# matsengrp/linearham

Measured on AMD Instinct MI355X. Metric: phylo-HMM log-likelihood evals/sec (100-leaf x 400-site family), higher is better.
Workload: dtype f64

## Files before the change

include/linearham_amd.h:

```cpp
#ifndef LINEARHAM_AMD_H_
#define LINEARHAM_AMD_H_

#include <stddef.h>
#include <stdint.h>

#ifdef __cplusplus
extern "C" {
#endif

#define LH_ABI_VERSION 1

typedef struct lh_family lh_family;

typedef struct {
  int32_t n_genes;
  const int32_t* offsets;
  const int32_t* xmsa_inds;
} lh_segments;

typedef struct {
  int32_t n_rows;
  int32_t n_left;
  int32_t n_right;
  const double* enter_trans;
  const double* enter_lo;
  const double* left_trans;
  const double* left_lo;
  const int32_t* left_xmsa;
  const double* right_gp_nli;
  const double* right_ntt;
  const double* right_nlo;
  const double* right_trans;
  const double* right_gp_li;
  const int32_t* right_xmsa;
  const int32_t* nti_xmsa;
  const double* exit_nlo;
  const double* exit_trans;
  const double* exit_gp_li;
} lh_junction;

typedef struct {
  int32_t abi_version;
  int32_t has_d;
  int32_t n_seqs;
  int32_t n_sites;
  const uint8_t* msa;
  int32_t n_xmsa;
  const int32_t* xmsa_site;
  const uint8_t* xmsa_naive_base;
  lh_segments vpadding, vgerm, dgerm, jgerm, jpadding;
  const double* vgerm_gene_prob;
  const double* vpadding_transition;
  const double* vgerm_trans_prod;
  const double* jpadding_transition;
  lh_junction vd, dj;
} lh_family_desc;

typedef struct {
  double* rates;
  double* xmsa_emission;
  double* forward;
  int32_t* scaler_counts;
} lh_eval_outputs;

const char* lh_last_error(void);
int lh_device_count(void);

int lh_warmup(void);
int lh_set_device(int32_t device);
void* lh_host_alloc(size_t bytes);
void lh_host_free(void* p);

int lh_family_create(const lh_family_desc* desc, lh_family** out);
void lh_family_destroy(lh_family* fam);

int64_t lh_forward_size(const lh_family* fam);
int64_t lh_scaler_size(const lh_family* fam);

int lh_family_info(const lh_family* fam, int32_t* n_patterns, int32_t* n_unique_columns);

int lh_family_consensus_sets(const lh_family* fam);

const char* lh_family_prune_form(const lh_family* fam);

const char* lh_family_forward_form(const lh_family* fam);

int lh_family_forward_dj_samples(const lh_family* fam);

int lh_family_forward_dj_waves(const lh_family* fam);

int lh_family_set_extended_range(lh_family* fam, int enable);

typedef struct {
  int32_t n_rows, n_left, n_right, n_states;
  const int32_t* left_rows;
  const int32_t* left_dense;
  const double* left_lo;
  const double* left_trans;
  const double* enter_lo;
  const int32_t* right_dense;
  const int32_t* right_first;
  const double* gene_prob;
  const double* nti_landing_in;
  const double* nti_transition;
  const double* nti_landing_out;
  const double* landing_in;
  const double* right_trans;
  const double* exit_nlo;
  const double* exit_trans;
  const double* exit_li;
  const double* prod;
} lh_sampler_junction;

typedef struct {
  lh_sampler_junction vd, dj;
} lh_sampler_desc;

int lh_family_set_sampler(lh_family* fam, const lh_sampler_desc* desc);

int32_t lh_sample_words(const lh_family* fam);
int32_t lh_sample_states(const lh_family* fam);

int lh_eval_sample_batch(lh_family* fam, int32_t n, int32_t n_tips, int32_t max_depth, const int32_t* ops,
                         const double* brlen, const double* er, const double* pi, const double* alpha,
                         int32_t num_rates, const uint32_t* words, double* loglik, double* rates, int32_t* states);

int lh_eval_sample_batch_device(lh_family* fam, int32_t n, int32_t n_tips, int32_t max_depth, const int32_t* ops,
                                const double* brlen, const double* er, const double* pi, const double* alpha,
                                int32_t num_rates, const uint32_t* words, double* loglik, double* rates,
                                int32_t* states, void* hip_stream);

typedef struct {
  const double* log_offset;
  double* loglik;
  double* posterior;
  double* weighted_sum;
  double* weight_stats;
} lh_posterior_outputs;

int lh_eval_posterior_batch(lh_family* fam, int32_t n, int32_t n_tips, int32_t max_depth, const int32_t* ops,
                            const double* brlen, const double* er, const double* pi, const double* alpha,
                            int32_t num_rates, const lh_posterior_outputs* outs);

int lh_eval_posterior_batch_device(lh_family* fam, int32_t n, int32_t n_tips, int32_t max_depth, const int32_t* ops,
                                   const double* brlen, const double* er, const double* pi, const double* alpha,
                                   int32_t num_rates, const lh_posterior_outputs* outs, void* hip_stream);

int lh_posterior_profile_read(lh_family* fam, double* ms_posterior, int64_t* n_launches);

int lh_family_set_candidates(lh_family* fam, int32_t K, const uint8_t* seqs, double* log_prior);

typedef struct {
  const double* log_offset;
  double* loglik;
  double* log_cand;
  double* weighted_sum;
  double* weight_stats;
} lh_candidate_outputs;

int lh_eval_candidates_batch(lh_family* fam, int32_t n, int32_t n_tips, int32_t max_depth, const int32_t* ops,
                             const double* brlen, const double* er, const double* pi, const double* alpha,
                             int32_t num_rates, const lh_candidate_outputs* outs);

int lh_eval_candidates_batch_device(lh_family* fam, int32_t n, int32_t n_tips, int32_t max_depth, const int32_t* ops,
                                    const double* brlen, const double* er, const double* pi, const double* alpha,
                                    int32_t num_rates, const lh_candidate_outputs* outs, void* hip_stream);

int lh_candidates_info(const lh_family* fam, int32_t* n_candidates, int32_t* n_sites);

int lh_candidates_layout(const lh_family* fam, int32_t* n_var_sites, int32_t* n_lem, int32_t* n_vlem);

int lh_candidates_profile_read(lh_family* fam, double* ms, int64_t* n_launches);

int lh_eval_draw_batch(lh_family* fam, int32_t n, int32_t n_tips, int32_t max_depth, const int32_t* ops,
                       const double* brlen, const double* er, const double* pi, const double* alpha,
                       int32_t num_rates, const uint32_t* words, double* loglik, uint64_t* hash, int32_t* states);

int lh_eval_draw_batch_device(lh_family* fam, int32_t n, int32_t n_tips, int32_t max_depth, const int32_t* ops,
                              const double* brlen, const double* er, const double* pi, const double* alpha,
                              int32_t num_rates, const uint32_t* words, double* loglik, uint64_t* hash,
                              int32_t* states, void* hip_stream);

int lh_naive_sequences(lh_family* fam, int32_t n, const int32_t* states, uint8_t* seqs, uint64_t* hash);

int lh_draws_resolve(lh_family* fam, int32_t n, const int32_t* cand, int32_t* n_mismatch, int32_t* mismatch_rows);
int lh_draws_rows_read(lh_family* fam, int32_t n_rows, const int32_t* rows, uint8_t* seqs);
int lh_draws_candidates_read(lh_family* fam, int32_t* K, uint8_t* seqs);
int lh_draws_reset(lh_family* fam);
int lh_collect_profile_read(lh_family* fam, double* ms, int64_t* n_launches);

#define LH_LINEAGE_PAD_HASH 0ull
int lh_lineage_batch(lh_family* fam, int32_t n, int32_t n_tips, int32_t max_depth, const int32_t* ops,
                     const double* brlen, const double* er, const double* pi, const double* rates, int32_t num_rates,
                     const uint8_t* naive, uint64_t seed, uint64_t first_sample, const int32_t* path,
                     int32_t path_len, uint64_t* nt_hash, uint64_t* aa_hash);

int lh_lineage_collect_device(lh_family* fam, int32_t n, int32_t n_tips, const uint8_t* anc, const uint8_t* naive,
                              const int32_t* path, int32_t path_len, uint64_t* nt_hash, uint64_t* aa_hash,
                              void* hip_stream);

int lh_lineage_resolve(lh_family* fam, int32_t n_slots, const int32_t* ids, int32_t* n_mismatch,
                       int32_t* mismatch_slots);
int lh_lineage_rows_read(lh_family* fam, int32_t n_slots, const int32_t* slots, uint8_t* seqs);
int lh_lineage_store_read(lh_family* fam, int32_t first, int32_t count, int32_t* K, uint8_t* seqs);
int lh_lineage_reset(lh_family* fam);
int lh_lineage_profile_read(lh_family* fam, double* ms, int64_t* n_launches);

typedef struct {
  double* loglik;
  double* rates;
  int32_t* states;
  uint8_t* naive;
  uint64_t* naive_hash;
  uint64_t* nt_hash;
  uint64_t* aa_hash;
} lh_lineage_eval_outputs;

int lh_eval_lineage_batch(lh_family* fam, int32_t n, int32_t n_tips, int32_t max_depth, const int32_t* ops,
                          const double* brlen, const double* er, const double* pi, const double* alpha,
                          int32_t num_rates, const uint32_t* words, uint64_t seed, uint64_t first_sample, int32_t draws,
                          const int32_t* path, int32_t path_len, const lh_lineage_eval_outputs* outs);

int lh_eval_lineage_batch_device(lh_family* fam, int32_t n, int32_t n_tips, int32_t max_depth, const int32_t* ops,
                                 const double* brlen, const double* er, const double* pi, const double* alpha,
                                 int32_t num_rates, const uint32_t* words, uint64_t seed, uint64_t first_sample,
                                 int32_t draws, const int32_t* path, int32_t path_len,
                                 const lh_lineage_eval_outputs* outs, void* hip_stream);

int lh_lineage_eval_profile_read(lh_family* fam, double* ms, int64_t* n_launches);

int lh_schedule_tree(int32_t n_tips, const int32_t* children, int32_t root, int32_t* ops,
                     int32_t* max_depth);

int lh_eval_batch(lh_family* fam, int32_t n, int32_t n_tips, int32_t max_depth, const int32_t* ops,
                  const double* brlen, const double* er, const double* pi, const double* alpha,
                  int32_t num_rates, double* loglik, const lh_eval_outputs* outs);

int lh_eval_batch_device(lh_family* fam, int32_t n, int32_t n_tips, int32_t max_depth,
                         const int32_t* ops, const double* brlen, const double* er, const double* pi,
                         const double* alpha, int32_t num_rates, double* loglik,
                         const lh_eval_outputs* outs, void* hip_stream);

int lh_family_status(lh_family* fam);
// ... 202 lines not shown
```

linearham_amd/capi.py:

```python
import ctypes as C
import os

import numpy as np

_HERE = os.path.dirname(os.path.abspath(__file__))

c_i32p = C.POINTER(C.c_int32)
c_u8p = C.POINTER(C.c_uint8)
c_f64p = C.POINTER(C.c_double)


class _Segments(C.Structure):
    _fields_ = [("n_genes", C.c_int32), ("offsets", c_i32p), ("xmsa_inds", c_i32p)]


class _Junction(C.Structure):
    _fields_ = [("n_rows", C.c_int32), ("n_left", C.c_int32), ("n_right", C.c_int32),
                ("enter_trans", c_f64p), ("enter_lo", c_f64p), ("left_trans", c_f64p),
                ("left_lo", c_f64p), ("left_xmsa", c_i32p), ("right_gp_nli", c_f64p),
                ("right_ntt", c_f64p), ("right_nlo", c_f64p), ("right_trans", c_f64p),
                ("right_gp_li", c_f64p), ("right_xmsa", c_i32p), ("nti_xmsa", c_i32p),
                ("exit_nlo", c_f64p), ("exit_trans", c_f64p), ("exit_gp_li", c_f64p)]


class _FamilyDesc(C.Structure):
    _fields_ = [("abi_version", C.c_int32), ("has_d", C.c_int32), ("n_seqs", C.c_int32),
                ("n_sites", C.c_int32), ("msa", c_u8p), ("n_xmsa", C.c_int32),
                ("xmsa_site", c_i32p), ("xmsa_naive_base", c_u8p),
                ("vpadding", _Segments), ("vgerm", _Segments), ("dgerm", _Segments),
                ("jgerm", _Segments), ("jpadding", _Segments),
                ("vgerm_gene_prob", c_f64p), ("vpadding_transition", c_f64p),
                ("vgerm_trans_prod", c_f64p), ("jpadding_transition", c_f64p),
                ("vd", _Junction), ("dj", _Junction)]


class _EvalOutputs(C.Structure):
    _fields_ = [("rates", c_f64p), ("xmsa_emission", c_f64p), ("forward", c_f64p),
                ("scaler_counts", c_i32p)]


EXPORTS = ["lh_last_error", "lh_device_count", "lh_family_create", "lh_family_destroy",
           "lh_forward_size", "lh_scaler_size", "lh_family_info", "lh_family_consensus_sets", "lh_schedule_tree", "lh_eval_batch",
           "lh_eval_batch_device", "lh_forward_batch", "lh_asr_batch", "lh_asr_batch_device",
           "lh_profile_enable", "lh_profile_read", "lh_asr_profile_read", "lh_family_set_extended_range", "lh_warmup", "lh_host_alloc", "lh_host_free", "lh_family_set_sampler",
           "lh_sample_words", "lh_sample_states", "lh_eval_sample_batch", "lh_set_device", "lh_family_status",
           "lh_eval_sample_batch_device", "lh_family_prune_form", "lh_family_forward_form",
           "lh_family_forward_dj_samples", "lh_family_forward_dj_waves"]
CRAFTED_EXPORTS = ["lh_sample_forward_batch", "lh_posterior_forward_batch"]
EXPORTS += CRAFTED_EXPORTS
POSTERIOR_EXPORTS = ["lh_eval_posterior_batch", "lh_eval_posterior_batch_device", "lh_posterior_profile_read"]
EXPORTS += POSTERIOR_EXPORTS
CANDIDATE_EXPORTS = ["lh_family_set_candidates", "lh_eval_candidates_batch", "lh_eval_candidates_batch_device",
                     "lh_candidates_profile_read", "lh_candidates_info", "lh_candidates_layout"]
EXPORTS += CANDIDATE_EXPORTS
COLLECT_EXPORTS = ["lh_eval_draw_batch", "lh_eval_draw_batch_device", "lh_naive_sequences", "lh_draws_resolve",
                   "lh_draws_rows_read", "lh_draws_candidates_read", "lh_draws_reset", "lh_collect_profile_read"]
EXPORTS += COLLECT_EXPORTS
LINEAGE_EXPORTS = ["lh_lineage_batch", "lh_lineage_collect_device", "lh_lineage_resolve", "lh_lineage_rows_read",
                   "lh_lineage_store_read", "lh_lineage_reset", "lh_lineage_profile_read"]
EXPORTS += LINEAGE_EXPORTS
LINEAGE_PAD_HASH = 0
LINEAGE_EVAL_EXPORTS = ["lh_eval_lineage_batch", "lh_eval_lineage_batch_device", "lh_lineage_eval_profile_read"]
EXPORTS += LINEAGE_EVAL_EXPORTS
VITERBI_EXPORTS = ["lh_eval_viterbi_batch", "lh_eval_viterbi_batch_device", "lh_viterbi_forward_batch",
                   "lh_family_set_candidate_paths", "lh_viterbi_profile_read"]
EXPORTS += VITERBI_EXPORTS
CODON_EXPORTS = ["lh_family_set_codons", "lh_codon_layout", "lh_eval_codons_batch", "lh_eval_codons_batch_device",
                 "lh_codon_profile_read"]
EXPORTS += CODON_EXPORTS
EVENTS_EXPORTS = ["lh_events_layout", "lh_eval_events_batch", "lh_eval_events_batch_device", "lh_events_forward_batch",
                  "lh_events_profile_read"]
EXPORTS += EVENTS_EXPORTS
ANCESTRAL_EXPORTS = ["lh_asr_marginals_batch", "lh_asr_marginals_batch_device", "lh_eval_ancestral_batch",
                     "lh_eval_ancestral_batch_device", "lh_ancestral_profile_read"]
EXPORTS += ANCESTRAL_EXPORTS
EDGES_EXPORTS = ["lh_asr_edges_batch", "lh_asr_edges_batch_device", "lh_eval_edges_batch", "lh_eval_edges_batch_device",
                 "lh_edges_profile_read"]
EXPORTS += EDGES_EXPORTS
ANCESTRAL_PROBS_EXPORTS = ["lh_family_set_ancestral_candidates", "lh_ancestral_candidates_info",
                           "lh_eval_ancestral_candidates_batch", "lh_eval_ancestral_candidates_batch_device",
                           "lh_ancestral_candidates_profile_read"]
EXPORTS += ANCESTRAL_PROBS_EXPORTS
NODE_PARENT, NODE_MRCA = 0, 1


class _CodonOutputs(C.Structure):
    _fields_ = [("log_offset", c_f64p), ("loglik", c_f64p), ("windows", c_f64p), ("genes", c_f64p),
                ("weighted_windows", c_f64p), ("weighted_genes", c_f64p), ("weight_stats", c_f64p)]


class _CodonOutputsDevice(C.Structure):
    _fields_ = [(k, C.c_void_p) for k in ("log_offset", "loglik", "windows", "genes", "weighted_windows",
                                          "weighted_genes", "weight_stats")]


class _EventsOutputs(C.Structure):
    _fields_ = [("log_offset", c_f64p), ("loglik", c_f64p), ("events", c_f64p), ("genes", c_f64p),
                ("weighted_events", c_f64p), ("weighted_genes", c_f64p), ("weight_stats", c_f64p)]


class _EventsOutputsDevice(C.Structure):
    _fields_ = [(k, C.c_void_p) for k in ("log_offset", "loglik", "events", "genes", "weighted_events", "weighted_genes",
                                          "weight_stats")]


class _ViterbiOutputs(C.Structure):
    _fields_ = [("log_offset", c_f64p), ("loglik", c_f64p), ("states", c_i32p), ("log_path", c_f64p),
                ("weight_stats", c_f64p)]


class _ViterbiOutputsDevice(C.Structure):
    _fields_ = [(k, C.c_void_p) for k in ("log_offset", "loglik", "states", "log_path", "weight_stats")]


_ANCESTRAL_MEMBERS = ("log_offset", "loglik", "site_base", "marg", "rate_post", "weighted_sum", "weighted_rate",
                      "weight_stats")


class _AncestralOutputs(C.Structure):
    _fields_ = [(k, c_f64p) for k in _ANCESTRAL_MEMBERS]


class _AncestralOutputsDevice(C.Structure):
    _fields_ = [(k, C.c_void_p) for k in _ANCESTRAL_MEMBERS]


_EDGES_MEMBERS = ("edge", "naive_edge", "chain_counts", "edge_load", "rate_post")
_EVAL_EDGES_MEMBERS = ("log_offset", "loglik", "site_base", "edge", "naive_edge", "chain_counts", "seed_edge", "edge_load",
                       "rate_post", "weighted_counts", "weighted_seed_edge", "weighted_naive_edge", "weight_stats")


class _EdgesOutputs(C.Structure):
    _fields_ = [(k, c_f64p) for k in _EDGES_MEMBERS]


class _EdgesOutputsDevice(C.Structure):
    _fields_ = [(k, C.c_void_p) for k in _EDGES_MEMBERS]


class _EvalEdgesOutputs(C.Structure):
    _fields_ = [(k, c_f64p) for k in _EVAL_EDGES_MEMBERS]


class _EvalEdgesOutputsDevice(C.Structure):
    _fields_ = [(k, C.c_void_p) for k in _EVAL_EDGES_MEMBERS]


_ANCESTRAL_PROBS_MEMBERS = ("log_offset", "loglik", "cond", "log_cand", "weighted_sum", "weight_stats")


class _AncestralProbsOutputs(C.Structure):
    _fields_ = [(k, c_f64p) for k in _ANCESTRAL_PROBS_MEMBERS]


class _AncestralProbsOutputsDevice(C.Structure):
    _fields_ = [(k, C.c_void_p) for k in _ANCESTRAL_PROBS_MEMBERS]


class _SamplerJunction(C.Structure):
    _fields_ = [("n_rows", C.c_int32), ("n_left", C.c_int32), ("n_right", C.c_int32), ("n_states", C.c_int32),
                ("left_rows", c_i32p), ("left_dense", c_i32p), ("left_lo", c_f64p), ("left_trans", c_f64p),
                ("enter_lo", c_f64p), ("right_dense", c_i32p), ("right_first", c_i32p), ("gene_prob", c_f64p),
                ("nti_landing_in", c_f64p), ("nti_transition", c_f64p), ("nti_landing_out", c_f64p),
                ("landing_in", c_f64p), ("right_trans", c_f64p), ("exit_nlo", c_f64p), ("exit_trans", c_f64p),
                ("exit_li", c_f64p), ("prod", c_f64p)]


class _SamplerDesc(C.Structure):
    _fields_ = [("vd", _SamplerJunction), ("dj", _SamplerJunction)]


class _PosteriorOutputs(C.Structure):
    _fields_ = [("log_offset", c_f64p), ("loglik", c_f64p), ("posterior", c_f64p), ("weighted_sum", c_f64p),
                ("weight_stats", c_f64p)]


class _CandidateOutputs(C.Structure):
    _fields_ = [("log_offset", c_f64p), ("loglik", c_f64p), ("log_cand", c_f64p), ("weighted_sum", c_f64p),
                ("weight_stats", c_f64p)]


class _LineageEvalOutputs(C.Structure):
    _fields_ = [("loglik", c_f64p), ("rates", c_f64p), ("states", c_i32p), ("naive", c_u8p),
                ("naive_hash", C.POINTER(C.c_uint64)), ("nt_hash", C.POINTER(C.c_uint64)),
                ("aa_hash", C.POINTER(C.c_uint64))]


class _LineageEvalOutputsDevice(C.Structure):
    _fields_ = [(k, C.c_void_p) for k in ("loglik", "rates", "states", "naive", "naive_hash", "nt_hash", "aa_hash")]


def library_path():
    return os.path.join(os.environ.get("LH_LIB_DIR") or os.path.join(_HERE, "lib"), "liblinearham_hip.so")


_HOST_TREE = [C.c_void_p, C.c_int32, C.c_int32, C.c_int32, c_i32p, c_f64p, c_f64p, c_f64p, c_f64p, C.c_int32]
_DEV_TREE = [C.c_void_p, C.c_int32, C.c_int32, C.c_int32] + [C.c_void_p] * 5 + [C.c_int32]
_PROFILE_READ = [C.c_void_p, c_f64p, C.POINTER(C.c_int64)]


class HipLibrary:
    def __init__(self, path=None):
        path = path or library_path()
        if not os.path.exists(path):
            raise RuntimeError("HIP library %s is missing: run `python -c 'import __graft_entry__ as g; "
                               "g.build()'` (there is no CPU fallback)" % path)
        self.lib = lib = C.CDLL(path)
        c_u32p, c_u64p = C.POINTER(C.c_uint32), C.POINTER(C.c_uint64)
        lib.lh_last_error.restype = C.c_char_p
        lib.lh_device_count.restype = C.c_int
        lib.lh_family_create.argtypes = [C.POINTER(_FamilyDesc), C.POINTER(C.c_void_p)]
        lib.lh_family_destroy.argtypes = [C.c_void_p]
        lib.lh_family_destroy.restype = None
        lib.lh_forward_size.argtypes = [C.c_void_p]
        lib.lh_forward_size.restype = C.c_int64
        lib.lh_scaler_size.argtypes = [C.c_void_p]
        lib.lh_scaler_size.restype = C.c_int64
        lib.lh_family_info.argtypes = [C.c_void_p, C.POINTER(C.c_int32), C.POINTER(C.c_int32)]
        lib.lh_family_info.restype = C.c_int
        lib.lh_family_consensus_sets.argtypes = [C.c_void_p]
        lib.lh_family_consensus_sets.restype = C.c_int
        lib.lh_family_prune_form.argtypes = [C.c_void_p]
        lib.lh_family_prune_form.restype = C.c_char_p
        lib.lh_family_forward_form.argtypes = [C.c_void_p]
        lib.lh_family_forward_form.restype = C.c_char_p
        if hasattr(lib, "lh_family_forward_dj_samples"):
            lib.lh_family_forward_dj_samples.argtypes = [C.c_void_p]
            lib.lh_family_forward_dj_samples.restype = C.c_int
        if hasattr(lib, "lh_family_forward_dj_waves"):
            lib.lh_family_forward_dj_waves.argtypes = [C.c_void_p]
            lib.lh_family_forward_dj_waves.restype = C.c_int
        lib.lh_schedule_tree.argtypes = [C.c_int32, c_i32p, C.c_int32, c_i32p, c_i32p]
        lib.lh_eval_batch.argtypes = _HOST_TREE + [c_f64p, C.POINTER(_EvalOutputs)]
        lib.lh_eval_batch_device.argtypes = _DEV_TREE + [C.c_void_p, C.POINTER(_EvalOutputs), C.c_void_p]
        lib.lh_forward_batch.argtypes = [C.c_void_p, C.c_int32, c_f64p, c_f64p, C.POINTER(_EvalOutputs)]
        lib.lh_asr_batch.argtypes = _HOST_TREE + [c_u8p, C.c_uint64, C.c_uint64, c_u8p, c_u8p]
        lib.lh_asr_batch_device.argtypes = _DEV_TREE + [C.c_void_p, C.c_uint64, C.c_uint64] + [C.c_void_p] * 3
        lib.lh_asr_profile_read.argtypes = _PROFILE_READ
        lib.lh_profile_enable.argtypes = [C.c_void_p, C.c_int]
        lib.lh_family_set_extended_range.argtypes = [C.c_void_p, C.c_int]
        lib.lh_profile_read.argtypes = [C.c_void_p, c_f64p, c_f64p, c_f64p, C.POINTER(C.c_int64)]
        if hasattr(lib, "lh_eval_sample_batch_device"):
            lib.lh_eval_sample_batch_device.argtypes = _DEV_TREE + [C.c_void_p] * 5
            lib.lh_sample_words.argtypes = [C.c_void_p]
            lib.lh_sample_states.argtypes = [C.c_void_p]
        if hasattr(lib, "lh_sample_forward_batch"):
            lib.lh_sample_forward_batch.argtypes = [C.c_void_p, C.c_int32, c_f64p, c_u32p, c_f64p, c_i32p,
                                                    C.POINTER(_EvalOutputs)]
            lib.lh_posterior_forward_batch.argtypes = [C.c_void_p, C.c_int32, c_f64p, c_f64p, c_f64p]
        if hasattr(lib, "lh_eval_posterior_batch"):
            lib.lh_eval_posterior_batch.argtypes = _HOST_TREE + [C.POINTER(_PosteriorOutputs)]
            lib.lh_eval_posterior_batch_device.argtypes = _DEV_TREE + [C.POINTER(_PosteriorOutputs), C.c_void_p]
            lib.lh_posterior_profile_read.argtypes = _PROFILE_READ
        if hasattr(lib, "lh_family_set_candidates"):
            lib.lh_family_set_candidates.argtypes = [C.c_void_p, C.c_int32, c_u8p, c_f64p]
            lib.lh_eval_candidates_batch.argtypes = _HOST_TREE + [C.POINTER(_CandidateOutputs)]
            lib.lh_eval_candidates_batch_device.argtypes = _DEV_TREE + [C.POINTER(_CandidateOutputs), C.c_void_p]
            lib.lh_candidates_profile_read.argtypes = _PROFILE_READ
            lib.lh_candidates_info.argtypes = [C.c_void_p, c_i32p, c_i32p]
            lib.lh_candidates_layout.argtypes = [C.c_void_p, c_i32p, c_i32p, c_i32p]
        if hasattr(lib, "lh_naive_sequences"):
            lib.lh_eval_draw_batch.argtypes = _HOST_TREE + [c_u32p, c_f64p, c_u64p, c_i32p]
            lib.lh_eval_draw_batch_device.argtypes = _DEV_TREE + [C.c_void_p] * 5
            lib.lh_naive_sequences.argtypes = [C.c_void_p, C.c_int32, c_i32p, c_u8p, c_u64p]
            lib.lh_draws_resolve.argtypes = [C.c_void_p, C.c_int32, c_i32p, c_i32p, c_i32p]
            lib.lh_draws_rows_read.argtypes = [C.c_void_p, C.c_int32, c_i32p, c_u8p]
            lib.lh_draws_candidates_read.argtypes = [C.c_void_p, c_i32p, c_u8p]
            lib.lh_draws_reset.argtypes = [C.c_void_p]
            lib.lh_collect_profile_read.argtypes = _PROFILE_READ
        if hasattr(lib, "lh_lineage_batch"):
            lib.lh_lineage_batch.argtypes = _HOST_TREE + [c_u8p, C.c_uint64, C.c_uint64, c_i32p, C.c_int32, c_u64p, c_u64p]
            lib.lh_lineage_collect_device.argtypes = [C.c_void_p, C.c_int32, C.c_int32, C.c_void_p, C.c_void_p,
                                                      C.c_void_p, C.c_int32, C.c_void_p, C.c_void_p, C.c_void_p]
            lib.lh_lineage_resolve.argtypes = [C.c_void_p, C.c_int32, c_i32p, c_i32p, c_i32p]
            lib.lh_lineage_rows_read.argtypes = [C.c_void_p, C.c_int32, c_i32p, c_u8p]
            lib.lh_lineage_store_read.argtypes = [C.c_void_p, C.c_int32, C.c_int32, c_i32p, c_u8p]
            lib.lh_lineage_reset.argtypes = [C.c_void_p]
            lib.lh_lineage_profile_read.argtypes = _PROFILE_READ
        if hasattr(lib, "lh_eval_lineage_batch"):
            lib.lh_eval_lineage_batch.argtypes = _HOST_TREE + [c_u32p, C.c_uint64, C.c_uint64, C.c_int32, c_i32p, C.c_int32,
                                                               C.POINTER(_LineageEvalOutputs)]
            lib.lh_eval_lineage_batch_device.argtypes = _DEV_TREE + [
                C.c_void_p, C.c_uint64, C.c_uint64, C.c_int32, C.c_void_p, C.c_int32, C.POINTER(_LineageEvalOutputsDevice),
                C.c_void_p]
            lib.lh_lineage_eval_profile_read.argtypes = _PROFILE_READ
        if hasattr(lib, "lh_eval_viterbi_batch"):
            lib.lh_family_set_sampler.argtypes = [C.c_void_p, C.POINTER(_SamplerDesc)]
            lib.lh_eval_viterbi_batch.argtypes = _HOST_TREE + [C.POINTER(_ViterbiOutputs)]
            lib.lh_eval_viterbi_batch_device.argtypes = _DEV_TREE + [C.POINTER(_ViterbiOutputsDevice), C.c_void_p]
            lib.lh_viterbi_forward_batch.argtypes = [C.c_void_p, C.c_int32, c_f64p, c_f64p, c_i32p]
            lib.lh_family_set_candidate_paths.argtypes = [C.c_void_p, C.c_int32, c_i32p, c_f64p]
            lib.lh_viterbi_profile_read.argtypes = _PROFILE_READ
        if hasattr(lib, "lh_family_set_codons"):
            lib.lh_family_set_codons.argtypes = [C.c_void_p, C.c_int32]
            lib.lh_codon_layout.argtypes = [C.c_void_p, c_i32p, c_i32p, c_i32p, c_i32p]
            lib.lh_eval_codons_batch.argtypes = _HOST_TREE + [C.POINTER(_CodonOutputs)]
            lib.lh_eval_codons_batch_device.argtypes = _DEV_TREE + [C.POINTER(_CodonOutputsDevice), C.c_void_p]
            lib.lh_codon_profile_read.argtypes = _PROFILE_READ
        if hasattr(lib, "lh_events_layout"):
            c_i64p = C.POINTER(C.c_int64)
            lib.lh_events_layout.argtypes = [C.c_void_p, c_i32p, c_i32p, c_i32p, c_i32p, c_i64p, c_i64p, c_i64p, c_i64p,
                                             c_i32p]
            lib.lh_eval_events_batch.argtypes = _HOST_TREE + [C.POINTER(_EventsOutputs)]
            lib.lh_eval_events_batch_device.argtypes = _DEV_TREE + [C.POINTER(_EventsOutputsDevice), C.c_void_p]
            lib.lh_events_forward_batch.argtypes = [C.c_void_p, C.c_int32, c_f64p, c_f64p, c_f64p]
            lib.lh_events_profile_read.argtypes = _PROFILE_READ
        if hasattr(lib, "lh_asr_marginals_batch"):
            lib.lh_asr_marginals_batch.argtypes = _HOST_TREE + [c_f64p, c_i32p, C.c_int32, c_f64p, c_f64p]
            lib.lh_asr_marginals_batch_device.argtypes = _DEV_TREE + [C.c_void_p, C.c_void_p, C.c_int32] + [C.c_void_p] * 3
            lib.lh_eval_ancestral_batch.argtypes = _HOST_TREE + [c_i32p, C.c_int32, C.POINTER(_AncestralOutputs)]
            lib.lh_eval_ancestral_batch_device.argtypes = _DEV_TREE + [C.c_void_p, C.c_int32,
                                                                       C.POINTER(_AncestralOutputsDevice), C.c_void_p]
            lib.lh_ancestral_profile_read.argtypes = _PROFILE_READ
        if hasattr(lib, "lh_asr_edges_batch"):
            lib.lh_asr_edges_batch.argtypes = _HOST_TREE + [c_f64p, c_i32p, C.c_int32, C.c_int32, C.POINTER(_EdgesOutputs)]
            lib.lh_asr_edges_batch_device.argtypes = _DEV_TREE + [C.c_void_p, C.c_void_p, C.c_int32, C.c_int32,
                                                                  C.POINTER(_EdgesOutputsDevice), C.c_void_p]
            lib.lh_eval_edges_batch.argtypes = _HOST_TREE + [c_i32p, C.c_int32, C.c_int32, C.POINTER(_EvalEdgesOutputs)]
            lib.lh_eval_edges_batch_device.argtypes = _DEV_TREE + [C.c_void_p, C.c_int32, C.c_int32,
                                                                   C.POINTER(_EvalEdgesOutputsDevice), C.c_void_p]
            lib.lh_edges_profile_read.argtypes = _PROFILE_READ
        if hasattr(lib, "lh_family_set_ancestral_candidates"):
            lib.lh_family_set_ancestral_candidates.argtypes = [C.c_void_p, C.c_int32, c_u8p]
            lib.lh_ancestral_candidates_info.argtypes = [C.c_void_p, c_i32p, c_i32p]
            lib.lh_eval_ancestral_candidates_batch.argtypes = _HOST_TREE + [c_i32p, C.c_int32, C.c_int32,
                                                                            C.POINTER(_AncestralProbsOutputs)]
            lib.lh_eval_ancestral_candidates_batch_device.argtypes = _DEV_TREE + [
                C.c_void_p, C.c_int32, C.c_int32, C.POINTER(_AncestralProbsOutputsDevice), C.c_void_p]
            lib.lh_ancestral_candidates_profile_read.argtypes = _PROFILE_READ
        if hasattr(lib, "lh_set_device"):
            lib.lh_set_device.argtypes = [C.c_int32]
            lib.lh_family_status.argtypes = [C.c_void_p]

    def error(self):
        return self.lib.lh_last_error().decode()

    def check(self, rc):
        if rc != 0:
            raise RuntimeError("linearham_hip: " + self.error())

    def device_count(self):
        return self.lib.lh_device_count()

    def _profile_read(self, name, family, n_ms=1):
        ms, k = (C.c_double * n_ms)(), C.c_int64()
        self.check(getattr(self.lib, name)(_handle(family), ms, C.byref(k)))
        return tuple(ms) + (k.value,)

    def eval_posterior_batch(self, family, n_tips, max_depth, ops, brlen, er, pi, alpha, num_rates, log_offset=None,
                             want=("loglik", "posterior", "weighted_sum", "weight_stats")):
        h = _handle(family)
        n, arrays = _tree_args(ops, brlen, er, pi, alpha)
        fs = self.lib.lh_forward_size(h)
        res, outs = _outputs(_PosteriorOutputs, want, log_offset, loglik=(n,), posterior=(n, fs), weighted_sum=(fs,),
                             weight_stats=(3,))
        self.check(self.lib.lh_eval_posterior_batch(h, n, n_tips, max_depth, *_tree_ptrs(arrays), num_rates, C.byref(outs)))
        return res

    def eval_ancestral_batch(self, family, n_tips, max_depth, ops, brlen, er, pi, alpha, num_rates, path, log_offset=None,
                             want=("loglik", "site_base", "marg", "rate_post", "weighted_sum", "weighted_rate",
                                   "weight_stats")):
        h = _handle(family)
        n, arrays = _tree_args(ops, brlen, er, pi, alpha)
        path = _i32(path)
        assert path.ndim == 2 and path.shape[0] == n
        P, R = path.shape[1], num_rates
        _, L = self.candidates_info(h)
        res, outs = _outputs(_AncestralOutputs, want, log_offset, loglik=(n,), site_base=(n, L, 5), marg=(n, P, L, 4),
                             rate_post=(n, L, R), weighted_sum=(2, L, 4), weighted_rate=(L, R), weight_stats=(3,))
        self.check(self.lib.lh_eval_ancestral_batch(h, n, n_tips, max_depth, *_tree_ptrs(arrays), num_rates,
                                                    _ptr(path, c_i32p), P, C.byref(outs)))
        return res

    def eval_ancestral_batch_device(self, family, n, n_tips, max_depth, ops_ptr, brlen_ptr, er_ptr, pi_ptr, alpha_ptr,
                                    num_rates, path_ptr, path_len, outs, stream=0):
        o = _AncestralOutputsDevice(**{k: int(v) for k, v in outs.items() if v})
        self.check(self.lib.lh_eval_ancestral_batch_device(_handle(family), n, n_tips, max_depth, ops_ptr, brlen_ptr, er_ptr,
                                                           pi_ptr, alpha_ptr, num_rates, path_ptr, path_len, C.byref(o),
                                                           stream))

    def ancestral_profile_read(self, family):
        return self._profile_read("lh_ancestral_profile_read", family, 3)

    def ancestral_candidates_info(self, family):
# ... 412 lines not shown

    def c(self):
        j = _Junction()
        j.n_rows, j.n_left, j.n_right = self.n_rows, self.n_left, self.n_right
        for k in self.F64:
            setattr(j, k, getattr(self, k).ctypes.data_as(c_f64p))
        for k in self.I32:
            setattr(j, k, getattr(self, k).ctypes.data_as(c_i32p))
        return j


class SamplerJunction:
    F64 = ["left_lo", "left_trans", "enter_lo", "gene_prob", "nti_landing_in", "nti_transition", "nti_landing_out",
           "landing_in", "right_trans", "exit_nlo", "exit_trans", "exit_li", "prod"]
    I32 = ["left_rows", "left_dense", "right_dense", "right_first"]

    def __init__(self, n_rows, n_left, n_right, n_states, **arrays):
        self.n_rows, self.n_left, self.n_right, self.n_states = n_rows, n_left, n_right, n_states
        for k in self.F64:
            setattr(self, k, _f64(arrays[k]))
        for k in self.I32:
            setattr(self, k, _i32(arrays[k]))

    def c(self):
        j = _SamplerJunction()
        j.n_rows, j.n_left, j.n_right, j.n_states = self.n_rows, self.n_left, self.n_right, self.n_states
        for k in self.F64:
            setattr(j, k, getattr(self, k).ctypes.data_as(c_f64p))
        for k in self.I32:
            setattr(j, k, getattr(self, k).ctypes.data_as(c_i32p))
        return j


class FamilyDesc:

    def __init__(self, has_d, msa, xmsa_site, xmsa_naive_base, vpadding, vgerm, dgerm, jgerm, jpadding,
                 vgerm_gene_prob, vpadding_transition, vgerm_trans_prod, jpadding_transition, vd, dj,
                 n_xmsa=None):
        self.has_d = int(has_d)
        self.msa = np.ascontiguousarray(msa, dtype=np.uint8)
        self.xmsa_site = _i32(xmsa_site)
        self.xmsa_naive_base = np.ascontiguousarray(xmsa_naive_base, dtype=np.uint8)
        self.n_xmsa = int(n_xmsa if n_xmsa is not None else len(self.xmsa_site))
        self.vpadding, self.vgerm, self.dgerm, self.jgerm, self.jpadding = vpadding, vgerm, dgerm, jgerm, jpadding
        self.vgerm_gene_prob = _f64(vgerm_gene_prob)
        self.vpadding_transition = _f64(vpadding_transition)
        self.vgerm_trans_prod = _f64(vgerm_trans_prod)
        self.jpadding_transition = _f64(jpadding_transition)
        self.vd, self.dj = vd, dj

    def c(self):
        d = _FamilyDesc()
        d.abi_version = 1
        d.has_d = self.has_d
        d.n_seqs = self.msa.shape[0] if self.msa.ndim == 2 else 0
        d.n_sites = self.msa.shape[1] if self.msa.ndim == 2 else 0
        d.msa = self.msa.ctypes.data_as(c_u8p)
        d.n_xmsa = self.n_xmsa
        d.xmsa_site = self.xmsa_site.ctypes.data_as(c_i32p)
        d.xmsa_naive_base = self.xmsa_naive_base.ctypes.data_as(c_u8p)
        d.vpadding, d.vgerm, d.jgerm, d.jpadding = (self.vpadding.c(), self.vgerm.c(), self.jgerm.c(),
                                                    self.jpadding.c())
        if self.dgerm is not None:
            d.dgerm = self.dgerm.c()
        d.vgerm_gene_prob = self.vgerm_gene_prob.ctypes.data_as(c_f64p)
        d.vpadding_transition = self.vpadding_transition.ctypes.data_as(c_f64p)
        d.vgerm_trans_prod = self.vgerm_trans_prod.ctypes.data_as(c_f64p)
        d.jpadding_transition = self.jpadding_transition.ctypes.data_as(c_f64p)
        d.vd = self.vd.c()
        if self.dj is not None:
            d.dj = self.dj.c()
        return d


class Family:

    def __init__(self, desc, lib=None):
        self.hip = lib or load_library()
        self.desc = desc
        h = C.c_void_p()
        cdesc = desc.c()
        self.hip.check(self.hip.lib.lh_family_create(C.byref(cdesc), C.byref(h)))
        self.handle = h
        self.forward_size = self.hip.lib.lh_forward_size(h)
        self.scaler_size = self.hip.lib.lh_scaler_size(h)
        self.n_xmsa = desc.n_xmsa
        self.consensus_sets = self.hip.lib.lh_family_consensus_sets(h)

    @classmethod
    def borrow(cls, handle, lib=None):
        self = cls.__new__(cls)
        self.hip = lib or load_library()
        self.desc = None
        self.handle = C.c_void_p(handle) if isinstance(handle, int) else handle
        self.owned = False
        self.forward_size = self.hip.lib.lh_forward_size(self.handle)
        self.scaler_size = self.hip.lib.lh_scaler_size(self.handle)
        return self

    def close(self):
        if self.handle:
            if getattr(self, "owned", True):
                self.hip.lib.lh_family_destroy(self.handle)
            self.handle = None

    def __del__(self):
        try:
            self.close()
        except Exception:
            pass

    def _outs(self, n, R, want):
        shapes = dict(rates=(n, R), forward=(n, self.forward_size), scaler_counts=((n, self.scaler_size), np.int32))
        if "xmsa_emission" in want:
            shapes["xmsa_emission"] = (n, self.n_xmsa)
        res, outs = _outputs(_EvalOutputs, want, **shapes)
        return outs, res

    def eval_batch(self, n_tips, max_depth, ops, brlen, er, pi, alpha, num_rates, want=()):
        _, arrays = _tree_args(ops, brlen, er, pi, alpha)
        ops, brlen, er, pi, alpha = arrays
        n = alpha.shape[0]
        assert ops.shape == (n, n_tips - 2, 4) and brlen.shape == (n, 2 * n_tips - 2)
        assert er.shape == (n, 6) and pi.shape == (n, 4)
        ll = np.zeros(n)
        outs, res = self._outs(n, num_rates, want)
        self.hip.check(self.hip.lib.lh_eval_batch(self.handle, n, n_tips, max_depth, *_tree_ptrs(arrays), num_rates,
                                                  _ptr(ll), C.byref(outs)))
        return ll, res

    def eval_batch_device(self, n, n_tips, max_depth, ops_ptr, brlen_ptr, er_ptr, pi_ptr, alpha_ptr,
                          num_rates, loglik_ptr, stream=0):
        self.hip.check(self.hip.lib.lh_eval_batch_device(
            self.handle, n, n_tips, max_depth, ops_ptr, brlen_ptr, er_ptr, pi_ptr, alpha_ptr, num_rates,
            loglik_ptr, None, stream))

    def info(self):
        a, b = C.c_int32(), C.c_int32()
        self.hip.check(self.hip.lib.lh_family_info(self.handle, C.byref(a), C.byref(b)))
        return a.value, b.value

    def k1_form(self):
        return self.hip.lib.lh_family_prune_form(self.handle).decode()

    def k2_form(self):
        return self.hip.lib.lh_family_forward_form(self.handle).decode()

    def k2_dj_samples(self):
        return int(self.hip.lib.lh_family_forward_dj_samples(self.handle))

    def k2_dj_waves(self):
        return int(self.hip.lib.lh_family_forward_dj_waves(self.handle))

    def status(self):
        self.hip.check(self.hip.lib.lh_family_status(self.handle))

    def forward_batch(self, em, want=()):
        em = _f64(em)
        n = em.shape[0]
        assert em.shape == (n, self.n_xmsa)
        ll = np.zeros(n)
        outs, res = self._outs(n, 1, [w for w in want if w in ("forward", "scaler_counts")])
        self.hip.check(self.hip.lib.lh_forward_batch(self.handle, n, em.ctypes.data_as(c_f64p),
                                                     ll.ctypes.data_as(c_f64p), C.byref(outs)))
        return ll, res

    def asr_batch(self, n_tips, max_depth, ops, brlen, er, pi, rates, naive, seed, first_sample=0):
        _, arrays = _tree_args(ops, brlen, er, pi, rates)
        ops, brlen, er, pi, rates = arrays
        naive = np.ascontiguousarray(naive, dtype=np.uint8)
        n, L = naive.shape
        assert ops.shape == (n, n_tips - 2, 4) and brlen.shape == (n, 2 * n_tips - 2)
        assert er.shape == (n, 6) and pi.shape == (n, 4) and rates.shape[0] == n
        anc = np.zeros((n, n_tips - 2, L), dtype=np.uint8)
        choice = np.zeros((n, L), dtype=np.uint8)
        self.hip.check(self.hip.lib.lh_asr_batch(self.handle, n, n_tips, max_depth, *_tree_ptrs(arrays), rates.shape[1],
                                                 _ptr(naive, c_u8p), seed, first_sample, _ptr(anc, c_u8p),
                                                 _ptr(choice, c_u8p)))
        return anc, choice

    def asr_marginals_batch(self, n_tips, max_depth, ops, brlen, er, pi, rates, naive_prob, path,
                            want=("marg", "rate_post")):
        _, arrays = _tree_args(ops, brlen, er, pi, rates)
        ops, brlen, er, pi, rates = arrays
        naive_prob = _f64(naive_prob)
        path = _i32(path)
        n, L = naive_prob.shape[:2]
        assert naive_prob.shape == (n, L, 5) and path.ndim == 2 and path.shape[0] == n
        assert ops.shape == (n, n_tips - 2, 4) and brlen.shape == (n, 2 * n_tips - 2)
        assert er.shape == (n, 6) and pi.shape == (n, 4) and rates.shape[0] == n
        P, R = path.shape[1], rates.shape[1]
        marg = np.zeros((n, P, L, 4)) if "marg" in want else None
        rate_post = np.zeros((n, L, R)) if "rate_post" in want else None
        self.hip.check(self.hip.lib.lh_asr_marginals_batch(
            self.handle, n, n_tips, max_depth, *_tree_ptrs(arrays), R, _ptr(naive_prob), _ptr(path, c_i32p), P,
            _ptr(marg), _ptr(rate_post)))
        return marg, rate_post

    def asr_marginals_batch_device(self, n, n_tips, max_depth, ops_ptr, brlen_ptr, er_ptr, pi_ptr, rates_ptr, num_rates,
                                   naive_prob_ptr, path_ptr, path_len, marg_ptr, rate_post_ptr, stream=0):
        self.hip.check(self.hip.lib.lh_asr_marginals_batch_device(
            self.handle, n, n_tips, max_depth, ops_ptr, brlen_ptr, er_ptr, pi_ptr, rates_ptr, num_rates, naive_prob_ptr,
            path_ptr, path_len, marg_ptr, rate_post_ptr, stream))

    def ancestral_profile_read(self):
        r = self.hip._profile_read("lh_ancestral_profile_read", self.handle, 3)
        return dict(zip(("k11a_ms", "k11b_ms", "reduce_ms"), r[:3])), r[3]

    def asr_edges_batch(self, n_tips, max_depth, ops, brlen, er, pi, rates, naive_prob, path, seed_tip,
                        want=_EDGES_MEMBERS):
        _, arrays = _tree_args(ops, brlen, er, pi, rates)
        ops, brlen, er, pi, rates = arrays
        naive_prob = _f64(naive_prob)
        path = _i32(path)
        n, L = naive_prob.shape[:2]
        assert naive_prob.shape == (n, L, 5) and path.ndim == 2 and path.shape[0] == n
        assert ops.shape == (n, n_tips - 2, 4) and brlen.shape == (n, 2 * n_tips - 2)
        assert er.shape == (n, 6) and pi.shape == (n, 4) and rates.shape[0] == n
        P, R = path.shape[1], rates.shape[1]
        res, outs = _outputs(_EdgesOutputs, want, edge=(n, P, L, 4, 4), naive_edge=(n, L, 5, 4), chain_counts=(n, L, 4, 4),
                             edge_load=(n, P + 1), rate_post=(n, L, R))
        self.hip.check(self.hip.lib.lh_asr_edges_batch(
            self.handle, n, n_tips, max_depth, *_tree_ptrs(arrays), R, _ptr(naive_prob), _ptr(path, c_i32p), P, int(seed_tip),
            C.byref(outs)))
        return res

    def asr_edges_batch_device(self, n, n_tips, max_depth, ops_ptr, brlen_ptr, er_ptr, pi_ptr, rates_ptr, num_rates,
                               naive_prob_ptr, path_ptr, path_len, seed_tip, outs, stream=0):
        o = _EdgesOutputsDevice(**{k: int(v) for k, v in outs.items() if v})
        self.hip.check(self.hip.lib.lh_asr_edges_batch_device(
            self.handle, n, n_tips, max_depth, ops_ptr, brlen_ptr, er_ptr, pi_ptr, rates_ptr, num_rates, naive_prob_ptr,
            path_ptr, path_len, int(seed_tip), C.byref(o), stream))

    def edges_profile_read(self):
        r = self.hip._profile_read("lh_edges_profile_read", self.handle, 3)
        return dict(zip(("k11a_ms", "k12b_ms", "reduce_ms"), r[:3])), r[3]

    def lineage_batch(self, n_tips, max_depth, ops, brlen, er, pi, rates, naive, seed, path, first_sample=0):
        _, arrays = _tree_args(ops, brlen, er, pi, rates)
        ops, brlen, er, pi, rates = arrays
        naive = np.ascontiguousarray(naive, dtype=np.uint8)
        path = _i32(path)
        n, L = naive.shape
        assert ops.shape == (n, n_tips - 2, 4) and brlen.shape == (n, 2 * n_tips - 2)
        assert er.shape == (n, 6) and pi.shape == (n, 4) and rates.shape[0] == n and path.shape[0] == n
        P = path.shape[1]
        nt = np.zeros((n, P + 1), dtype=np.uint64)
        aa = np.zeros((n, P + 1), dtype=np.uint64)
        u64 = C.POINTER(C.c_uint64)
        self.hip.check(self.hip.lib.lh_lineage_batch(
            self.handle, n, n_tips, max_depth, *_tree_ptrs(arrays), rates.shape[1], _ptr(naive, c_u8p), seed, first_sample,
            _ptr(path, c_i32p), P, _ptr(nt, u64), _ptr(aa, u64)))
        self._lineage_sites = L
        return nt, aa

    def eval_lineage_batch(self, n_tips, max_depth, ops, brlen, er, pi, alpha, num_rates, words, seed, path, draws=1,
                           first_sample=0):
        n, arrays = _tree_args(ops, brlen, er, pi, alpha)
        ops, brlen, er, pi, alpha = arrays
        words = np.ascontiguousarray(words, dtype=np.uint32)
        path = _i32(path)
        assert ops.shape == (n, n_tips - 2, 4) and brlen.shape == (n, 2 * n_tips - 2)
        assert er.shape == (n, 6) and pi.shape == (n, 4) and alpha.shape == (n,) and path.shape[0] == n
        P = path.shape[1]
        lib = self.hip.lib
        _, L = self.hip.candidates_info(self.handle)
        d = max(int(draws), 0)
        shapes = dict(loglik=(n,), rates=(n, num_rates), states=((n, lib.lh_sample_states(self.handle)), np.int32),
                      naive=((n, L), np.uint8), naive_hash=((n,), np.uint64), nt_hash=((n, d, P + 1), np.uint64),
                      aa_hash=((n, d, P + 1), np.uint64))
        res, outs = _outputs(_LineageEvalOutputs, shapes, **shapes)
        self.hip.check(lib.lh_eval_lineage_batch(
            self.handle, n, n_tips, max_depth, *_tree_ptrs(arrays), num_rates, _ptr(words, C.POINTER(C.c_uint32)), seed,
            first_sample, draws, _ptr(path, c_i32p), P, C.byref(outs)))
        self._lineage_sites = L
        return res

    def eval_lineage_batch_device(self, n, n_tips, max_depth, ops_ptr, brlen_ptr, er_ptr, pi_ptr, alpha_ptr, num_rates,
                                  words_ptr, seed, first_sample, draws, path_ptr, path_len, outs, stream=0):
        o = _LineageEvalOutputsDevice(**{k: int(v) for k, v in outs.items() if v})
        self.hip.check(self.hip.lib.lh_eval_lineage_batch_device(
            self.handle, n, n_tips, max_depth, ops_ptr, brlen_ptr, er_ptr, pi_ptr, alpha_ptr, num_rates, words_ptr, seed,
            first_sample, draws, path_ptr, path_len, C.byref(o), stream))
        _, self._lineage_sites = self.hip.candidates_info(self.handle)

    def lineage_eval_profile_read(self):
        r = self.hip._profile_read("lh_lineage_eval_profile_read", self.handle, 5)
        return dict(zip(("k0_ms", "k1_ms", "k2_k4_k6c_ms", "k3_ms", "k7_ms"), r[:5])), r[5]

    def lineage_collect_device(self, n, n_tips, anc_ptr, naive_ptr, path_ptr, path_len, nt_hash_ptr, aa_hash_ptr,
                               stream=0):
        self.hip.check(self.hip.lib.lh_lineage_collect_device(self.handle, n, n_tips, anc_ptr, naive_ptr, path_ptr,
                                                              path_len, nt_hash_ptr, aa_hash_ptr, stream))

    def lineage_resolve(self, ids):
        ids = np.ascontiguousarray(ids, dtype=np.int32).reshape(-1)
        slots = np.zeros(max(len(ids), 1), dtype=np.int32)
        nm = C.c_int32()
        self.hip.check(self.hip.lib.lh_lineage_resolve(self.handle, len(ids), ids.ctypes.data_as(c_i32p), C.byref(nm),
                                                       slots.ctypes.data_as(c_i32p)))
        return slots[:nm.value].copy()

    def lineage_rows_read(self, slots, n_sites=None):
        slots = np.ascontiguousarray(slots, dtype=np.int32)
        out = np.zeros((len(slots), n_sites or self._lineage_sites), dtype=np.uint8)
        self.hip.check(self.hip.lib.lh_lineage_rows_read(self.handle, len(slots), slots.ctypes.data_as(c_i32p),
# ... 49 lines not shown
```

linearham_amd/csrc/lh_capi.hip:

```cpp
#include <algorithm>
#include <array>
#include <map>
#include <cstdio>
#include <cstring>
#include <functional>
#include <atomic>
#include <chrono>
#include <string>
#include <thread>
#include <utility>
#include <vector>

#include "lh_device.h"

namespace lh {
const DebugOptions& debug_options() {
  static const DebugOptions opts = [] {
    DebugOptions o;
    auto set = [](const char* name) { return std::getenv(name) != nullptr; };
    auto num = [](const char* name, int dflt) { const char* e = std::getenv(name); return e ? std::atoi(e) : dflt; };
    o.chunk = std::max(256, num("LH_CHUNK", o.chunk));
    o.host_sub = std::max(256, num("LH_HOST_SUB", o.host_sub));
    o.eval_split = std::min(8, std::max(0, num("LH_EVAL_SPLIT", o.eval_split)));
    o.k0_serial = set("LH_K0_SERIAL");
    o.eval_fwd_priority = std::min(1, num("LH_EVAL_FWD_PRIORITY", o.eval_fwd_priority));
    o.k2b_no_pair = set("LH_K2B_NO_PAIR");
    o.k2b_vd_single = set("LH_K2B_VD_SINGLE");
    o.k2b_dj_pair = set("LH_K2B_DJ_PAIR");
    o.sample_timing = set("LH_SAMPLE_TIMING");
    o.k4_no_save = set("LH_K4_NO_SAVE");
    o.k1_tile_cap = num("LH_K1_TILE_CAP", 0);
    o.k1_cxx_walk = set("LH_K1_CXX_WALK");
    o.k1_tables = set("LH_K1_TABLES");
    o.k1_stack = set("LH_K1_STACK");
    o.k1_no_tables = set("LH_K1_NO_TABLES");
    o.k1_segments = set("LH_K1_SEGMENTS");
    o.k1_seg_waves = num("LH_K1_SEG_WAVES", o.k1_seg_waves);
    o.k1_no_fuse = set("LH_K1_NO_FUSE");
    o.codon_blocks = std::max(1, num("LH_CODON_BLOCKS", o.codon_blocks));
    o.events_blocks = std::max(1, num("LH_EVENTS_BLOCKS", o.events_blocks));
    o.anc_out_mb = std::max(1, num("LH_ANC_OUT_MB", o.anc_out_mb));
    o.edge_out_mb = std::max(1, num("LH_EDGE_OUT_MB", o.edge_out_mb));
    o.anc_pairs = std::max(0, num("LH_ANC_PAIRS", o.anc_pairs));
    o.collect_hash_bits = std::min(64, std::max(1, num("LH_COLLECT_HASH_BITS", o.collect_hash_bits)));
    return o;
  }();
  return opts;
}
}

namespace {

thread_local std::string g_error;

int fail(const std::string& msg) {
  g_error = msg;
  return 1;
}

#define LH_HIP(expr)                                                                      \
  do {                                                                                    \
    hipError_t e_ = (expr);                                                               \
    if (e_ != hipSuccess)                                                                 \
      return fail(std::string(#expr) + ": " + hipGetErrorString(e_));                     \
  } while (0)

template <bool Pinned>
class Buffer {
 public:
  Buffer() = default;
  Buffer(const Buffer&) = delete;
  Buffer& operator=(const Buffer&) = delete;
  ~Buffer() { release(); }
  int ensure(size_t bytes) {
    bytes = std::max<size_t>(bytes, 64);
    if (bytes <= cap_) return 0;
    if (p_) {
      LH_HIP(hipDeviceSynchronize());
      release();
    }
    LH_HIP(Pinned ? hipHostMalloc(&p_, bytes, hipHostMallocDefault) : hipMalloc(&p_, bytes));
    cap_ = bytes;
    return 0;
  }
  template <typename T = void>
  T* get() const { return static_cast<T*>(p_); }

 private:
  void release() {
    if (p_) (void)(Pinned ? hipHostFree(p_) : hipFree(p_));
    p_ = nullptr;
    cap_ = 0;
  }
  void* p_ = nullptr;
  size_t cap_ = 0;
};
using DevBuf = Buffer<false>;
using PinnedBuf = Buffer<true>;

template <int Stages>
class KernelTimer {
 public:
  KernelTimer() = default;
  KernelTimer(const KernelTimer&) = delete;
  KernelTimer& operator=(const KernelTimer&) = delete;
  ~KernelTimer() {
    for (Events& es : done_) destroy(es);
    destroy(open_);
    destroy(done_spans_);
    destroy(open_spans_);
  }
  int begin(hipStream_t s) {
    destroy(open_);
    for (hipEvent_t& e : open_) LH_HIP(hipEventCreate(&e));
    return mark(0, s);
  }
  int mark(int k, hipStream_t s) {
    LH_HIP(hipEventRecord(open_[k], s));
    return 0;
  }
  int end(hipStream_t s) {
    if (mark(Stages, s)) return 1;
    done_.push_back(std::exchange(open_, Events{}));
    return 0;
  }
  void begin_spans() {
    destroy(open_);
    destroy(open_spans_);
  }
  int span_begin(int stage, hipStream_t s) {
    Span sp{stage, nullptr, nullptr};
    LH_HIP(hipEventCreate(&sp.a));
    open_spans_.push_back(sp);
    LH_HIP(hipEventCreate(&open_spans_.back().b));
    LH_HIP(hipEventRecord(sp.a, s));
    return 0;
  }
  int span_end(hipStream_t s) {
    LH_HIP(hipEventRecord(open_spans_.back().b, s));
    return 0;
  }
  void end_spans() {
    done_spans_.insert(done_spans_.end(), open_spans_.begin(), open_spans_.end());
    open_spans_.clear();
    ++span_groups_;
  }
  int read(double* ms, int64_t* launches) {
    double sum[Stages] = {};
    hipError_t e = hipSuccess;
    for (Span& sp : done_spans_) {
      if (e == hipSuccess) e = hipEventSynchronize(sp.b);
      float t = 0;
      if (e == hipSuccess) e = hipEventElapsedTime(&t, sp.a, sp.b);
      sum[sp.stage] += t;
    }
    destroy(done_spans_);
    for (Events& es : done_) {
      if (e == hipSuccess) e = hipEventSynchronize(es[Stages]);
      for (int k = 0; k < Stages && e == hipSuccess; ++k) {
        float t = 0;
        e = hipEventElapsedTime(&t, es[k], es[k + 1]);
        sum[k] += t;
      }
      destroy(es);
    }
    const int64_t n = (int64_t)done_.size() + std::exchange(span_groups_, 0);
    done_.clear();
    LH_HIP(e);
    if (ms) std::copy(sum, sum + Stages, ms);
    if (launches) *launches = n;
    return 0;
  }

 private:
  using Events = std::array<hipEvent_t, Stages + 1>;
  static void destroy(Events& es) {
    for (hipEvent_t& e : es)
      if (e) (void)hipEventDestroy(std::exchange(e, nullptr));
  }
  struct Span {
    int stage;
// ... 300 lines not shown
    for (int j = a + 1; j < b; ++j)
      if (xmsa_site[s.xmsa_inds[j]] != xmsa_site[s.xmsa_inds[j - 1]] + 1) return 0;
    lo = std::min(lo, xmsa_site[s.xmsa_inds[a]]);
    hi = std::max(hi, xmsa_site[s.xmsa_inds[b - 1]] + 1);
    total += b - a;
  }
  if (hi < 0 || total < 4096) return 0;
  const int ns = hi - lo;
  if (ns > 510) return 0;
  std::vector<std::map<int32_t, int>> votes(ns);
  for (int g = 0; g < n; ++g)
    for (int j = s.offsets[g]; j < s.offsets[g + 1]; ++j) ++votes[xmsa_site[s.xmsa_inds[j]] - lo][ucol[s.xmsa_inds[j]]];
  std::vector<int32_t> cons(ns, n_ucol);
  for (int p = 0; p < ns; ++p) {
    int best = 0;
    for (const auto& kv : votes[p])
      if (kv.second > best) {
        best = kv.second;
        cons[p] = kv.first;
      }
  }
  std::vector<std::vector<uint32_t>> diffs(n);
  std::vector<uint32_t> rng(n, 0);
  size_t max_diff = 0;
  for (int g = 0; g < n; ++g) {
    const int a = s.offsets[g], b = s.offsets[g + 1];
    if (a == b) continue;
    const int first = xmsa_site[s.xmsa_inds[a]] - lo;
    rng[g] = (uint32_t)first | ((uint32_t)(first + (b - a)) << 16);
    for (int j = a; j < b; ++j) {
      const int p = first + (j - a);
      const int32_t u = ucol[s.xmsa_inds[j]];
      if (u != cons[p]) diffs[g].push_back((uint32_t)p | ((uint32_t)(u * scale) << 16));
    }
    max_diff = std::max(max_diff, diffs[g].size());
    rng[g] |= (uint32_t)((diffs[g].size() + 7) / 8) << 25;
  }
  max_diff = (max_diff + 7) & ~(size_t)7;
  if ((long long)ns + (long long)n * (long long)(max_diff + 8) > total / 2) return 0;
  std::vector<uint16_t> col(ns);
  for (int p = 0; p < ns; ++p) col[p] = (uint16_t)(cons[p] * scale);
  const uint32_t pad = (uint32_t)ns | ((uint32_t)(n_ucol * scale) << 16);
  std::vector<uint32_t> dif(std::max<size_t>(max_diff, 8) * n, pad);
  for (int g = 0; g < n; ++g)
    for (size_t k = 0; k < diffs[g].size(); ++k) dif[k * n + g] = diffs[g][k];
  if (upload_vec(f, col, &d->cons_col)) return 1;
  if (upload_vec(f, rng, &d->cons_rng)) return 1;
  if (upload_vec(f, dif, &d->cons_dif)) return 1;
  d->cons_sites = ns;
  d->cons_diffs = (int32_t)max_diff;
  return 0;
}

int upload_segments(lh_family* f, const lh_segments& s, int n_xmsa, const std::vector<int32_t>& ucol, int n_ucol,
                    const int32_t* xmsa_site, lh::DevSegments* d) {
  const int scale = f->host.idx_byte_offsets ? 8 : 1;
  if (s.n_genes < 0) return fail("segments: negative gene count");
  d->n_genes = s.n_genes;
  d->cons_sites = 0;
  d->cons_diffs = 0;
  d->cons_col = nullptr;
  d->cons_rng = nullptr;
  d->cons_dif = nullptr;
  if (s.n_genes > 0) {
    if (!s.offsets) return fail("segments: null offsets");
    if (s.offsets[0] != 0) return fail("segments: offsets[0] != 0");
    for (int g = 0; g < s.n_genes; ++g)
      if (s.offsets[g + 1] < s.offsets[g]) return fail("segments: offsets not monotone");
    const int total = s.offsets[s.n_genes];
    for (int j = 0; j < total; ++j)
      if (s.xmsa_inds[j] < 0 || s.xmsa_inds[j] >= n_xmsa) return fail("segments: xMSA index out of range");
    int longest = 0;
    for (int g = 0; g < s.n_genes; ++g) longest = std::max(longest, s.offsets[g + 1] - s.offsets[g]);
    d->n_chunks = (longest + 7) / 8;
    if (n_ucol > 0xfffe) return fail("segments: more than 65534 distinct xMSA columns");
    std::vector<uint16_t> t((size_t)d->n_chunks * s.n_genes * 8, (uint16_t)(n_ucol * scale));
    for (int g = 0; g < s.n_genes; ++g)
      for (int j = s.offsets[g]; j < s.offsets[g + 1]; ++j) {
        const int k = j - s.offsets[g];
        t[((size_t)(k / 8) * s.n_genes + g) * 8 + (k % 8)] = (uint16_t)(ucol[s.xmsa_inds[j]] * scale);
      }
    const uint16_t* dev = nullptr;
    if (upload(f, t.data(), t.size(), &dev)) return 1;
    d->inds_c = reinterpret_cast<const uint4*>(dev);
    if (upload_consensus(f, s, ucol, n_ucol, xmsa_site, scale, d)) return 1;
  } else {
    d->n_chunks = 0;
    const uint16_t* dev = nullptr;
    if (upload<uint16_t>(f, nullptr, 0, &dev)) return 1;
    d->inds_c = reinterpret_cast<const uint4*>(dev);
  }
  return 0;
}

int check_idx(const int32_t* a, size_t n, int n_xmsa, bool allow_neg, const char* what) {
  for (size_t i = 0; i < n; ++i)
    if (a[i] >= n_xmsa || (a[i] < 0 && !(allow_neg && a[i] == -1)))
      return fail(std::string("junction: xMSA index out of range in ") + what);
  return 0;
}

int collect_junction_cols(const lh_junction& j, int n_xmsa, std::vector<int32_t>* used) {
  const size_t W = j.n_rows, nL = j.n_left, nR = j.n_right;
  if (j.n_rows < 1 || j.n_left < 1 || j.n_right < 1) return fail("junction: bad dimensions");
  if (!j.left_xmsa || !j.right_xmsa || !j.nti_xmsa) return fail("lh_family_create: null array in junction descriptor");
  if (check_idx(j.left_xmsa, W * nL, n_xmsa, true, "left_xmsa")) return 1;
  if (check_idx(j.right_xmsa, W * nR, n_xmsa, true, "right_xmsa")) return 1;
  if (check_idx(j.nti_xmsa, W * nR * 4, n_xmsa, false, "nti_xmsa")) return 1;
  auto mark = [&](const int32_t* p, size_t n) {
    for (size_t i = 0; i < n; ++i)
      if (p[i] >= 0) (*used)[p[i]] = 1;
  };
  mark(j.left_xmsa, W * nL);
  mark(j.right_xmsa, W * nR);
  mark(j.nti_xmsa, W * nR * 4);
  return 0;
}

template <typename T>
std::vector<T> pad_genes(const T* src, size_t rows, size_t n, size_t n_pad, size_t inner, T fill) {
  std::vector<T> t(rows * n_pad * inner, fill);
  for (size_t i = 0; i < rows; ++i)
    for (size_t g = 0; g < n; ++g)
      for (size_t u = 0; u < inner; ++u) t[(i * n_pad + g) * inner + u] = src[(i * n + g) * inner + u];
  return t;
}

template <typename T>
int upload_vec(lh_family* f, const std::vector<T>& v, const T** out) {
  return upload(f, v.data(), v.size(), out);
}

int upload_junction(lh_family* f, const lh_junction& j, const std::vector<int32_t>& remap, int n_jcols,
                    const int32_t* xmsa_site, const std::vector<int32_t>& pat_of_site, int left_chunks, int right_chunks,
                    lh::DevJunction* d) {
  const size_t W = j.n_rows, nL = j.n_left, nR = j.n_right;
  const size_t pL = std::max<size_t>((nL + 63) / 64, (size_t)left_chunks) * 64,
               pR = std::max<size_t>((nR + 63) / 64, (size_t)right_chunks) * 64;
  d->n_rows = j.n_rows;
  d->n_left = j.n_left;
  d->n_right = j.n_right;
  d->left_pad = (int32_t)pL;
  d->right_pad = (int32_t)pR;
  if (!j.enter_trans || !j.enter_lo || !j.left_trans || !j.left_lo || !j.right_gp_nli || !j.right_ntt ||
      !j.right_nlo || !j.right_trans || !j.right_gp_li || !j.exit_nlo || !j.exit_trans || !j.exit_gp_li)
    return fail("lh_family_create: null array in junction descriptor");
  auto cols = [&](const int32_t* src, size_t rows, size_t n, size_t n_pad, size_t inner) {
    std::vector<int32_t> t = pad_genes<int32_t>(src, rows, n, n_pad, inner, -1);
    for (int32_t& x : t) x = x >= 0 ? remap[x] : n_jcols;
    return t;
  };
  std::vector<double> ltr = pad_genes<double>(j.left_trans, W, nL, pL, 1, 0.0);
  for (size_t l = 0; l < nL; ++l) ltr[l] = j.enter_trans[l];
  std::vector<double> ntt(pR * 16, 0.0);
  for (size_t r = 0; r < nR; ++r)
    for (int a = 0; a < 4; ++a)
      for (int b = 0; b < 4; ++b) ntt[r * 16 + b * 4 + a] = j.right_ntt[r * 16 + a * 4 + b];
  if (upload_vec(f, pad_genes<double>(j.enter_lo, 1, nL, pL, 1, 0.0), &d->enter_lo)) return 1;
  if (upload_vec(f, ltr, &d->left_trans)) return 1;
  if (upload_vec(f, pad_genes<double>(j.left_lo, W, nL, pL, 1, 0.0), &d->left_lo)) return 1;
  if (upload_vec(f, cols(j.left_xmsa, W, nL, pL, 1), &d->left_xmsa)) return 1;
  if (upload_vec(f, pad_genes<double>(j.right_gp_nli, 1, nR, pR, 4, 0.0), &d->right_gp_nli)) return 1;
  if (upload_vec(f, ntt, &d->right_ntt)) return 1;
  if (upload_vec(f, pad_genes<double>(j.right_nlo, W, nR, pR, 4, 0.0), &d->right_nlo)) return 1;
  if (upload_vec(f, pad_genes<double>(j.right_trans, W, nR, pR, 1, 0.0), &d->right_trans)) return 1;
  if (upload_vec(f, pad_genes<double>(j.right_gp_li, W, nR, pR, 1, 0.0), &d->right_gp_li)) return 1;
  if (upload_vec(f, cols(j.right_xmsa, W, nR, pR, 1), &d->right_xmsa)) return 1;
  if (upload_vec(f, cols(j.nti_xmsa, W, nR, pR, 4), &d->nti_xmsa)) return 1;
  if (upload_vec(f, pad_genes<double>(j.exit_nlo, 1, nR, pR, 4, 0.0), &d->exit_nlo)) return 1;
  if (upload_vec(f, pad_genes<double>(j.exit_trans, 1, nR, pR, 1, 0.0), &d->exit_trans)) return 1;
  if (upload_vec(f, pad_genes<double>(j.exit_gp_li, 1, nR, pR, 1, 0.0), &d->exit_gp_li)) return 1;
  std::vector<int32_t> row_pat(W, f->host.n_prune);
  if (xmsa_site)
    for (size_t i = 0; i < W; ++i) row_pat[i] = pat_of_site[xmsa_site[j.nti_xmsa[i * nR * 4]]];
  if (upload_vec(f, row_pat, &d->row_pat)) return 1;
  return 0;
}

size_t k1_bytes_per_sample(const lh_family* f, int T, int R) {
  const lh::PruneWsSizes z = lh::prune_ws_sizes(T, f->host.msa_mixed_n != 0);
  const size_t n_ops = (size_t)std::max(T - 2, 1);
  return sizeof(double) * R * z.scratch_doubles_per_rate + n_ops * (sizeof(int2) + sizeof(double)) +
         z.tabs_per_sample * sizeof(int4) + sizeof(int4);
}

int ensure_workspace(lh_family* f, int n, int R, int T) {
  Workspace& w = f->ws;
  const size_t L = std::max<size_t>(f->host.n_prune, 1), cap = std::max(n, 1);
  const lh::PruneWsSizes z = lh::prune_ws_sizes(T, f->host.msa_mixed_n != 0);
  const size_t n_ops = (size_t)std::max(T - 2, 1);
  if (w.rates.ensure(sizeof(double) * cap * R) || w.eig.ensure(sizeof(double) * cap * 36) ||
      w.scratch.ensure(sizeof(double) * cap * R * z.scratch_doubles_per_rate) || w.wops.ensure(sizeof(int2) * cap * n_ops) ||
      w.wlen.ensure(sizeof(double) * cap * n_ops) || w.tabs.ensure(sizeof(int4) * cap * z.tabs_per_sample) ||
      w.hdr.ensure(sizeof(int4) * cap) || w.site_lik.ensure(sizeof(double) * cap * R * 5 * L) ||
      w.site_scal.ensure(sizeof(int32_t) * cap * R * L))
    return 1;
  w.prune = {w.scratch.get<double>(), w.wops.get<int2>(), w.wlen.get<double>(), w.tabs.get<int4>(), w.hdr.get<int4>(),
             f->err_flag};
  return 0;
}

static const int kChunk = lh::debug_options().chunk;

int run_forward(lh_family* f, int n, int R, const double* site_lik, const int32_t* site_scal, const double* pi,
                const double* em_in, double* em_out, double* loglik_dev, const lh_eval_outputs* outs,
                size_t sample_offset, hipStream_t stream, const lh::LogEmRequest& lem = lh::LogEmRequest{}, size_t row0 = 0,
                size_t rows = 0) {
  double* fwd = (outs && outs->forward) ? outs->forward + sample_offset * f->host.forward_size : nullptr;
  int32_t* sco =
      (outs && outs->scaler_counts) ? outs->scaler_counts + sample_offset * f->host.scaler_size : nullptr;
  ForwardWs& w = f->fws;
  const size_t m = std::max(rows, row0 + (size_t)n);
  const size_t jrows = f->host.vd.n_rows + (f->host.has_d ? f->host.dj.n_rows : 0);
  if (w.jrs.ensure(sizeof(int32_t) * m * std::max(f->host.vd.n_rows + f->host.dj.n_rows, 1)) ||
      w.dxf.ensure(sizeof(double) * m * 32) || w.dxc.ensure(sizeof(int32_t) * m) ||
      w.gem.ensure(sizeof(double) * m * std::max<int64_t>(f->host.gem_size, 1)) ||
      w.jem.ensure(sizeof(double) * m * std::max(f->host.n_jcols, 1)) || w.gcnt.ensure(sizeof(int32_t) * m * 3))
    return 1;
  lh::launch_forward(f->host, f->dev, n, R, site_lik, site_scal, pi, em_in, em_out, w.gem.get<double>() + row0 * f->host.gem_size,
                     w.gcnt.get<int32_t>() + row0 * 3, w.jem.get<double>() + row0 * f->host.n_jcols,
                     w.jrs.get<int32_t>() + row0 * jrows, w.dxf.get<double>() + row0 * 32, w.dxc.get<int32_t>() + row0, loglik_dev,
                     fwd, sco, f->extended, stream, lem);
  f->k2_form = lh::forward_last_form();
  f->k2_dj_samples = lh::forward_last_dj_samples();
  f->k2_dj_waves = lh::forward_last_dj_waves();
  LH_HIP(hipGetLastError());
  return 0;
}

int check_async_error(lh_family* f, const char* who) {
  int32_t flag = 0;
  LH_HIP(hipDeviceSynchronize());
  LH_HIP(hipMemcpy(&flag, f->err_flag, sizeof(flag), hipMemcpyDeviceToHost));
  if (flag) {
    LH_HIP(hipMemset(f->err_flag, 0, sizeof(flag)));
    if (flag == 2)
      return fail(std::string(who) + ": lineage path that is not a chain up to the root, or (edge tables) a seed tip that is not a "
                                     "child of its first node; the affected samples' results are NaN");
    return fail(std::string(who) + ": malformed schedule op (use lh_schedule_tree); the affected samples' results are NaN");
  }
  return 0;
}

struct TreeBatch {
  int32_t n, T, max_depth;
  const int32_t* ops;
  const double* brlen;
  const double* er;
  const double* pi;
  const double* model;
  int32_t R;
  bool per_rate = false;
  size_t nodes() const { return 2 * (size_t)T - 2; }
  size_t n_ops() const { return (size_t)T - 2; }
  size_t model_stride() const { return per_rate ? (size_t)R : 1; }
  bool has_arrays() const { return ops && brlen && er && pi && model; }
  const int32_t* schedule(size_t i) const { return ops + i * n_ops() * 4; }
  TreeBatch slice(size_t off, int32_t m) const {
    return {m, T, max_depth, schedule(off), brlen + off * nodes(), er + off * 6, pi + off * 4, model + off * model_stride(),
            R, per_rate};
  }
  std::array<size_t, 5> sample_bytes() const {
    return {sizeof(int32_t) * 4 * n_ops(), sizeof(double) * nodes(), sizeof(double) * 6, sizeof(double) * 4,
            sizeof(double) * model_stride()};
  }
};

int check_batch(const lh_family* f, const std::string& w, const TreeBatch& b, bool needs_sampler = false) {
  const int n = b.n, T = b.T, R = b.R, max_depth = b.max_depth;
  if (!f) return fail(w + ": null family");
  if (needs_sampler && !f->have_sampler) return fail(w + ": lh_family_set_sampler has not been called");
  if (n < 0) return fail(w + ": negative batch size");
  if (n == 0) return -1;
  if (f->host.n_seqs < 1) return fail(w + ": family was created without an MSA (forward-only)");
  if (T != f->host.n_seqs + 1) return fail(w + ": n_tips must equal n_seqs + 1 (naive)");
  if (T < 3) return fail(w + ": need at least 3 tips");
  if (R < 1 || R > 64) return fail(w + ": num_rates out of range");
  if (max_depth < 0 || max_depth > 16) return fail(w + ": max_depth out of range");
  if ((size_t)T * 128 > 160 * 1024) return fail(w + ": too many tips for the LDS tip table");
  return 0;
}

size_t eval_bytes_per_sample(const lh_family* f, int T, int R) {
  return k1_bytes_per_sample(f, T, R) + sizeof(double) * R * 6 * (size_t)std::max(f->host.n_prune, 1);
}

size_t eval_group(const lh_family* f, int T, int R) {
  return std::min<size_t>(kChunk, std::max<size_t>(1024, ((size_t)16 << 30) / eval_bytes_per_sample(f, T, R)));
}

size_t asr_group(const lh_family* f, int T, int R, size_t clv_per_sample) {
  return std::min<size_t>(8192, std::max<size_t>(64, ((size_t)8 << 30) / (clv_per_sample + eval_bytes_per_sample(f, T, R))));
}

int prune_group(lh_family* f, const std::string& who, const TreeBatch& g, const double* rates, bool mix, hipStream_t stream,
                int* planes, size_t row0 = 0, int row0_planes = 0, const lh::PruneFork* fork = nullptr) {
  Workspace& w = f->ws;
  const lh::PruneWsSizes z = lh::prune_ws_sizes(g.T, f->host.msa_mixed_n != 0);
  const size_t L = (size_t)std::max(f->host.n_prune, 0), pl = (size_t)row0_planes;
  lh::PruneWs p = w.prune;
  p.scratch += row0 * g.R * z.scratch_doubles_per_rate;
  p.wops += row0 * g.n_ops();
  p.wlen += row0 * g.n_ops();
  p.tabs += row0 * z.tabs_per_sample;
  p.hdr += row0;
  *planes = lh::launch_prune(f->host, g.n, g.R, g.T, g.max_depth, g.ops, g.brlen, rates, w.eig.get<double>() + row0 * 36, p, g.pi,
                             w.site_lik.get<double>() + row0 * pl * 5 * L, w.site_scal.get<int32_t>() + row0 * pl * L, stream,
                             mix, f->extended || !mix, fork);
  if (*planes < 0) return fail(who + ": " + lh::prune_last_error());
  f->k1_form = lh::prune_last_form();
  if (!mix && *planes != g.R && f->host.n_prune > 0) return fail(who + ": internal error (rate planes were mixed)");
  if (row0 > 0 && *planes != row0_planes) return fail(who + ": internal error (sub-batches with different rate planes)");
  return 0;
}

bool valid_op(const int32_t* op, int T, int nodes, int max_depth) {
  const int kind = op[0] & 15;
  const bool push = op[0] & lh::OP_PUSH_FLAG;
  const int rank = op[0] >> lh::OP_RANK_SHIFT;
// ... 313 lines not shown
      rc = rc || upload(f, u_pat.data(), u_pat.size(), &h.u_pat);
      rc = rc || upload(f, u_base.data(), u_base.size(), &h.u_base);
      rc = rc || upload(f, ucol.data(), C, &h.ucol_of_col);
      rc = rc || upload(f, col_of_ucol.data(), col_of_ucol.size(), &h.col_of_ucol);
    }
  } else {
    for (size_t c = 0; c < C; ++c) ucol[c] = (int32_t)c;
    h.n_pat = 0;
    h.n_prune = 0;
    h.msa_mixed_n = 0;
    h.n_ucol = (int32_t)C;
    f->n_ucol_used = (int32_t)C;
    rc = rc || upload<uint8_t>(f, nullptr, 0, &h.msa);
    h.msa_planes = nullptr;
    rc = rc || upload<int32_t>(f, nullptr, 0, &h.site_pat);
    rc = rc || upload<int32_t>(f, nullptr, 0, &h.u_pat);
    rc = rc || upload<uint8_t>(f, nullptr, 0, &h.u_base);
    rc = rc || upload(f, ucol.data(), C, &h.ucol_of_col);
    rc = rc || upload(f, ucol.data(), C, &h.col_of_ucol);
  }
  h.idx_byte_offsets = ((int64_t)h.n_ucol + 1) * 8 <= 0xffff ? 1 : 0;
  const int32_t* seg_site = (desc->n_seqs > 0 && !rc) ? desc->xmsa_site : nullptr;
  rc = rc || upload_segments(f, desc->vpadding, desc->n_xmsa, ucol, h.n_ucol, seg_site, &h.vpadding);
  rc = rc || upload_segments(f, desc->vgerm, desc->n_xmsa, ucol, h.n_ucol, seg_site, &h.vgerm);
  rc = rc || upload_segments(f, desc->jgerm, desc->n_xmsa, ucol, h.n_ucol, seg_site, &h.jgerm);
  rc = rc || upload_segments(f, desc->jpadding, desc->n_xmsa, ucol, h.n_ucol, seg_site, &h.jpadding);
  const size_t nV = desc->vgerm.n_genes, nJ = desc->jgerm.n_genes;
  if (!rc && (desc->vpadding.n_genes != (int)nV || desc->jpadding.n_genes != (int)nJ))
    rc = fail("lh_family_create: padding/germline gene counts differ");
  rc = rc || upload(f, desc->vgerm_gene_prob, nV, &h.vgerm_gene_prob);
  rc = rc || upload(f, desc->vpadding_transition, nV, &h.vpadding_transition);
  rc = rc || upload(f, desc->vgerm_trans_prod, nV, &h.vgerm_trans_prod);
  rc = rc || upload(f, desc->jpadding_transition, nJ, &h.jpadding_transition);
  std::vector<int32_t> remap(desc->n_xmsa, 0);
  rc = rc || collect_junction_cols(desc->vd, desc->n_xmsa, &remap);
  if (h.has_d) rc = rc || collect_junction_cols(desc->dj, desc->n_xmsa, &remap);
  if (!rc) {
    std::vector<int32_t> jpos(h.n_ucol, -1), jcols;
    std::vector<char> used_u(h.n_ucol, 0);
    for (int c = 0; c < desc->n_xmsa; ++c)
      if (remap[c]) used_u[ucol[c]] = 1;
    for (int u = 0; u < h.n_ucol; ++u)
      if (used_u[u]) {
        jpos[u] = (int32_t)jcols.size();
        jcols.push_back(u);
      }
    for (int c = 0; c < desc->n_xmsa; ++c) remap[c] = remap[c] ? jpos[ucol[c]] : -1;
    h.n_jcols = (int32_t)jcols.size();
    rc = upload(f, jcols.data(), jcols.size(), &h.jcols);
  }
  auto round_to = [](int c, std::initializer_list<int> steps) {
    for (int s : steps)
      if (c <= s) return s;
    return c;
  };
  const int ga_t = round_to(((int)nV + 63) / 64, {1, 2, 4, 8, 16});
  const int gb_t = round_to((std::max((int)desc->dgerm.n_genes * (h.has_d ? 1 : 0), (int)nJ) + 63) / 64, {1, 2, 4});
  rc = rc || upload_junction(f, desc->vd, remap, h.n_jcols, seg_site, pat_of_site_all, ga_t, gb_t, &h.vd);
  if (!rc && desc->vd.n_left != (int)nV) rc = fail("lh_family_create: vd.n_left != number of V genes");
  if (h.has_d) {
    rc = rc || upload_segments(f, desc->dgerm, desc->n_xmsa, ucol, h.n_ucol, seg_site, &h.dgerm);
    rc = rc || upload_junction(f, desc->dj, remap, h.n_jcols, seg_site, pat_of_site_all, gb_t, gb_t, &h.dj);
    if (!rc && (desc->vd.n_right != desc->dgerm.n_genes || desc->dj.n_left != desc->dgerm.n_genes ||
                desc->dj.n_right != (int)nJ))
      rc = fail("lh_family_create: junction gene counts do not match the germline regions");
  } else {
    lh_segments empty{0, nullptr, nullptr};
    rc = rc || upload_segments(f, empty, desc->n_xmsa, ucol, h.n_ucol, seg_site, &h.dgerm);
    memset(&h.dj, 0, sizeof(h.dj));
    if (!rc && desc->vd.n_right != (int)nJ) rc = fail("lh_family_create: vd.n_right != number of J genes");
  }
  if (!rc) {
    h.max_genes = std::max({(int)nV, (int)nJ, h.dgerm.n_genes, 1});
    h.forward_size = (int64_t)nV + (int64_t)h.vd.n_rows * (h.vd.n_left + 5 * (int64_t)h.vd.n_right) + nJ;
    h.scaler_size = 1 + h.vd.n_rows + 1;
    if (h.has_d) {
      h.forward_size += h.dgerm.n_genes + (int64_t)h.dj.n_rows * (h.dj.n_left + 5 * (int64_t)h.dj.n_right);
      h.scaler_size += h.dj.n_rows + 1;
    }
    h.gem_size = 2 * (int64_t)nV + h.dgerm.n_genes + 2 * (int64_t)nJ;
    if (lh::forward_lds_bytes(h) > 160 * 1024)
      rc = fail("lh_family_create: family too large for the forward kernels' LDS working set");
    else if (nV > 1024 || h.dgerm.n_genes > 256 || nJ > 256)
      rc = fail("lh_family_create: more than 1024 V genes or 256 D/J genes");
  }
  if (!rc) {
    void* p = nullptr;
    if (hipMalloc(&p, sizeof(lh::DevFamily)) != hipSuccess ||
        hipMemcpy(p, &h, sizeof(lh::DevFamily), hipMemcpyHostToDevice) != hipSuccess)
      rc = fail("lh_family_create: device allocation failed");
    else {
      f->dev = static_cast<lh::DevFamily*>(p);
      f->allocs.push_back(p);
    }
  }
  if (!rc && desc->n_seqs > 0) {
    CodonSource& cs = f->codon_src;
    cs.site.assign(desc->xmsa_site, desc->xmsa_site + C);
    cs.base.assign(desc->xmsa_naive_base, desc->xmsa_naive_base + C);
    auto seg = [](const lh_segments& s, CodonSegments* o) {
      o->offsets.assign(s.offsets, s.offsets + s.n_genes + 1);
      o->inds.assign(s.xmsa_inds, s.xmsa_inds + s.offsets[s.n_genes]);
    };
    auto junc = [](const lh_junction& j, CodonSourceJunction* o) {
      const size_t W = j.n_rows, nL = j.n_left, nR = j.n_right;
      o->left_xmsa.assign(j.left_xmsa, j.left_xmsa + W * nL);
      o->right_xmsa.assign(j.right_xmsa, j.right_xmsa + W * nR);
      o->nti_xmsa.assign(j.nti_xmsa, j.nti_xmsa + W * nR * 4);
    };
    seg(desc->vgerm, &cs.v);
    seg(desc->jgerm, &cs.j);
    junc(desc->vd, &cs.vd);
    if (h.has_d) {
      seg(desc->dgerm, &cs.d);
      junc(desc->dj, &cs.dj);
    }
    cs.have = true;
  }
  if (!rc && desc->n_seqs > 0) {
    rc = upload(f, desc->xmsa_site, C, &f->cand.col_site) || upload(f, desc->xmsa_naive_base, C, &f->cand.col_base);
    lh_family_desc d2 = *desc;
    d2.n_seqs = 0;
    d2.msa = nullptr;
    const std::string keep = g_error;
    if (!rc && lh_family_create(&d2, &f->cand.twin)) f->cand.twin_error = g_error;
    g_error = keep;
  }
  if (rc) {
    std::string keep = g_error;
    lh_family_destroy(f);
    g_error = keep;
    return 1;
  }
  *out = f;
  return 0;
}

void lh_family_destroy(lh_family* f) {
  if (!f) return;
  DeviceGuard guard(f);
  lh_family_destroy(std::exchange(f->cand.twin, nullptr));
  for (void* p : f->allocs) (void)hipFree(p);
  delete f;
}

int64_t lh_forward_size(const lh_family* f) { return f ? f->host.forward_size : 0; }

const char* lh_family_prune_form(const lh_family* f) { return f ? f->k1_form.c_str() : ""; }

const char* lh_family_forward_form(const lh_family* f) { return f ? f->k2_form.c_str() : ""; }
int lh_family_forward_dj_samples(const lh_family* f) { return f ? f->k2_dj_samples : 0; }
int lh_family_forward_dj_waves(const lh_family* f) { return f ? f->k2_dj_waves : 0; }

int lh_family_consensus_sets(const lh_family* f) {
  if (!f) return 0;
  const lh::DevFamily& h = f->host;
  return (h.vpadding.cons_sites > 0) | (h.vgerm.cons_sites > 0) << 1 | (h.dgerm.cons_sites > 0) << 2 |
         (h.jgerm.cons_sites > 0) << 3 | (h.jpadding.cons_sites > 0) << 4;
}

int lh_family_info(const lh_family* f, int32_t* n_patterns, int32_t* n_unique_columns) {
  if (!f) return fail("lh_family_info: null family");
  if (n_patterns) *n_patterns = f->host.n_prune;
  if (n_unique_columns) *n_unique_columns = f->n_ucol_used;
  return 0;
}
int64_t lh_scaler_size(const lh_family* f) { return f ? f->host.scaler_size : 0; }

int lh_schedule_tree(int32_t T, const int32_t* children, int32_t root, int32_t* ops, int32_t* max_depth) {
  if (T < 3) return fail("lh_schedule_tree: need at least 3 tips (naive + 2 sequences)");
  const int n_nodes = 2 * T - 2, I = T - 2;
  if (!children || !ops) return fail("lh_schedule_tree: null argument");
  if (root < T || root >= n_nodes) return fail("lh_schedule_tree: root must be an inner node");
  std::vector<int> seen(n_nodes, 0);
  for (int i = 0; i < 2 * I; ++i) {
    const int c = children[i];
    if (c < 1 || c >= n_nodes) return fail("lh_schedule_tree: child id out of range");
    if (seen[c]++) return fail("lh_schedule_tree: node appears twice as a child");
  }
  if (seen[root]) return fail("lh_schedule_tree: root appears as a child");
  for (int v = 1; v < n_nodes; ++v)
    if (v != root && !seen[v]) return fail("lh_schedule_tree: node is not attached to the tree");
  std::vector<int> size(n_nodes, 0), order;
  order.reserve(I);
  {
    std::vector<int> stack{root};
    std::vector<char> visited(n_nodes, 0);
    while (!stack.empty()) {
      const int v = stack.back();
      stack.pop_back();
      if (visited[v]) return fail("lh_schedule_tree: cycle in children array");
      visited[v] = 1;
      if (v >= T) {
        order.push_back(v);
        stack.push_back(children[2 * (v - T)]);
        stack.push_back(children[2 * (v - T) + 1]);
      }
    }
    if ((int)order.size() != I) return fail("lh_schedule_tree: tree does not span all inner nodes");
    for (int k = I - 1; k >= 0; --k) {
      const int v = order[k];
      const int a = children[2 * (v - T)], b = children[2 * (v - T) + 1];
      size[v] = (a < T ? 1 : size[a]) + (b < T ? 1 : size[b]);
    }
  }
  struct Frame {
    int v, phase, first, second;
  };
  std::vector<Frame> fs;
  fs.push_back({root, 0, 0, 0});
  int n_out = 0, depth = 0, maxd = 0;
  int n_inner_mats = 0;
  bool acc_live = false;
  bool push_pending = false;
  while (!fs.empty()) {
    Frame& fr = fs.back();
    const int v = fr.v;
    const int a = children[2 * (v - T)], b = children[2 * (v - T) + 1];
    const bool ta = a < T, tb = b < T;
    int32_t* op = ops + 4 * (size_t)n_out;
    if (ta && tb) {
      op[0] = lh::OP_CHERRY;
      op[1] = a;
      op[2] = b;
      op[3] = 0;
      if (push_pending) {
        op[0] |= lh::OP_PUSH_FLAG;
        op[3] = depth++;
        maxd = std::max(maxd, depth);
        push_pending = false;
      }
      ++n_out;
      acc_live = true;
      fs.pop_back();
    } else if (ta != tb) {
      const int tip = ta ? a : b, inner = ta ? b : a;
      if (fr.phase == 0) {
        fr.phase = 1;
        fs.push_back({inner, 0, 0, 0});
      } else {
        op[0] = lh::OP_TIP_ACC | (n_inner_mats << lh::OP_RANK_SHIFT);
        n_inner_mats += 1;
        op[1] = tip;
        op[2] = inner;
        op[3] = 0;
        ++n_out;
        fs.pop_back();
      }
    } else {
      if (fr.phase == 0) {
        fr.first = size[a] >= size[b] ? a : b;
        fr.second = size[a] >= size[b] ? b : a;
        fr.phase = 1;
        const int first = fr.first;
        fs.push_back({first, 0, 0, 0});
      } else if (fr.phase == 1) {
        fr.phase = 2;
        push_pending = true;
        const int second = fr.second;
        fs.push_back({second, 0, 0, 0});
      } else {
        op[0] = lh::OP_POP_ACC | (n_inner_mats << lh::OP_RANK_SHIFT);
        n_inner_mats += 2;
        op[1] = fr.first;
        op[2] = fr.second;
        op[3] = --depth;
        ++n_out;
        fs.pop_back();
      }
    }
  }
  (void)acc_live;
  if (n_out != I || depth != 0) return fail("lh_schedule_tree: internal scheduling error");
  if (maxd > 16) return fail("lh_schedule_tree: tree needs more than 16 stack slots");
  if (max_depth) *max_depth = maxd;
  return 0;
}

int lh_family_set_extended_range(lh_family* f, int enable) {
  if (!f) return fail("null family");
  f->extended = enable != 0;
  return 0;
}

static int upload_sampler_junction(lh_family* f, const lh_sampler_junction& j, lh::DevSampleJunction* d) {
  const size_t W = j.n_rows, nL = j.n_left, nR = j.n_right;
  if (j.n_rows < 1 || j.n_left < 1 || j.n_right < 1 || j.n_states < 2) return fail("lh_family_set_sampler: bad dimensions");
  if (!j.left_rows || !j.left_dense || !j.left_lo || !j.left_trans || !j.enter_lo || !j.right_dense || !j.right_first ||
      !j.gene_prob || !j.nti_landing_in || !j.nti_transition || !j.nti_landing_out || !j.landing_in || !j.right_trans ||
      !j.exit_nlo || !j.exit_trans || !j.exit_li || !j.prod)
    return fail("lh_family_set_sampler: null array in descriptor");
  int lo_l = INT32_MAX, hi_l = -1, lo_r = INT32_MAX, hi_r = -1;
  for (size_t l = 0; l < nL; ++l) {
    if (j.left_rows[l] < 0 || j.left_rows[l] > j.n_rows || j.left_dense[l] < 0) return fail("lh_family_set_sampler: bad left gene");
    if (l > 0 && j.left_dense[l] < j.left_dense[l - 1] + j.left_rows[l - 1]) return fail("lh_family_set_sampler: left genes out of order");
    lo_l = std::min(lo_l, j.left_dense[l]);
    hi_l = std::max(hi_l, j.left_dense[l] + j.left_rows[l]);
  }
  for (size_t r = 0; r < nR; ++r) {
    if (j.right_first[r] < 0 || j.right_first[r] > j.n_rows || j.right_dense[r] < 0) return fail("lh_family_set_sampler: bad right gene");
    const int len = 4 + (j.n_rows - j.right_first[r]);
    if (r > 0 && j.right_dense[r] < j.right_dense[r - 1] + 4) return fail("lh_family_set_sampler: right genes out of order");
    lo_r = std::min(lo_r, j.right_dense[r]);
    hi_r = std::max(hi_r, j.right_dense[r] + len);
  }
  if (!(hi_r <= lo_l || hi_l <= lo_r) || std::max(hi_l, hi_r) > j.n_states)
// ... 2549 lines not shown
```

linearham_amd/csrc/lh_device.h:

```cpp
#pragma once
#include <hip/hip_runtime.h>
#include <stdint.h>

#include <functional>

#include "linearham_amd.h"

namespace lh {

constexpr double kScaleFactor = 0x1p256;
constexpr double kScaleThreshold = 0x1p-256;
constexpr double kLogScaleFactor = 177.445678223345993274;

template <class... P, class... A>
static inline void launch_lds(void (*kernel)(P...), dim3 grid, dim3 block, size_t lds, hipStream_t stream,
                              const A&... args) {
  if (lds > 64 * 1024)
    (void)hipFuncSetAttribute(reinterpret_cast<const void*>(kernel), hipFuncAttributeMaxDynamicSharedMemorySize, (int)lds);
  hipLaunchKernelGGL(kernel, grid, block, lds, stream, args...);
}

enum : int { OP_CHERRY = 0, OP_TIP_ACC = 1, OP_POP_ACC = 2, OP_PUSH_FLAG = 16, OP_RANK_SHIFT = 8 };

enum : int { W_CHERRY = 0, W_TIP_ACC = 1, W_POP = 2, W_CTIP = 3, W_CTAB_ACC = 4 };

struct PruneWs {
  double* scratch;
  int2* wops;
  double* wlen;
  int4* tabs;
  int4* hdr;
  int32_t* err_flag;
};
struct PruneWsSizes {
  size_t scratch_doubles_per_rate;
  size_t tabs_per_sample;
};
PruneWsSizes prune_ws_sizes(int T, bool mixed_n);
struct PruneFork {
  hipStream_t sched;
  std::function<int()> join;
};

struct DevSegments {
  int32_t n_genes;
  int32_t n_chunks;
  int32_t cons_sites;
  int32_t cons_diffs;
  const uint16_t* cons_col;
  const uint32_t* cons_rng;
  const uint32_t* cons_dif;
  const uint4* inds_c;
};

struct DevJunction {
  int32_t n_rows, n_left, n_right;
  int32_t left_pad, right_pad;
  const double *enter_lo;
  const double *left_trans;
  const double *left_lo;
  const int32_t* left_xmsa;
  const double *right_gp_nli;
  const double *right_ntt;
  const double *right_nlo;
  const double *right_trans, *right_gp_li;
  const int32_t *right_xmsa;
  const int32_t *nti_xmsa;
  const double *exit_nlo;
  const double *exit_trans, *exit_gp_li;
  const int32_t* row_pat;
};

struct DevFamily {
  int32_t has_d, n_seqs, n_sites, n_xmsa;
  int32_t n_pat;
  int32_t n_prune;
  int32_t msa_mixed_n;
  int32_t n_ucol;
  int32_t idx_byte_offsets;
  const uint8_t* msa;
  const uint64_t* msa_planes;
  const int32_t* site_pat;
  const int32_t* u_pat;
  const uint8_t* u_base;
  const int32_t* ucol_of_col;
  const int32_t* col_of_ucol;
  DevSegments vpadding, vgerm, dgerm, jgerm, jpadding;
  const double *vgerm_gene_prob, *vpadding_transition, *vgerm_trans_prod, *jpadding_transition;
  DevJunction vd, dj;
  int32_t max_genes;
  int32_t n_jcols;
  const int32_t* jcols;
  int64_t gem_size;
  int64_t forward_size;
  int64_t scaler_size;
};

__device__ static inline double fast_rcp(double v) {
  double r = __builtin_amdgcn_rcp(v);
  r = fma(fma(-v, r, 1.0), r, r);
  r = fma(fma(-v, r, 1.0), r, r);
  return r;
}

struct DevSampleJunction {
  int32_t n_rows, n_left, n_right, n_states;
  int32_t right_first_block;
  const int32_t* state_class;
  const int32_t* left_rows;
  const int32_t* left_dense;
  const double* left_lo;
  const double* left_trans;
  const double* enter_lo;
  const int32_t* right_dense;
  const int32_t* right_first;
  const double* gp;
  const double* nli;
  const double* ntt;
  const double* nlo;
  const double* li;
  const double* rtrans;
  const double* exit_nlo;
  const double* exit_trans;
  const double* exit_li;
  const double* prod;
};

struct DevSampler {
  int32_t has_d, n_v, n_d, n_j, states_per_sample, words_per_sample;
  DevSampleJunction vd, dj;
};

void launch_sample(const DevSampler& smp, const DevSampler* smp_dev, int n, const double* fwd, size_t forward_size, const uint32_t* words,
                   int words_per_sample, int32_t* states, hipStream_t stream);

void launch_posterior(const DevSampler* smp_dev, int n, double* post, size_t forward_size, const double* loglik,
                      hipStream_t stream);
int posterior_slabs(int n);
void launch_posterior_reduce(int n, size_t forward_size, const double* post, const double* loglik, const double* log_offset,
                             double* w, double* partial, double* weighted_sum, double* stats, hipStream_t stream);
void launch_slab_sum(int n_slabs, size_t size, const double* partial, double* out, hipStream_t stream);
void launch_weighted_slabs(int n, size_t size, const double* rows, const double* w, double* partial, double* weighted_sum,
                           hipStream_t stream);

struct CodonWindow {
  int32_t npos, top, out;
  int32_t mult[3], ncodes[3], code_off[3];
};
struct CodonTables {
  int32_t n_window, n_genes, n_pos;
  int32_t max_vec;
  const CodonWindow* win;
  const uint8_t* codes;
};
int codon_slots(int n);
void launch_codons(const DevSampler* smp_dev, const CodonTables& t, int n, const double* fwd, size_t forward_size,
                   const double* loglik, double* scratch, double* windows, double* genes, hipStream_t stream);

int events_slots(int n);
size_t events_scratch_doubles(const DevSampler& smp);
void launch_events(const DevSampler& smp, const DevSampler* smp_dev, int n, const double* fwd, const double* post,
                   size_t forward_size, const double* loglik, double* scratch, double* events, size_t events_size,
                   double* genes, hipStream_t stream);

void launch_candidate_indicators(int K, int L, int C, const uint8_t* seqs, const int32_t* col_site, const uint8_t* col_base,
                                 double* em, hipStream_t stream);
struct CandidateTables {
  int32_t K, V, n_lem, n_vlem;
  const uint16_t* idx;
  const double* agree;
  const double* log_prior;
};
int candidate_slabs(int n);
size_t candidate_lds_limit();
void launch_candidates(const CandidateTables& t, int n, const double* lem, const double* loglik, const double* w,
                       double* base, double* log_cand, double* partial, hipStream_t stream);

struct CollectSegments {
  int32_t n_genes, n_chunks;
  const uint4* inds;
};
struct CollectJunction {
  int32_t n_rows, n_left, n_right, left_pad, right_pad, n_states;
  const int32_t *left_xmsa, *right_xmsa, *nti_xmsa;
  const int32_t* state_class;
};
struct CollectTables {
  int32_t L, has_d, states_per_sample, n_cols;
  int32_t seg_scale, seg_sentinel;
  CollectSegments vg, dg, jg;
  CollectJunction vd, dj;
  const int32_t* jcols;
  int32_t n_jcols;
  const int32_t* col_site;
  const uint8_t* col_base;
  uint64_t hash_mask;
};
__host__ __device__ inline uint64_t mix64(uint64_t z) {
  z = (z ^ (z >> 30)) * 0xbf58476d1ce4e5b9ull;
  z = (z ^ (z >> 27)) * 0x94d049bb133111ebull;
  return z ^ (z >> 31);
}
__host__ __device__ inline uint64_t hash_word(uint64_t word, int q) {
  return mix64(word + 0x9e3779b97f4a7c15ull * (uint64_t)(q + 1));
}
__host__ __device__ inline uint64_t hash_finish(uint64_t h, int length) { return mix64(h ^ (uint64_t)length); }

void launch_collect(const CollectTables& t, int n, const int32_t* states, uint8_t* seqs, uint64_t* hash, hipStream_t stream);
size_t collect_lds_bytes(int L);

struct FlatRows {
  int32_t n, L;
  const uint8_t* seqs;
};
__host__ __device__ inline size_t n_slots(const FlatRows& r) { return r.n > 0 ? (size_t)r.n : 0; }
__device__ inline const uint8_t* slot_row(const FlatRows& r, int x) { return r.seqs + (size_t)x * r.L; }

struct LineageBatch {
  int32_t n, T, L, P;
  const uint8_t* anc;
  const uint8_t* naive;
  const int32_t* path;
  uint64_t hash_mask;
// ... 14 lines not shown
void launch_lineage(const LineageBatch& b, uint64_t* nt_hash, uint64_t* aa_hash, hipStream_t stream);

template <class Rows>
void launch_store_verify(const Rows& src, int K, const int32_t* ids, const uint8_t* store, uint8_t* flag,
                         hipStream_t stream);
template <class Rows>
void launch_store_append(const Rows& src, int K, int n_pairs, const int32_t* pairs, uint8_t* store, hipStream_t stream);
template <class Rows>
void launch_store_gather(const Rows& src, int n_out, const int32_t* slots, uint8_t* out, hipStream_t stream);

__device__ static inline void compute_pmatrix(const double* __restrict__ e, double tr, double P[4][4]) {
  double ex[4];
#pragma unroll
  for (int k = 1; k < 4; ++k) ex[k] = expm1(e[k] * tr);
#pragma unroll
  for (int i = 0; i < 4; ++i)
#pragma unroll
    for (int j = 0; j < 4; ++j) {
      double v = (i == j) ? 1.0 : 0.0;
#pragma unroll
      for (int k = 1; k < 4; ++k) v = fma(e[4 + i * 4 + k] * ex[k], e[20 + k * 4 + j], v);
      P[i][j] = fmax(v, 0.0);
    }
}


void launch_model_setup(int n, int R, const double* er, const double* pi, const double* alpha,
                        double* rates, double* eig, hipStream_t stream);

int launch_prune(const DevFamily& fam, int n, int R, int T, int max_depth, const int32_t* ops,
                 const double* brlen, const double* rates, const double* eig, const PruneWs& ws, const double* pi,
                 double* site_lik, int32_t* site_scal, hipStream_t stream, bool allow_fused = true,
                 bool test_every_op = false, const PruneFork* fork = nullptr);
const char* prune_last_form();
const char* prune_last_error();

void launch_gtr_setup(int n, const double* er, const double* pi, double* eig, hipStream_t stream);

int launch_asr(const DevFamily& fam, int n, int R, int T, const int32_t* ops, const double* brlen, const double* rates,
               const double* eig, const double* pi, const double* site_lik, const int32_t* site_scal,
               const uint8_t* naive, uint64_t seed, uint64_t sample0, double* clv, void* desc, uint8_t* anc,
               uint8_t* rate_choice, const int4* hdr , hipStream_t stream,
               int draws = 1);
size_t asr_desc_bytes(int T);
size_t asr_lds_bytes(int T, int L, int R, int n_prune);
size_t asr_slots(int L, int R);

struct AsrOp {
  int4 a, b;
};

void launch_asr_sched(int n, int T, const int32_t* ops, const int4* hdr, void* desc, hipStream_t stream);

struct AncWs {
  double* clv;
  double* part;
  double* tvec;
  double* rho;
  int32_t* chain;
  int32_t* plen;
  void* desc;
};
struct AncWsBytes {
  size_t clv, part, tvec, rho, chain;
  size_t total() const { return clv + part + tvec + rho + chain; }
};
AncWsBytes anc_ws_bytes(int T, int L, int R, int n_prune, int P);
size_t anc_lds_bytes(int T);
int launch_ancestral(const DevFamily& fam, int n, int R, int T, const int32_t* ops, const double* brlen, const double* rates,
                     const double* eig, const double* pi, const double* site_lik, const int32_t* site_scal,
                     const double* naive_prob, const int32_t* path, int P, const AncWs& ws, double* marg, double* rate_post,
                     const int4* hdr, int32_t* err_flag, hipStream_t stream);
void launch_site_base(int n, int L, size_t forward_size, const int32_t* off, const int32_t* idx, const double* post,
                      const double* loglik, double* site_base, hipStream_t stream);
void launch_ancestral_ends(int n, int P, int L, const int32_t* plen, const double* marg, const double* loglik, double* ends,
                           double* ll_used, hipStream_t stream);
void launch_ancestral_front(const DevFamily& fam, int n, int R, int T, const int32_t* ops, const double* pi,
                            const double* site_lik, const int32_t* site_scal, const double* naive_prob, const int32_t* path,
                            int P, const AncWs& ws, double* rate_post, const int4* hdr, int32_t* err_flag, hipStream_t stream);
size_t anc_lp(int n_prune);

void launch_rate_sum(int n, int R, int slots, size_t width, bool last_live, const int32_t* plen, const double* part,
                     double* out, hipStream_t stream);

struct SubWs {
  double* cc;
  double* ne;
  double* se;
  double* el;
  double* edge;
};
struct SubWsBytes {
  size_t cc, ne, se, el, edge;
  size_t total(bool with_edge) const { return cc + ne + se + el + (with_edge ? edge : 0); }
};
SubWsBytes sub_ws_bytes(int L, int R, int P);
size_t sub_lds_bytes(int T, int P);
struct SubOut {
  double *edge, *naive_edge, *chain_counts, *seed_edge, *edge_load, *rate_post;
};
int launch_substitutions(const DevFamily& fam, int n, int R, int T, const int32_t* ops, const double* brlen, const double* rates,
                         const double* eig, const double* pi, const double* site_lik, const int32_t* site_scal,
                         const double* naive_prob, const int32_t* path, int P, int seed_tip, const AncWs& ws, const SubWs& sws,
                         const SubOut& out, const int4* hdr, int32_t* err_flag, hipStream_t stream);

struct CondWsBytes {
  size_t part, table;
};
CondWsBytes cond_ws_bytes(int R, int n_prune);
int launch_ancestral_cond(const DevFamily& fam, int n, int R, int T, const int32_t* ops, const double* brlen,
                          const double* rates, const double* eig, const double* pi, const double* site_lik,
                          const int32_t* site_scal, const double* naive_prob, const int32_t* path, int P, int node,
                          const AncWs& ws, double* table, double* cond, const int4* hdr, int32_t* err_flag,
                          hipStream_t stream);
void launch_row_mask(int n, int C, const int32_t* plen, double* em, hipStream_t stream);
void launch_pair_emissions(const DevFamily& fam, int K, long long q0, int count, const uint8_t* seqs, const int32_t* col_site,
                           const uint8_t* col_base, const int32_t* plen, const double* em, const double* table, double* out,
                           hipStream_t stream);
void launch_pair_finish(int K, long long q0, int count, const double* pair_ll, const double* open_ll, const int32_t* plen,
                        double* log_cand, double* prob, hipStream_t stream);

struct LogEmRequest {
  const int32_t* cols = nullptr;
  int n = 0;
  double* out = nullptr;
};
void launch_forward(const DevFamily& fam, const DevFamily* fam_dev, int n, int R, const double* site_lik,
                    const int32_t* site_scal, const double* pi, const double* em_in, double* em_out, double* gem,
                    int32_t* gcnt, double* jem,
                    int32_t* jrs, double* dxf, int32_t* dxc, double* loglik, double* forward_out, int32_t* scaler_out,
                    bool extended, hipStream_t stream, const LogEmRequest& lem = LogEmRequest{});
size_t forward_lds_bytes(const DevFamily& fam);
const char* forward_last_form();
int forward_last_dj_samples();
int forward_last_dj_waves();

size_t viterbi_bp_bytes(const DevFamily& fam);
size_t viterbi_lds_bytes(const DevFamily& fam);
void launch_viterbi(const DevFamily& fam, const DevSampler* smp_dev, int n, const double* gem, const int32_t* gcnt,
                    const double* jem, const int32_t* jrs, const double* loglik, uint8_t* bp, int32_t* states,
                    double* log_path, bool extended, hipStream_t stream);
void launch_path_prior(const DevFamily& fam, const DevSampler* smp_dev, int K, const int32_t* states, double* log_prior,
                       int32_t* first_bad, hipStream_t stream);

struct DebugOptions {
  int chunk = 49152;
  int host_sub = 12288;
  int eval_split = 0;
  bool k0_serial = false;
  int eval_fwd_priority = -1;
  bool k2b_no_pair = false;
  bool k2b_vd_single = false;
  bool k2b_dj_pair = false;
  bool sample_timing = false;
  bool k4_no_save = false;
  int k1_tile_cap = 0;
  bool k1_cxx_walk = false;
  bool k1_tables = false;
  bool k1_stack = false;
  bool k1_no_tables = false;
  bool k1_segments = false;
  int k1_seg_waves = 4;
  bool k1_no_fuse = false;
  int codon_blocks = 2048;
  int events_blocks = 1024;
  int anc_out_mb = 4096;
  int edge_out_mb = 4096;
  int anc_pairs = 0;
  int collect_hash_bits = 64;
};
const DebugOptions& debug_options();

}
```

linearham_amd/csrc/lh_forward.hip:

```cpp
#include <cstdio>
#include <cstdlib>
#include <type_traits>

#include "lh_device.h"

namespace lh {

constexpr int kFwdThreads = 256;
constexpr int kFwdWaves = kFwdThreads / 64;
constexpr int kJunctionWaves = 4;

thread_local char g_k2a_form[64] = "", g_k2b_form[32] = "", g_forward_form[160] = "";
thread_local int g_k2b_dj_samples = 0;
thread_local int g_k2b_dj_waves = 0;

__device__ static inline int block_max_int(int v, int* red, int phase) {
#pragma unroll
  for (int off = 32; off > 0; off >>= 1) v = max(v, __shfl_xor(v, off, 64));
  int* r = red + phase * kFwdWaves;
  if ((threadIdx.x & 63) == 0) r[threadIdx.x >> 6] = v;
  __syncthreads();
  return max(max(r[0], r[1]), max(r[2], r[3]));
}

// ... 486 lines not shown
      jrs[r] = smin;
    }
  }

  const int nV = fam.vgerm.n_genes, nD = fam.dgerm.n_genes, nJ = fam.jgerm.n_genes;
  double* gem = gem_all + s * fam.gem_size;
  const bool direct = *em_bad != 0;
  auto fill = [&](const DevSegments& seg, double* out, int phase) {
    if constexpr (kExt) return fill_segments_ext<kG, kByteOff>(seg, em, ems, tid, out, redi, phase);
    if (seg.cons_sites > 0 && !direct)
      return fill_consensus<kG, kByteOff>(seg, em, tid, out, redi, phase, cons_inv, cons_pv, cons_pk, cons_cap);
    return fill_segments<kG, kByteOff>(seg, em, tid, out, redi, phase);
  };
  int cv = fill(fam.vpadding, gem, 0);
  cv += fill(fam.vgerm, gem + nV, 1);
  int cd = 0, cj;
  if (small_sets_by_wave(fam, kExt, direct)) {
    const int wave = tid >> 6, lane = tid & 63;
    double* jg = gem + 2 * (size_t)nV + (fam.has_d ? nD : 0);
    int m = 0;
    if (wave == 1 && fam.has_d) m = fill_segments_wave<kByteOff>(fam.dgerm, em, lane, gem + 2 * (size_t)nV);
    if (wave == 2) m = fill_segments_wave<kByteOff>(fam.jgerm, em, lane, jg);
    if (wave == 3) m = fill_segments_wave<kByteOff>(fam.jpadding, em, lane, jg + nJ);
    if (lane == 0) redi[wave] = m;
    __syncthreads();
    cd = redi[1];
    cj = redi[2] + redi[3];
  } else if (fam.has_d) {
    cd = fill(fam.dgerm, gem + 2 * (size_t)nV, 0);
    cj = fill(fam.jgerm, gem + 2 * (size_t)nV + nD, 1);
    cj += fill(fam.jpadding, gem + 2 * (size_t)nV + nD + nJ, 0);
  } else {
    cj = fill(fam.jgerm, gem + 2 * (size_t)nV, 0);
    cj += fill(fam.jpadding, gem + 2 * (size_t)nV + nJ, 1);
  }
  if (tid == 0) {
    gcnt_all[s * 3 + 0] = cv;
    gcnt_all[s * 3 + 1] = cd;
    gcnt_all[s * 3 + 2] = cj;
  }
}


template <int kCtrl>
__device__ static inline double dpp_move(double v) {
  const int lo = __builtin_amdgcn_update_dpp(0, __double2loint(v), kCtrl, 0xf, 0xf, true);
  const int hi = __builtin_amdgcn_update_dpp(0, __double2hiint(v), kCtrl, 0xf, 0xf, true);
  return __hiloint2double(hi, lo);
}

__device__ static inline double read_lane(double v, int lane) {
  return __hiloint2double(__builtin_amdgcn_readlane(__double2hiint(v), lane),
                          __builtin_amdgcn_readlane(__double2loint(v), lane));
}

constexpr int kDppQuadSwap1 = 0xB1;
constexpr int kDppQuadSwap2 = 0x4E;
constexpr int kDppHalfMirror = 0x141;
constexpr int kDppMirror = 0x140;

__device__ static inline double wave_sum(double v) {
  v += dpp_move<kDppQuadSwap1>(v);
  v += dpp_move<kDppQuadSwap2>(v);
  v += dpp_move<kDppHalfMirror>(v);
  v += dpp_move<kDppMirror>(v);
  return (read_lane(v, 0) + read_lane(v, 16)) + (read_lane(v, 32) + read_lane(v, 48));
}

__device__ static inline unsigned scale_key(double v) { return (unsigned)__double2hiint(v) - 1u; }

template <int kCtrl>
__device__ static inline unsigned dpp_min_u32(unsigned v) {
  return min(v, (unsigned)__builtin_amdgcn_update_dpp(0, (int)v, kCtrl, 0xf, 0xf, true));
}

__device__ static inline unsigned wave_min_key(unsigned v) {
  v = dpp_min_u32<kDppQuadSwap1>(v);
  v = dpp_min_u32<kDppQuadSwap2>(v);
  v = dpp_min_u32<kDppHalfMirror>(v);
  v = dpp_min_u32<kDppMirror>(v);
  const unsigned a = __builtin_amdgcn_readlane((int)v, 0), b = __builtin_amdgcn_readlane((int)v, 16);
  const unsigned c = __builtin_amdgcn_readlane((int)v, 32), d = __builtin_amdgcn_readlane((int)v, 48);
  return min(min(a, b), min(c, d));
}

template <int kCtrl>
__device__ static inline unsigned dpp_max_u32(unsigned v) {
  return max(v, (unsigned)__builtin_amdgcn_update_dpp(0, (int)v, kCtrl, 0xf, 0xf, true));
}

__device__ static inline unsigned wave_max_u32(unsigned v) {
  v = dpp_max_u32<kDppQuadSwap1>(v);
  v = dpp_max_u32<kDppQuadSwap2>(v);
  v = dpp_max_u32<kDppHalfMirror>(v);
  v = dpp_max_u32<kDppMirror>(v);
  const unsigned a = __builtin_amdgcn_readlane((int)v, 0), b = __builtin_amdgcn_readlane((int)v, 16);
  const unsigned c = __builtin_amdgcn_readlane((int)v, 32), d = __builtin_amdgcn_readlane((int)v, 48);
  return max(max(a, b), max(c, d));
}

template <bool kExt>
__device__ static inline unsigned key_start() {
  return kExt ? 0u : 0xffffffffu;
}
template <bool kExt>
__device__ static inline unsigned key_add(unsigned key, double v) {
  return kExt ? max(key, (unsigned)__double2hiint(v)) : min(key, scale_key(v));
}

struct RowScale {
  int k;
  double factor;
  bool extra;
  __device__ double apply(double v) const {
    v *= factor;
    if (extra) v *= kScaleFactor;
    return v;
  }
};

__device__ static inline RowScale row_scale(unsigned min_key) {
  const unsigned hw = min_key + 1u;
  const unsigned e = (hw >> 20) & 0x7ffu;
  RowScale s;
  s.extra = hw != 0 && e == 0 && (hw & 0xfffffu) < (1u << 18);
  const int k3 = hw == 0 ? 0 : (e < 767u) + (e < 511u) + (e < 255u);
  s.k = k3 + (s.extra ? 1 : 0);
  s.factor = __hiloint2double((1023 + 256 * k3) << 20, 0);
  return s;
}

template <bool kExt>
__device__ static inline RowScale wave_row_scale(unsigned key) {
  return row_scale(kExt ? wave_max_u32(key) - 1u : wave_min_key(key));
}

__device__ static __forceinline__ RowScale pick(bool hi, const RowScale& sa, const RowScale& sb) {
  return RowScale{hi ? sb.k : sa.k, hi ? sb.factor : sa.factor, hi ? sb.extra : sa.extra};
}

struct RightRow {
  double nlo[4], rtr, rli;
  int ridx;
  int4 nx;
};

template <int GL, int GR>
struct RowTables {
  double ltr[GL], llo[GL];
  int lidx[GL];
  RightRow right[GR];
};

__device__ static __forceinline__ void load_right_row(const DevJunction& J, int i, unsigned r, RightRow& t) {
  const size_t orr = (size_t)i * J.right_pad;
  const double2* pn = reinterpret_cast<const double2*>(J.right_nlo) + 2 * orr;
  const double2 a = pn[2u * r], b = pn[2u * r + 1u];
  t.nlo[0] = a.x;
  t.nlo[1] = a.y;
  t.nlo[2] = b.x;
  t.nlo[3] = b.y;
  t.nx = (reinterpret_cast<const int4*>(J.nti_xmsa) + orr)[r];
  t.rtr = (J.right_trans + orr)[r];
  t.rli = (J.right_gp_li + orr)[r];
  t.ridx = (J.right_xmsa + orr)[r];
}

template <int GL, int GR>
__device__ static inline void load_row(const DevJunction& J, int i, unsigned lane, RowTables<GL, GR>& t) {
  const size_t ol = (size_t)i * J.left_pad;
  const double* lt = J.left_trans + ol;
  const double* ll = J.left_lo + ol;
  const int32_t* lx = J.left_xmsa + ol;
#pragma unroll
  for (int q = 0; q < GL; ++q) {
    t.ltr[q] = lt[lane + 64u * q];
    t.llo[q] = ll[lane + 64u * q];
    t.lidx[q] = lx[lane + 64u * q];
  }
#pragma unroll
  for (int q = 0; q < GR; ++q) load_right_row(J, i, lane + 64u * q, t.right[q]);
}


__device__ static __forceinline__ void load_nli(const DevJunction& J, unsigned r, double (&nli)[4]) {
  const double2* p = reinterpret_cast<const double2*>(J.right_gp_nli) + 2u * r;
  const double2 a = p[0], b = p[1];
  nli[0] = a.x, nli[1] = a.y, nli[2] = b.x, nli[3] = b.y;
}

template <bool kExt>
__device__ static __forceinline__ unsigned right_gene_step(unsigned key, double (&fN)[4], double& fR, double A,
                                                           const double (&nli)[4], const double* ntt_lds, unsigned r,
                                                           const RightRow& t, const double* jem) {
  const double n0 = fN[0], n1 = fN[1], n2 = fN[2], n3 = fN[3];
  const double2* tt = reinterpret_cast<const double2*>(ntt_lds) + 8u * r;
  const int nxs[4] = {t.nx.x, t.nx.y, t.nx.z, t.nx.w};
#pragma unroll
  for (int b = 0; b < 4; ++b) {
    const double2 t01 = tt[2 * b], t23 = tt[2 * b + 1];
    double s = ((n0 * t01.x + n1 * t01.y) + n2 * t23.x) + n3 * t23.y;
    s += A * nli[b];
    fN[b] = s * jem[nxs[b]];
  }
  double s = ((n0 * t.nlo[0] + n1 * t.nlo[1]) + n2 * t.nlo[2]) + n3 * t.nlo[3];
  s += fR * t.rtr;
  s += A * t.rli;
  fR = s * jem[t.ridx];
#pragma unroll
  for (int b = 0; b < 4; ++b) key = key_add<kExt>(key, fN[b]);
  return key_add<kExt>(key, fR);
}

__device__ static __forceinline__ double exit_handoff(const DevJunction& J, unsigned r, int nR, const double (&fN)[4],
                                                      double fR, double A, const double* __restrict__ germ_em,
                                                      const double* __restrict__ pad_trans,
                                                      const double* __restrict__ pad_em) {
  const double2* xn = reinterpret_cast<const double2*>(J.exit_nlo) + 2u * r;
  const double2 x01 = xn[0], x23 = xn[1];
  double s = ((fN[0] * x01.x + fN[1] * x01.y) + fN[2] * x23.x) + fN[3] * x23.y;
  s += fR * J.exit_trans[r];
  s += A * J.exit_gp_li[r];
  double v = 0.0;
  if ((int)r < nR) {
    v = s * germ_em[r];
    if (pad_trans) v *= pad_trans[r];
    if (pad_em) v *= pad_em[r];
  }
  return v;
}

__device__ static __forceinline__ void store_right(double* __restrict__ o, int nL, int nR, unsigned r,
                                                   const double (&fN)[4], double fR) {
  if ((int)r < nR) {
    o[nL + 4 * (size_t)r + 0] = fN[0];
    o[nL + 4 * (size_t)r + 1] = fN[1];
    o[nL + 4 * (size_t)r + 2] = fN[2];
    o[nL + 4 * (size_t)r + 3] = fN[3];
    o[nL + 4 * (size_t)nR + r] = fR;
  }
}

__device__ static __forceinline__ size_t junction_fwd_size(const DevJunction& J) {
  return (size_t)J.n_rows * (J.n_left + 5 * (size_t)J.n_right);
}

template <int GL, int GR, bool kExt>
__device__ static int junction_wave(const DevJunction& J, const double* jem, const double* ntt_lds, int lane,
                                    const double (&f_in)[GL], int count_in, const double* __restrict__ germ_em,
                                    const double* __restrict__ pad_trans, const double* __restrict__ pad_em,
                                    double (&g_out)[GR], double* __restrict__ fwd_out,
                                    int32_t* __restrict__ scal_out, const int32_t* __restrict__ jrs) {
  const int W = J.n_rows, nL = J.n_left, nR = J.n_right;
  int count = count_in;
  double fL[GL], fN[GR][4], fR[GR];
  double nli[GR][4];
#pragma unroll
  for (int q = 0; q < GL; ++q) fL[q] = f_in[q];
#pragma unroll
  for (int q = 0; q < GR; ++q) {
    fR[q] = 0.0;
    fN[q][0] = fN[q][1] = fN[q][2] = fN[q][3] = 0.0;
    load_nli(J, lane + 64u * q, nli[q]);
  }
  const size_t row_stride = (size_t)nL + 5 * (size_t)nR;
  double A;
  {
    double part = 0.0;
#pragma unroll
    for (int q = 0; q < GL; ++q) part += f_in[q] * J.enter_lo[lane + 64u * q];
    A = wave_sum(part);
  }

  auto step = [&](int i, const RowTables<GL, GR>& t) __attribute__((always_inline)) {
    unsigned key = key_start<kExt>();
    double part = 0.0;
#pragma unroll
    for (int q = 0; q < GL; ++q) {
      const double v = (fL[q] * t.ltr[q]) * jem[t.lidx[q]];
      fL[q] = v;
      key = key_add<kExt>(key, v);
      part += v * t.llo[q];
    }
#pragma unroll
    for (int q = 0; q < GR; ++q)
      key = right_gene_step<kExt>(key, fN[q], fR[q], A, nli[q], ntt_lds, lane + 64u * q, t.right[q], jem);
    A = wave_sum(part);
    const RowScale sc = wave_row_scale<kExt>(key);
    if constexpr (kExt) count += jrs[i];
    if (sc.k != 0) {
      A = sc.apply(A);
#pragma unroll
      for (int q = 0; q < GL; ++q) fL[q] = sc.apply(fL[q]);
#pragma unroll
      for (int q = 0; q < GR; ++q) {
        fR[q] = sc.apply(fR[q]);
#pragma unroll
        for (int b = 0; b < 4; ++b) fN[q][b] = sc.apply(fN[q][b]);
      }
      count += sc.k;
    }
    if (fwd_out) {
      double* o = fwd_out + (size_t)i * row_stride;
#pragma unroll
      for (int q = 0; q < GL; ++q) {
        const int g = lane + 64 * q;
        if (g < nL) o[g] = fL[q];
      }
#pragma unroll
      for (int q = 0; q < GR; ++q) store_right(o, nL, nR, lane + 64u * q, fN[q], fR[q]);
    }
    if (scal_out && lane == 0) scal_out[i] = count;
  };

  for (int i = 0; i < W; ++i) {
    RowTables<GL, GR> t;
    load_row<GL, GR>(J, i, lane, t);
    step(i, t);
  }

  unsigned key = key_start<kExt>();
#pragma unroll
  for (int q = 0; q < GR; ++q) {
    const double v = exit_handoff(J, lane + 64u * q, nR, fN[q], fR[q], A, germ_em, pad_trans, pad_em);
    key = key_add<kExt>(key, v);
    g_out[q] = v;
  }
  const RowScale last = wave_row_scale<kExt>(key);
#pragma unroll
  for (int q = 0; q < GR; ++q) g_out[q] = last.apply(g_out[q]);
  return count + last.k;
}


struct HalfPair {
  double a, b;
};

__device__ static inline HalfPair half_sums(double v) {
  v += dpp_move<kDppQuadSwap1>(v);
  v += dpp_move<kDppQuadSwap2>(v);
  v += dpp_move<kDppHalfMirror>(v);
  v += dpp_move<kDppMirror>(v);
  return HalfPair{read_lane(v, 0) + read_lane(v, 16), read_lane(v, 32) + read_lane(v, 48)};
}

struct HalfKeys {
  unsigned a, b;
};

template <bool kExt>
__device__ static inline HalfKeys half_keys(unsigned v) {
  if (kExt) {
    v = dpp_max_u32<kDppQuadSwap1>(v);
    v = dpp_max_u32<kDppQuadSwap2>(v);
    v = dpp_max_u32<kDppHalfMirror>(v);
    v = dpp_max_u32<kDppMirror>(v);
  } else {
    v = dpp_min_u32<kDppQuadSwap1>(v);
    v = dpp_min_u32<kDppQuadSwap2>(v);
    v = dpp_min_u32<kDppHalfMirror>(v);
    v = dpp_min_u32<kDppMirror>(v);
  }
  const unsigned a = __builtin_amdgcn_readlane((int)v, 0), b = __builtin_amdgcn_readlane((int)v, 16);
  const unsigned c = __builtin_amdgcn_readlane((int)v, 32), d = __builtin_amdgcn_readlane((int)v, 48);
  return kExt ? HalfKeys{max(a, b) - 1u, max(c, d) - 1u} : HalfKeys{min(a, b), min(c, d)};
}

template <bool kExt>
__device__ static int junction_pair(const DevJunction& J, const double* jem, const double* ntt_lds, int lane, bool hi,
                                    double f_in, int count_in, const double* __restrict__ germ_em,
                                    const double* __restrict__ pad_trans, const double* __restrict__ pad_em,
                                    double& g_out, double* __restrict__ fwd_out, int32_t* __restrict__ scal_out,
                                    const int32_t* __restrict__ jrs, bool valid) {
  const int W = J.n_rows, nL = J.n_left, nR = J.n_right;
  const unsigned g = lane & 31;
  int count = count_in;
  double fL = f_in, fR = 0.0, fN[4] = {0.0, 0.0, 0.0, 0.0}, nli[4];
  load_nli(J, g, nli);
  const size_t row_stride = (size_t)nL + 5 * (size_t)nR;
  auto mine = [&](const HalfPair& p) { return hi ? p.b : p.a; };
  double A = mine(half_sums(f_in * J.enter_lo[g]));
  for (int i = 0; i < W; ++i) {
    const size_t ol = (size_t)i * J.left_pad;
    const double ltr = J.left_trans[ol + g], llo = J.left_lo[ol + g];
    const int lidx = J.left_xmsa[ol + g];
    RightRow t;
    load_right_row(J, i, g, t);

    unsigned key = key_start<kExt>();
    {
      const double v = (fL * ltr) * jem[lidx];
      fL = v;
      key = key_add<kExt>(key, v);
    }
    const double part = fL * llo;
    key = right_gene_step<kExt>(key, fN, fR, A, nli, ntt_lds, g, t, jem);
    A = mine(half_sums(part));
    const HalfKeys hk = half_keys<kExt>(key);
    const RowScale sa = row_scale(hk.a), sb = row_scale(hk.b);
    if constexpr (kExt) count += jrs[i];
    if ((sa.k | sb.k) != 0) {
      const RowScale sc = pick(hi, sa, sb);
      A = sc.apply(A);
      fL = sc.apply(fL);
      fR = sc.apply(fR);
#pragma unroll
      for (int b = 0; b < 4; ++b) fN[b] = sc.apply(fN[b]);
      count += sc.k;
    }
    if (fwd_out && valid) {
      double* o = fwd_out + (size_t)i * row_stride;
      if ((int)g < nL) o[g] = fL;
      store_right(o, nL, nR, g, fN, fR);
    }
    if (scal_out && valid && g == 0) scal_out[i] = count;
  }
  g_out = exit_handoff(J, g, nR, fN, fR, A, germ_em, pad_trans, pad_em);
  const HalfKeys hk = half_keys<kExt>(key_add<kExt>(key_start<kExt>(), g_out));
  const RowScale last = pick(hi, row_scale(hk.a), row_scale(hk.b));
  g_out = last.apply(g_out);
  return count + last.k;
}

template <int GL, bool kExt>
__device__ static void junction_vd_pair(const DevJunction& J, const double* jemA, const double* jemB,
                                        const double* ntt_lds, int lane, bool hi, const double (&fA_in)[GL],
                                        const double (&fB_in)[GL], int countA_in, int countB_in,
                                        const double* __restrict__ germ_em_mine, double& g_out, int& count_mine,
                                        double* __restrict__ fwdA, double* __restrict__ fwdB,
                                        int32_t* __restrict__ scoA, int32_t* __restrict__ scoB,
                                        const int32_t* __restrict__ jrsA, const int32_t* __restrict__ jrsB) {
  const int W = J.n_rows, nL = J.n_left, nR = J.n_right;
  const unsigned g = lane & 31;
  const double* jemM = hi ? jemB : jemA;
  int countA = countA_in, countB = countB_in;
  double fA[GL], fB[GL], fN[4] = {0.0, 0.0, 0.0, 0.0}, fR = 0.0, nli[4];
#pragma unroll
  for (int q = 0; q < GL; ++q) {
    fA[q] = fA_in[q];
    fB[q] = fB_in[q];
  }
  load_nli(J, g, nli);
  const size_t row_stride = (size_t)nL + 5 * (size_t)nR;
  double AA, AB;
  {
    double pa = 0.0, pb = 0.0;
#pragma unroll
    for (int q = 0; q < GL; ++q) {
      const double lo = J.enter_lo[lane + 64u * q];
      pa += fA_in[q] * lo;
      pb += fB_in[q] * lo;
    }
    AA = wave_sum(pa);
    AB = wave_sum(pb);
  }
  auto combine = [](unsigned a, unsigned b) { return kExt ? max(a, b) : min(a, b); };
  for (int i = 0; i < W; ++i) {
    const size_t ol = (size_t)i * J.left_pad;
    unsigned keyA = key_start<kExt>(), keyB = key_start<kExt>();
    double partA = 0.0, partB = 0.0;
    {
      const double* lt = J.left_trans + ol;
      const double* ll = J.left_lo + ol;
      const int32_t* lx = J.left_xmsa + ol;
#pragma unroll
      for (int q = 0; q < GL; ++q) {
        const double ltr = lt[lane + 64u * q], llo = ll[lane + 64u * q];
        const int lidx = lx[lane + 64u * q];
        const double va = (fA[q] * ltr) * jemA[lidx];
        const double vb = (fB[q] * ltr) * jemB[lidx];
        fA[q] = va;
        fB[q] = vb;
        keyA = key_add<kExt>(keyA, va);
        keyB = key_add<kExt>(keyB, vb);
        partA += va * llo;
        partB += vb * llo;
      }
    }
    {
      RightRow t;
      load_right_row(J, i, g, t);
      const unsigned keyR = right_gene_step<kExt>(key_start<kExt>(), fN, fR, hi ? AB : AA, nli, ntt_lds, g, t, jemM);
      if (hi)
        keyB = combine(keyB, keyR);
      else
        keyA = combine(keyA, keyR);
    }
    AA = wave_sum(partA);
    AB = wave_sum(partB);
    const RowScale sa = wave_row_scale<kExt>(keyA), sb = wave_row_scale<kExt>(keyB);
    if constexpr (kExt) {
      countA += jrsA[i];
      countB += jrsB[i];
    }
    if ((sa.k | sb.k) != 0) {
      AA = sa.apply(AA);
      AB = sb.apply(AB);
#pragma unroll
      for (int q = 0; q < GL; ++q) {
        fA[q] = sa.apply(fA[q]);
        fB[q] = sb.apply(fB[q]);
      }
      const RowScale sm = pick(hi, sa, sb);
      fR = sm.apply(fR);
#pragma unroll
      for (int b = 0; b < 4; ++b) fN[b] = sm.apply(fN[b]);
      countA += sa.k;
      countB += sb.k;
    }
    if (fwdA) {
      double* oa = fwdA + (size_t)i * row_stride;
      double* ob = fwdB ? fwdB + (size_t)i * row_stride : nullptr;
#pragma unroll
      for (int q = 0; q < GL; ++q) {
        const int t = lane + 64 * q;
        if (t < nL) {
          oa[t] = fA[q];
          if (ob) ob[t] = fB[q];
        }
      }
      double* om = hi ? ob : oa;
      if (om) store_right(om, nL, nR, g, fN, fR);
    }
    if (lane == 0) {
      if (scoA) scoA[i] = countA;
      if (scoB) scoB[i] = countB;
    }
  }
  g_out = exit_handoff(J, g, nR, fN, fR, hi ? AB : AA, germ_em_mine, nullptr, nullptr);
  const HalfKeys hk = half_keys<kExt>(key_add<kExt>(key_start<kExt>(), g_out));
  const RowScale last = pick(hi, row_scale(hk.a), row_scale(hk.b));
  g_out = last.apply(g_out);
  count_mine = (hi ? countB : countA) + last.k;
}


__device__ static __forceinline__ void stage_ntt(double* dst, const double* __restrict__ src, int count, int threads) {
  for (int t = threadIdx.x; t < count; t += threads) dst[t] = src[t];
}

template <int kSamples>
__device__ static __forceinline__ void stage_jem(double* jem0, const double* __restrict__ jem_all, int first, int n,
                                                 int NJ, int lane) {
  for (int h = 0; h < kSamples; ++h) {
    const double* src = jem_all + (size_t)min(first + h, n - 1) * NJ;
    double* dst = jem0 + (size_t)h * (NJ + 1);
    for (int j = lane; j < NJ; j += 64) dst[j] = src[j];
    if (lane == 0) dst[NJ] = 0.0;
  }
  __builtin_amdgcn_fence(__ATOMIC_RELEASE, "wavefront");
  __builtin_amdgcn_wave_barrier();
  __builtin_amdgcn_fence(__ATOMIC_ACQUIRE, "wavefront");
}

template <int GA, bool kExt>
__device__ static __forceinline__ int initial_v_forward(const DevFamily& fam, const double* __restrict__ gem, int lane,
                                                        int cv, double (&gV)[GA], double* __restrict__ fwd,
                                                        int32_t* __restrict__ sco) {
  const int nV = fam.vgerm.n_genes;
  unsigned key = key_start<kExt>();
#pragma unroll
  for (int q = 0; q < GA; ++q) {
    const int t = lane + 64 * q;
    double v = 0.0;
    if (t < nV) {
      v = fam.vgerm_gene_prob[t];
      v *= fam.vpadding_transition[t];
      v *= gem[t];
      v *= fam.vgerm_trans_prod[t];
      v *= gem[nV + t];
    }
    key = key_add<kExt>(key, v);
    gV[q] = v;
  }
  const RowScale sc = wave_row_scale<kExt>(key);
#pragma unroll
  for (int q = 0; q < GA; ++q) gV[q] = sc.apply(gV[q]);
  const int vcount = cv + sc.k;
  if (fwd) {
#pragma unroll
    for (int q = 0; q < GA; ++q)
      if (lane + 64 * q < nV) fwd[lane + 64 * q] = gV[q];
  }
  if (sco && lane == 0) sco[0] = vcount;
  return vcount;
}

template <int GA, bool kExt>
__global__ void __launch_bounds__(64 * kJunctionWaves)
    junction_vd_kernel(const DevFamily fam, int n, const double* __restrict__ gem_all,
                       const int32_t* __restrict__ gcnt_all, const double* __restrict__ jem_all,
                       const int32_t* __restrict__ jrs_all, double* __restrict__ fwd_all,
                       int32_t* __restrict__ scal_all, double* __restrict__ dxf, int32_t* __restrict__ dxc) {
  extern __shared__ double jlds[];
  const int lane = threadIdx.x & 63, wave = threadIdx.x >> 6;
  const int s = blockIdx.x * kJunctionWaves + wave;
  const int NJ = fam.n_jcols;
  double* ntt_vd = jlds;
  double* jem = ntt_vd + 16 * (size_t)fam.vd.right_pad + (size_t)wave * (NJ + 1);
  stage_ntt(ntt_vd, fam.vd.right_ntt, 16 * fam.vd.right_pad, 64 * kJunctionWaves);
  __syncthreads();
  if (s >= n) return;
  const int nV = fam.vgerm.n_genes, nD = fam.dgerm.n_genes;
  const size_t vd_fwd = junction_fwd_size(fam.vd);
  stage_jem<1>(jem, jem_all, s, n, NJ, lane);
  const double* gem = gem_all + (size_t)s * fam.gem_size;
  const int cv = gcnt_all[(size_t)s * 3 + 0], cd = gcnt_all[(size_t)s * 3 + 1];
  double* fwd = fwd_all ? fwd_all + (size_t)s * fam.forward_size : nullptr;
  int32_t* sco = scal_all ? scal_all + (size_t)s * fam.scaler_size : nullptr;
  double gV[GA];
  const int vcount = initial_v_forward<GA, kExt>(fam, gem, lane, cv, gV, fwd, sco);
  double gD[1];
  const int dcount =
      cd + junction_wave<GA, 1, kExt>(fam.vd, jem, ntt_vd, lane, gV, vcount, gem + 2 * (size_t)nV, nullptr, nullptr, gD,
                                      fwd ? fwd + nV : nullptr, sco ? sco + 1 : nullptr,
                                      kExt ? jrs_all + (size_t)s * (fam.vd.n_rows + fam.dj.n_rows) : nullptr);
  if (fwd && lane < nD) fwd[nV + vd_fwd + lane] = gD[0];
  if (sco && lane == 0) sco[1 + fam.vd.n_rows] = dcount;
  if (lane < 32) dxf[(size_t)s * 32 + lane] = gD[0];
  if (lane == 0) dxc[s] = dcount;
}

constexpr int kVdPairWaves = 4;
template <int GA, bool kExt>
__global__ void __launch_bounds__(64 * kVdPairWaves)
    junction_vd2_kernel(const DevFamily fam, int n, const double* __restrict__ gem_all,
                        const int32_t* __restrict__ gcnt_all, const double* __restrict__ jem_all,
                        const int32_t* __restrict__ jrs_all, double* __restrict__ fwd_all,
                        int32_t* __restrict__ scal_all, double* __restrict__ dxf, int32_t* __restrict__ dxc) {
  extern __shared__ double jlds[];
  const int lane = threadIdx.x & 63, wave = threadIdx.x >> 6;
  const int NJ = fam.n_jcols;
  double* ntt_vd = jlds;
  double* jem0 = ntt_vd + 16 * (size_t)fam.vd.right_pad + (size_t)(2 * wave) * (NJ + 1);
  stage_ntt(ntt_vd, fam.vd.right_ntt, 16 * fam.vd.right_pad, 64 * kVdPairWaves);
  __syncthreads();
  const int p = blockIdx.x * kVdPairWaves + wave;
  if (2 * p >= n) return;
  const bool hi = lane >= 32;
  const int sA = 2 * p, sB = min(2 * p + 1, n - 1);
  const bool validB = 2 * p + 1 < n;
  stage_jem<2>(jem0, jem_all, sA, n, NJ, lane);
  const int nV = fam.vgerm.n_genes, nD = fam.dgerm.n_genes;
  const size_t vd_fwd = junction_fwd_size(fam.vd);
  const double* gemA = gem_all + (size_t)sA * fam.gem_size;
  const double* gemB = gem_all + (size_t)sB * fam.gem_size;
  double* fwdA = fwd_all ? fwd_all + (size_t)sA * fam.forward_size : nullptr;
  double* fwdB = fwd_all && validB ? fwd_all + (size_t)sB * fam.forward_size : nullptr;
  int32_t* scoA = scal_all ? scal_all + (size_t)sA * fam.scaler_size : nullptr;
  int32_t* scoB = scal_all && validB ? scal_all + (size_t)sB * fam.scaler_size : nullptr;
  double gA[GA], gB[GA];
  unsigned keyA = key_start<kExt>(), keyB = key_start<kExt>();
#pragma unroll
  for (int q = 0; q < GA; ++q) {
    const int t = lane + 64 * q;
    double va = 0.0, vb = 0.0;
    if (t < nV) {
      const double c0 = fam.vgerm_gene_prob[t], c1 = fam.vpadding_transition[t], c2 = fam.vgerm_trans_prod[t];
      va = c0;
      va *= c1;
      va *= gemA[t];
      va *= c2;
      va *= gemA[nV + t];
      vb = c0;
      vb *= c1;
      vb *= gemB[t];
      vb *= c2;
      vb *= gemB[nV + t];
    }
    keyA = key_add<kExt>(keyA, va);
    keyB = key_add<kExt>(keyB, vb);
    gA[q] = va;
    gB[q] = vb;
  }
  int countA = gcnt_all[(size_t)sA * 3 + 0], countB = gcnt_all[(size_t)sB * 3 + 0];
  {
    const RowScale sa = wave_row_scale<kExt>(keyA), sb = wave_row_scale<kExt>(keyB);
#pragma unroll
    for (int q = 0; q < GA; ++q) {
      gA[q] = sa.apply(gA[q]);
      gB[q] = sb.apply(gB[q]);
    }
    countA += sa.k;
    countB += sb.k;
  }
  if (fwdA) {
#pragma unroll
    for (int q = 0; q < GA; ++q)
      if (lane + 64 * q < nV) {
        fwdA[lane + 64 * q] = gA[q];
        if (fwdB) fwdB[lane + 64 * q] = gB[q];
      }
  }
  if (lane == 0) {
    if (scoA) scoA[0] = countA;
    if (scoB) scoB[0] = countB;
  }
  const size_t jr = (size_t)fam.vd.n_rows + fam.dj.n_rows;
  double gD;
  int count_mine;
  junction_vd_pair<GA, kExt>(fam.vd, jem0, jem0 + (NJ + 1), ntt_vd, lane, hi, gA, gB, countA, countB,
                             (hi ? gemB : gemA) + 2 * (size_t)nV, gD, count_mine, fwdA ? fwdA + nV : nullptr,
                             fwdB ? fwdB + nV : nullptr, scoA ? scoA + 1 : nullptr, scoB ? scoB + 1 : nullptr,
                             kExt ? jrs_all + (size_t)sA * jr : nullptr, kExt ? jrs_all + (size_t)sB * jr : nullptr);
  const unsigned g = lane & 31;
  const int dcount = gcnt_all[(size_t)(hi ? sB : sA) * 3 + 1] + count_mine;
  if (!hi || validB) {
    const int sM = hi ? sB : sA;
    double* fwdM = hi ? fwdB : fwdA;
    int32_t* scoM = hi ? scoB : scoA;
    if (fwdM && (int)g < nD) fwdM[nV + vd_fwd + g] = gD;
    if (scoM && g == 0) scoM[1 + fam.vd.n_rows] = dcount;
    dxf[(size_t)sM * 32 + g] = gD;
    if (g == 0) dxc[sM] = dcount;
  }
}

constexpr int kPairWaves = 4;

struct DjSample {
  const double *jgerm_em, *jpad_em;
  int cj;
  double* fwd;
  int32_t* sco;
  const int32_t* jrs;
};

template <bool kExt>
__device__ static __forceinline__ DjSample dj_sample(const DevFamily& fam, int s, const double* __restrict__ gem_all,
                                                     const int32_t* __restrict__ gcnt_all,
                                                     const int32_t* __restrict__ jrs_all, double* __restrict__ fwd_all,
                                                     int32_t* __restrict__ scal_all) {
  const int nV = fam.vgerm.n_genes, nD = fam.dgerm.n_genes, nJ = fam.jgerm.n_genes;
  DjSample d;
  d.jgerm_em = gem_all + (size_t)s * fam.gem_size + 2 * (size_t)nV + nD;
  d.jpad_em = d.jgerm_em + nJ;
  d.cj = gcnt_all[(size_t)s * 3 + 2];
  d.fwd = fwd_all ? fwd_all + (size_t)s * fam.forward_size + nV + junction_fwd_size(fam.vd) + nD : nullptr;
  d.sco = scal_all ? scal_all + (size_t)s * fam.scaler_size + 2 + fam.vd.n_rows : nullptr;
  d.jrs = kExt ? jrs_all + (size_t)s * (fam.vd.n_rows + fam.dj.n_rows) + fam.vd.n_rows : nullptr;
  return d;
}

template <class Total>
__device__ static __forceinline__ void dj_finish(const DevFamily& fam, const DjSample& d, int s, bool valid, unsigned g,
                                                 double gJ, int jcount, Total&& total, double* __restrict__ loglik) {
  if (d.fwd && valid && (int)g < fam.jgerm.n_genes) d.fwd[junction_fwd_size(fam.dj) + g] = gJ;
  if (d.sco && valid && g == 0) d.sco[fam.dj.n_rows] = jcount;
  const double part = total();
  if (valid && g == 0) loglik[s] = log(part) - jcount * kLogScaleFactor;
}

template <bool kExt>
__global__ void __launch_bounds__(64 * kPairWaves)
    junction_dj_kernel(const DevFamily fam, int n, const double* __restrict__ gem_all,
                       const int32_t* __restrict__ gcnt_all, const double* __restrict__ jem_all,
                       const int32_t* __restrict__ jrs_all, const double* __restrict__ dxf,
                       const int32_t* __restrict__ dxc, double* __restrict__ loglik, double* __restrict__ fwd_all,
                       int32_t* __restrict__ scal_all) {
  extern __shared__ double jlds[];
  const int lane = threadIdx.x & 63, wave = threadIdx.x >> 6;
  const int NJ = fam.n_jcols;
  double* ntt_dj = jlds;
  double* jem0 = ntt_dj + 16 * (size_t)fam.dj.right_pad + (size_t)(2 * wave) * (NJ + 1);
  stage_ntt(ntt_dj, fam.dj.right_ntt, 16 * fam.dj.right_pad, 64 * kPairWaves);
  __syncthreads();
  const int p = blockIdx.x * kPairWaves + wave;
  if (2 * p >= n) return;
  const bool hi = lane >= 32;
  const int s2 = 2 * p + (hi ? 1 : 0);
  const bool valid = s2 < n;
  const int sr = valid ? s2 : n - 1;
  stage_jem<2>(jem0, jem_all, 2 * p, n, NJ, lane);
  const unsigned g = lane & 31;
  const DjSample d = dj_sample<kExt>(fam, sr, gem_all, gcnt_all, jrs_all, fwd_all, scal_all);
  const double f_in = valid ? dxf[(size_t)s2 * 32 + g] : 0.0;
  const int dcount = valid ? dxc[s2] : 0;
  double gJ;
  const int jcount = d.cj + junction_pair<kExt>(fam.dj, jem0 + (size_t)(hi ? 1 : 0) * (NJ + 1), ntt_dj, lane, hi, f_in,
                                                dcount, d.jgerm_em, fam.jpadding_transition, d.jpad_em, gJ, d.fwd,
                                                d.sco, d.jrs, valid);
  dj_finish(fam, d, s2, valid, g, gJ, jcount, [&] {
    const HalfPair tot = half_sums(gJ);
    return hi ? tot.b : tot.a;
  }, loglik);
}

constexpr int kDppRowFirst = 0x150;

__device__ static inline double row_tree_sum(double v) {
  v += dpp_move<kDppQuadSwap1>(v);
  v += dpp_move<kDppQuadSwap2>(v);
  v += dpp_move<kDppHalfMirror>(v);
  v += dpp_move<kDppMirror>(v);
  return v;
}

template <int GL>
__device__ static inline double row_sums(const double (&p)[GL]) {
  double t = row_tree_sum(p[0]);
  if constexpr (GL == 2)
    t = t + row_tree_sum(p[1]);
  else
    t = t + 0.0;
  return dpp_move<kDppRowFirst>(t);
}

template <bool kExt>
__device__ static inline unsigned row_key(unsigned v) {
  if (kExt) {
    v = dpp_max_u32<kDppQuadSwap1>(v);
    v = dpp_max_u32<kDppQuadSwap2>(v);
    v = dpp_max_u32<kDppHalfMirror>(v);
    v = dpp_max_u32<kDppMirror>(v);
    return v - 1u;
  }
  v = dpp_min_u32<kDppQuadSwap1>(v);
  v = dpp_min_u32<kDppQuadSwap2>(v);
  v = dpp_min_u32<kDppHalfMirror>(v);
  v = dpp_min_u32<kDppMirror>(v);
  return v;
}

constexpr unsigned kRescaleKeyEnd = (767u << 20) - 1u;

template <int GL, bool kExt>
__device__ static int junction_quad(const DevJunction& J, const double* jem, const double* ntt_lds, unsigned l,
                                    const double (&f_in)[GL], int count_in, const double* __restrict__ germ_em,
                                    const double* __restrict__ pad_trans, const double* __restrict__ pad_em,
                                    double& g_out, double* __restrict__ fwd_out, int32_t* __restrict__ scal_out,
                                    const int32_t* __restrict__ jrs, bool valid) {
  const int W = J.n_rows, nL = J.n_left, nR = J.n_right;
  int count = count_in;
  double fL[GL], fR = 0.0, fN[4] = {0.0, 0.0, 0.0, 0.0}, nli[4];
#pragma unroll
  for (int q = 0; q < GL; ++q) fL[q] = f_in[q];
  load_nli(J, l, nli);
  const size_t row_stride = (size_t)nL + 5 * (size_t)nR;
  double A;
  {
    double part[GL];
#pragma unroll
    for (int q = 0; q < GL; ++q) part[q] = f_in[q] * J.enter_lo[l + 16u * q];
    A = row_sums<GL>(part);
  }
  for (int i = 0; i < W; ++i) {
    const size_t ol = (size_t)i * J.left_pad;
    double ltr[GL], llo[GL];
    int lidx[GL];
#pragma unroll
    for (int q = 0; q < GL; ++q) {
      ltr[q] = J.left_trans[ol + l + 16u * q];
      llo[q] = J.left_lo[ol + l + 16u * q];
      lidx[q] = J.left_xmsa[ol + l + 16u * q];
    }
    RightRow t;
    load_right_row(J, i, l, t);

    unsigned key = key_start<kExt>();
    double part[GL];
#pragma unroll
    for (int q = 0; q < GL; ++q) {
      const double v = (fL[q] * ltr[q]) * jem[lidx[q]];
      fL[q] = v;
      key = key_add<kExt>(key, v);
      part[q] = fL[q] * llo[q];
    }
    key = right_gene_step<kExt>(key, fN, fR, A, nli, ntt_lds, l, t, jem);
    A = row_sums<GL>(part);
    const unsigned rk = row_key<kExt>(key);
    if constexpr (kExt) count += jrs[i];
    if (__builtin_amdgcn_ballot_w64(rk < kRescaleKeyEnd) != 0) {
      const RowScale sc = row_scale(rk);
      A = sc.apply(A);
#pragma unroll
      for (int q = 0; q < GL; ++q) fL[q] = sc.apply(fL[q]);
      fR = sc.apply(fR);
#pragma unroll
      for (int b = 0; b < 4; ++b) fN[b] = sc.apply(fN[b]);
      count += sc.k;
    }
    if (fwd_out && valid) {
      double* o = fwd_out + (size_t)i * row_stride;
#pragma unroll
      for (int q = 0; q < GL; ++q)
        if ((int)(l + 16u * q) < nL) o[l + 16u * q] = fL[q];
      store_right(o, nL, nR, l, fN, fR);
    }
    if (scal_out && valid && l == 0) scal_out[i] = count;
  }
  g_out = exit_handoff(J, l, nR, fN, fR, A, germ_em, pad_trans, pad_em);
  const RowScale last = row_scale(row_key<kExt>(key_add<kExt>(key_start<kExt>(), g_out)));
  g_out = last.apply(g_out);
  return count + last.k;
}

template <int GL, bool kExt>
__global__ void __launch_bounds__(1024)
    junction_dj4_kernel(const DevFamily fam, int n, const double* __restrict__ gem_all,
                        const int32_t* __restrict__ gcnt_all, const double* __restrict__ jem_all,
                        const int32_t* __restrict__ jrs_all, const double* __restrict__ dxf,
                        const int32_t* __restrict__ dxc, double* __restrict__ loglik, double* __restrict__ fwd_all,
                        int32_t* __restrict__ scal_all) {
  extern __shared__ double jlds[];
  const int lane = threadIdx.x & 63, wave = threadIdx.x >> 6, waves = blockDim.x >> 6;
  const int NJ = fam.n_jcols;
  double* ntt_dj = jlds;
  double* jem0 = ntt_dj + 16 * 16 + (size_t)(4 * wave) * (NJ + 1);
  stage_ntt(ntt_dj, fam.dj.right_ntt, 16 * 16, blockDim.x);
  __syncthreads();
  const int p = blockIdx.x * waves + wave;
  if (4 * p >= n) return;
  const int sub = lane >> 4;
  const unsigned l = lane & 15;
  const int s4 = 4 * p + sub;
  const bool valid = s4 < n;
  const int sr = valid ? s4 : n - 1;
  stage_jem<4>(jem0, jem_all, 4 * p, n, NJ, lane);
  const DjSample d = dj_sample<kExt>(fam, sr, gem_all, gcnt_all, jrs_all, fwd_all, scal_all);
  double f_in[GL];
#pragma unroll
  for (int q = 0; q < GL; ++q) f_in[q] = valid ? dxf[(size_t)s4 * 32 + l + 16u * q] : 0.0;
  const int dcount = valid ? dxc[s4] : 0;
  double gJ;
  const int jcount = d.cj + junction_quad<GL, kExt>(fam.dj, jem0 + (size_t)sub * (NJ + 1), ntt_dj, l, f_in, dcount,
                                                    d.jgerm_em, fam.jpadding_transition, d.jpad_em, gJ, d.fwd, d.sco,
                                                    d.jrs, valid);
  dj_finish(fam, d, s4, valid, l, gJ, jcount, [&] { return row_sums<1>({gJ}); }, loglik);
}

template <int GA, int GB, bool kExt = false>
__global__ void __launch_bounds__(64 * kJunctionWaves)
    junction_kernel(const DevFamily fam, int n, const double* __restrict__ gem_all,
                    const int32_t* __restrict__ gcnt_all, const double* __restrict__ jem_all,
                    const int32_t* __restrict__ jrs_all, double* __restrict__ loglik, double* __restrict__ fwd_all,
                    int32_t* __restrict__ scal_all) {
  extern __shared__ double jlds[];
  const int lane = threadIdx.x & 63, wave = threadIdx.x >> 6;
  const int s = blockIdx.x * kJunctionWaves + wave;
  const int NJ = fam.n_jcols;
  double* ntt_vd = jlds;
  double* ntt_dj = ntt_vd + 16 * (size_t)fam.vd.right_pad;
  double* jem = ntt_dj + (fam.has_d ? 16 * (size_t)fam.dj.right_pad : 0) + (size_t)wave * (NJ + 1);
  stage_ntt(ntt_vd, fam.vd.right_ntt, 16 * fam.vd.right_pad, 64 * kJunctionWaves);
  if (fam.has_d) stage_ntt(ntt_dj, fam.dj.right_ntt, 16 * fam.dj.right_pad, 64 * kJunctionWaves);
  __syncthreads();
  if (s >= n) return;
  stage_jem<1>(jem, jem_all, s, n, NJ, lane);

  const int nV = fam.vgerm.n_genes, nD = fam.dgerm.n_genes, nJ = fam.jgerm.n_genes;
  const double* gem = gem_all + (size_t)s * fam.gem_size;
  const int cv = gcnt_all[(size_t)s * 3 + 0], cd = gcnt_all[(size_t)s * 3 + 1], cj = gcnt_all[(size_t)s * 3 + 2];
  double* fwd = fwd_all ? fwd_all + (size_t)s * fam.forward_size : nullptr;
  int32_t* sco = scal_all ? scal_all + (size_t)s * fam.scaler_size : nullptr;

  double gV[GA];
  const int vcount = initial_v_forward<GA, kExt>(fam, gem, lane, cv, gV, fwd, sco);
  const int32_t* jrs = kExt ? jrs_all + (size_t)s * (fam.vd.n_rows + (fam.has_d ? fam.dj.n_rows : 0)) : nullptr;
  if (fwd) fwd += nV;
  if (sco) sco += 1;

  double gJ[GB];
  int jcount;
  if (fam.has_d) {
    double gD[GB];
    const double* dgerm_em = gem + 2 * (size_t)nV;
    const double* jgerm_em = dgerm_em + nD;
    const double* jpad_em = jgerm_em + nJ;
    const int dcount = cd + junction_wave<GA, GB, kExt>(fam.vd, jem, ntt_vd, lane, gV, vcount, dgerm_em, nullptr,
                                                        nullptr, gD, fwd, sco, jrs);
    if (fwd) {
      fwd += junction_fwd_size(fam.vd);
#pragma unroll
      for (int q = 0; q < GB; ++q)
        if (lane + 64 * q < nD) fwd[lane + 64 * q] = gD[q];
      fwd += nD;
    }
    if (sco) {
      sco += fam.vd.n_rows;
      if (lane == 0) sco[0] = dcount;
      sco += 1;
    }
    jcount = cj + junction_wave<GB, GB, kExt>(fam.dj, jem, ntt_dj, lane, gD, dcount, jgerm_em,
                                              fam.jpadding_transition, jpad_em, gJ, fwd, sco,
                                              kExt ? jrs + fam.vd.n_rows : nullptr);
    if (fwd) fwd += junction_fwd_size(fam.dj);
    if (sco) sco += fam.dj.n_rows;
  } else {
    const double* jgerm_em = gem + 2 * (size_t)nV;
    const double* jpad_em = jgerm_em + nJ;
    jcount = cj + junction_wave<GA, GB, kExt>(fam.vd, jem, ntt_vd, lane, gV, vcount, jgerm_em,
                                              fam.jpadding_transition, jpad_em, gJ, fwd, sco, jrs);
    if (fwd) fwd += junction_fwd_size(fam.vd);
    if (sco) sco += fam.vd.n_rows;
  }
  if (fwd) {
#pragma unroll
    for (int q = 0; q < GB; ++q)
      if (lane + 64 * q < nJ) fwd[lane + 64 * q] = gJ[q];
  }
  if (sco && lane == 0) sco[0] = jcount;

  double part = 0.0;
#pragma unroll
  for (int q = 0; q < GB; ++q) part += gJ[q];
  part = wave_sum(part);
  if (lane == 0) loglik[s] = log(part) - jcount * kLogScaleFactor;
}

static size_t junction_lds_bytes(const DevFamily& fam) {
  return ((size_t)2 * kJunctionWaves * (fam.n_jcols + 1) +
          16 * ((size_t)fam.vd.right_pad + (fam.has_d ? fam.dj.right_pad : 0))) *
         sizeof(double);
}

static bool junction_pair_form(const DevFamily& fam) {
  static const bool off = debug_options().k2b_no_pair;
  return !off && fam.has_d && fam.dgerm.n_genes <= 32 && fam.jgerm.n_genes <= 32;
}

static size_t dj4_lds_bytes(const DevFamily& fam, int waves) {
  return ((size_t)4 * waves * (fam.n_jcols + 1) + 16 * 16) * sizeof(double);
}

static int dj4_waves(const DevFamily& fam, size_t lds_pair) {
  static const bool pair = debug_options().k2b_dj_pair;
  if (pair || fam.jgerm.n_genes > 16 || fam.dgerm.n_genes > 32) return 0;
  constexpr size_t kCuLds = 160 * 1024;
  auto per_simd = [](size_t lds, int waves) { return std::min<size_t>(4, lds > kCuLds ? 0 : kCuLds / lds * waves / 4); };
  const size_t need = per_simd(lds_pair, kPairWaves);
  for (int waves = 4; waves <= 16; waves *= 2)
    if (per_simd(dj4_lds_bytes(fam, waves), waves) >= need && need > 0) return waves;
  return 0;
}

static size_t emission_lds_bytes(const DevFamily& fam, bool ext) {
  const size_t cap = (size_t)cons_capacity(fam);
  return ((((size_t)fam.n_ucol + 2) & ~(size_t)1) + 6) * sizeof(double) + (2 * kFwdWaves + 2) * sizeof(int) +
         (cap ? (2 * cap + 4) * sizeof(double) + (cap + 4) * sizeof(int) : 0) +
         (ext ? ((size_t)fam.n_ucol + 2) * sizeof(int) : 0);
}

size_t forward_lds_bytes(const DevFamily& fam) {
  const size_t a = emission_lds_bytes(fam, true), b = junction_lds_bytes(fam);
  return a > b ? a : b;
}

template <class F>
static void with_bool(bool b, F&& f) {
  if (b)
    f(std::true_type{});
  else
    f(std::false_type{});
}
template <int N>
using slots_c = std::integral_constant<int, N>;

template <int kG, bool kSite, bool kByteOff, bool kExt, bool kLem>
static void launch_emission_l(const DevFamily& fam, const DevFamily* fam_dev, int n, int R, const double* site_lik,
                              const int32_t* site_scal, const double* pi, const double* em_in, double* em_out,
                              double* gem, int32_t* gcnt, double* jem, int32_t* jrs, const LogEmRequest& lem,
                              hipStream_t stream) {
  const size_t lds = emission_lds_bytes(fam, kExt);
  snprintf(g_k2a_form, sizeof(g_k2a_form), "emission<%d,%s,%s%s%s>", kG, kSite ? "site" : "caller",
           kByteOff ? "byte" : "index", kExt ? ",ext" : "", kLem ? ",lem" : "");
  launch_lds(emission_kernel<kG, kSite, kByteOff, kExt, kLem>, dim3(n), dim3(kFwdThreads), lds, stream, fam_dev, R,
             site_lik, site_scal, pi, em_in, em_out, gem, gcnt, jem, jrs, lem.cols, lem.n, lem.out);
}

template <int kG, bool kSite, bool kByteOff, bool kExt>
static void launch_emission_k(const DevFamily& fam, const DevFamily* fam_dev, int n, int R, const double* site_lik,
                              const int32_t* site_scal, const double* pi, const double* em_in, double* em_out,
                              double* gem, int32_t* gcnt, double* jem, int32_t* jrs, const LogEmRequest& lem,
                              hipStream_t stream) {
  if constexpr (kSite) {
    if (lem.out) {
      launch_emission_l<kG, kSite, kByteOff, kExt, true>(fam, fam_dev, n, R, site_lik, site_scal, pi, em_in, em_out, gem,
                                                         gcnt, jem, jrs, lem, stream);
      return;
    }
  }
  launch_emission_l<kG, kSite, kByteOff, kExt, false>(fam, fam_dev, n, R, site_lik, site_scal, pi, em_in, em_out, gem, gcnt,
                                                      jem, jrs, lem, stream);
}

template <int kG>
static void launch_emission_g(const DevFamily& fam, const DevFamily* fam_dev, int n, int R, const double* site_lik,
                              const int32_t* site_scal, const double* pi, const double* em_in, double* em_out,
                              double* gem, int32_t* gcnt, double* jem, int32_t* jrs, bool ext, const LogEmRequest& lem,
                              hipStream_t stream) {
  with_bool(site_lik != nullptr, [&](auto S) {
    with_bool(fam.idx_byte_offsets != 0, [&](auto B) {
      with_bool(ext, [&](auto E) {
        launch_emission_k<kG, decltype(S)::value, decltype(B)::value, decltype(E)::value>(
            fam, fam_dev, n, R, site_lik, site_scal, pi, em_in, em_out, gem, gcnt, jem, jrs, lem, stream);
      });
    });
  });
}

template <bool kExt>
static void launch_dj(const DevFamily& fam, int n, const double* gem, const int32_t* gcnt, const double* jem,
                      const int32_t* jrs, const double* dxf, const int32_t* dxc, double* loglik, double* forward_out,
                      int32_t* scaler_out, hipStream_t stream) {
  const size_t lds_dj = ((size_t)2 * kPairWaves * (fam.n_jcols + 1) + 16 * (size_t)fam.dj.right_pad) * sizeof(double);
  const int waves = dj4_waves(fam, lds_dj);
  g_k2b_dj_samples = waves == 0 ? 2 : 4;
  g_k2b_dj_waves = waves == 0 ? kPairWaves : waves;
  auto kernel = junction_dj_kernel<kExt>;
  size_t lds = lds_dj;
  dim3 grid(((n + 1) / 2 + kPairWaves - 1) / kPairWaves), block(64 * kPairWaves);
  if (waves != 0) {
    kernel = fam.dgerm.n_genes <= 16 ? junction_dj4_kernel<1, kExt> : junction_dj4_kernel<2, kExt>;
    lds = dj4_lds_bytes(fam, waves);
    grid = dim3(((n + 3) / 4 + waves - 1) / waves);
    block = dim3(64 * waves);
  }
  launch_lds(kernel, grid, block, lds, stream, fam, n, gem, gcnt, jem, jrs, dxf, dxc, loglik, forward_out, scaler_out);
}

template <int GA, int GB>
static void launch_junction_g(const DevFamily& fam, int n, const double* gem, const int32_t* gcnt, const double* jem,
                              const int32_t* jrs, double* dxf, int32_t* dxc, double* loglik, double* forward_out,
                              int32_t* scaler_out, bool ext, hipStream_t stream) {
  g_k2b_dj_samples = g_k2b_dj_waves = 0;
  if constexpr (GB == 1) {
    if (junction_pair_form(fam)) {
      const size_t jem_slice = (size_t)fam.n_jcols + 1, ntt_vd = 16 * (size_t)fam.vd.right_pad;
      bool vd2 = false;
      if constexpr (GA <= 4) {
        static const bool vd_single = debug_options().k2b_vd_single;
        vd2 = !vd_single;
      }
      snprintf(g_k2b_form, sizeof(g_k2b_form), vd2 ? "vd2<%d>+dj" : "vd<%d>+dj", GA);
      with_bool(ext, [&](auto E) {
        constexpr bool kE = decltype(E)::value;
        if constexpr (GA <= 4) {
          if (vd2)
            launch_lds(junction_vd2_kernel<GA, kE>, dim3(((n + 1) / 2 + kVdPairWaves - 1) / kVdPairWaves),
                       dim3(64 * kVdPairWaves), (2 * kVdPairWaves * jem_slice + ntt_vd) * sizeof(double), stream, fam, n,
                       gem, gcnt, jem, jrs, forward_out, scaler_out, dxf, dxc);
        }
        if (!vd2)
          launch_lds(junction_vd_kernel<GA, kE>, dim3((n + kJunctionWaves - 1) / kJunctionWaves),
                     dim3(64 * kJunctionWaves), (kJunctionWaves * jem_slice + ntt_vd) * sizeof(double), stream, fam, n,
                     gem, gcnt, jem, jrs, forward_out, scaler_out, dxf, dxc);
        launch_dj<kE>(fam, n, gem, gcnt, jem, jrs, dxf, dxc, loglik, forward_out, scaler_out, stream);
      });
      return;
    }
  }
  snprintf(g_k2b_form, sizeof(g_k2b_form), "junction<%d,%d>", GA, GB);
  with_bool(ext, [&](auto E) {
    launch_lds(junction_kernel<GA, GB, decltype(E)::value>, dim3((n + kJunctionWaves - 1) / kJunctionWaves),
               dim3(64 * kJunctionWaves), junction_lds_bytes(fam), stream, fam, n, gem, gcnt, jem, jrs, loglik,
               forward_out, scaler_out);
  });
}

template <int GA>
static void launch_junction_a(int gb, const DevFamily& fam, int n, const double* gem, const int32_t* gcnt,
                              const double* jem, const int32_t* jrs, double* dxf, int32_t* dxc, double* loglik,
                              double* forward_out, int32_t* scaler_out, bool ext, hipStream_t stream) {
  if (gb <= 1)
    launch_junction_g<GA, 1>(fam, n, gem, gcnt, jem, jrs, dxf, dxc, loglik, forward_out, scaler_out, ext, stream);
  else if (gb <= 2)
    launch_junction_g<GA, 2>(fam, n, gem, gcnt, jem, jrs, dxf, dxc, loglik, forward_out, scaler_out, ext, stream);
  else
    launch_junction_g<GA, 4>(fam, n, gem, gcnt, jem, jrs, dxf, dxc, loglik, forward_out, scaler_out, ext, stream);
}

void launch_forward(const DevFamily& fam, const DevFamily* fam_dev, int n, int R, const double* site_lik,
                    const int32_t* site_scal, const double* pi, const double* em_in, double* em_out, double* gem,
                    int32_t* gcnt, double* jem, int32_t* jrs, double* dxf, int32_t* dxc, double* loglik,
                    double* forward_out, int32_t* scaler_out, bool ext, hipStream_t stream, const LogEmRequest& lem) {
  const int slots = (fam.max_genes + kFwdThreads - 1) / kFwdThreads;
  auto emission = [&](auto G) {
    launch_emission_g<decltype(G)::value>(fam, fam_dev, n, R, site_lik, site_scal, pi, em_in, em_out, gem, gcnt, jem, jrs,
                                          ext, lem, stream);
  };
  if (slots <= 1)
    emission(slots_c<1>{});
  else if (slots <= 2)
    emission(slots_c<2>{});
  else
    emission(slots_c<4>{});
  const int ga = (fam.vgerm.n_genes + 63) / 64;
  const int gb = (std::max(fam.dgerm.n_genes, fam.jgerm.n_genes) + 63) / 64;
  auto junction = [&](auto G) {
    launch_junction_a<decltype(G)::value>(gb, fam, n, gem, gcnt, jem, jrs, dxf, dxc, loglik, forward_out, scaler_out, ext,
                                          stream);
  };
  if (ga <= 1)
    junction(slots_c<1>{});
  else if (ga <= 2)
    junction(slots_c<2>{});
  else if (ga <= 4)
    junction(slots_c<4>{});
  else if (ga <= 8)
    junction(slots_c<8>{});
  else
    junction(slots_c<16>{});
  const int cons = ext ? 0
                       : (fam.vpadding.cons_sites > 0) | (fam.vgerm.cons_sites > 0) << 1 | (fam.dgerm.cons_sites > 0) << 2 |
                             (fam.jgerm.cons_sites > 0) << 3 | (fam.jpadding.cons_sites > 0) << 4;
  snprintf(g_forward_form, sizeof(g_forward_form), "%s cons=%d small=%s | %s", g_k2a_form, cons,
           small_sets_by_wave(fam, ext, false) ? "wave" : "block", g_k2b_form);
}

const char* forward_last_form() { return g_forward_form; }
int forward_last_dj_samples() { return g_k2b_dj_samples; }
int forward_last_dj_waves() { return g_k2b_dj_waves; }

}
```

Before: 8.749 million.

## Split junction row sweep into phases that skip dead left/right-germline rows

At upload time the host finds the last row where the left-gene tables are non-zero and the first row where the right-germline tables are non-zero. Junction kernels now sweep rows in up to four compile-time phases, and each phase leaves out the left-gene loads and maths or the right-germline loads and maths where those tables are all zero. The goal is less memory traffic and arithmetic per row in the junction forward pass. It costs extra code-path specialisation and register pressure, and the phasing is switched off for the VD wave path, the pair path and the extended GL==2 quad path.

Measured after the change: 8.683 million (median of 2 runs). No clear change (-0.8%).

```diff
diff --git a/include/linearham_amd.h b/include/linearham_amd.h
--- a/include/linearham_amd.h
+++ b/include/linearham_amd.h
@@ -89,6 +89,8 @@
 
 int lh_family_forward_dj_waves(const lh_family* fam);
 
+int lh_family_forward_row_phases(const lh_family* fam, int junction, int32_t* left_live_rows, int32_t* right_first_row);
+
 int lh_family_set_extended_range(lh_family* fam, int enable);
 
 typedef struct {
diff --git a/linearham_amd/capi.py b/linearham_amd/capi.py
--- a/linearham_amd/capi.py
+++ b/linearham_amd/capi.py
@@ -45,7 +45,7 @@
            "lh_profile_enable", "lh_profile_read", "lh_asr_profile_read", "lh_family_set_extended_range", "lh_warmup", "lh_host_alloc", "lh_host_free", "lh_family_set_sampler",
            "lh_sample_words", "lh_sample_states", "lh_eval_sample_batch", "lh_set_device", "lh_family_status",
            "lh_eval_sample_batch_device", "lh_family_prune_form", "lh_family_forward_form",
-           "lh_family_forward_dj_samples", "lh_family_forward_dj_waves"]
+           "lh_family_forward_dj_samples", "lh_family_forward_dj_waves", "lh_family_forward_row_phases"]
 CRAFTED_EXPORTS = ["lh_sample_forward_batch", "lh_posterior_forward_batch"]
 EXPORTS += CRAFTED_EXPORTS
 POSTERIOR_EXPORTS = ["lh_eval_posterior_batch", "lh_eval_posterior_batch_device", "lh_posterior_profile_read"]
@@ -230,6 +230,9 @@
         if hasattr(lib, "lh_family_forward_dj_waves"):
             lib.lh_family_forward_dj_waves.argtypes = [C.c_void_p]
             lib.lh_family_forward_dj_waves.restype = C.c_int
+        if hasattr(lib, "lh_family_forward_row_phases"):
+            lib.lh_family_forward_row_phases.argtypes = [C.c_void_p, C.c_int, C.POINTER(C.c_int32), C.POINTER(C.c_int32)]
+            lib.lh_family_forward_row_phases.restype = C.c_int
         lib.lh_schedule_tree.argtypes = [C.c_int32, c_i32p, C.c_int32, c_i32p, c_i32p]
         lib.lh_eval_batch.argtypes = _HOST_TREE + [c_f64p, C.POINTER(_EvalOutputs)]
         lib.lh_eval_batch_device.argtypes = _DEV_TREE + [C.c_void_p, C.POINTER(_EvalOutputs), C.c_void_p]
@@ -948,6 +951,11 @@
     def k2_dj_waves(self):
         return int(self.hip.lib.lh_family_forward_dj_waves(self.handle))
 
+    def k2_row_phases(self, junction):
+        a, b = C.c_int32(), C.c_int32()
+        self.hip.check(self.hip.lib.lh_family_forward_row_phases(self.handle, junction, C.byref(a), C.byref(b)))
+        return a.value, b.value
+
     def status(self):
         self.hip.check(self.hip.lib.lh_family_status(self.handle))
 
diff --git a/linearham_amd/csrc/lh_capi.hip b/linearham_amd/csrc/lh_capi.hip
--- a/linearham_amd/csrc/lh_capi.hip
+++ b/linearham_amd/csrc/lh_capi.hip
@@ -27,6 +27,7 @@
     o.k2b_no_pair = set("LH_K2B_NO_PAIR");
     o.k2b_vd_single = set("LH_K2B_VD_SINGLE");
     o.k2b_dj_pair = set("LH_K2B_DJ_PAIR");
+    o.k2b_full_rows = set("LH_K2B_FULL_ROWS");
     o.sample_timing = set("LH_SAMPLE_TIMING");
     o.k4_no_save = set("LH_K4_NO_SAVE");
     o.k1_tile_cap = num("LH_K1_TILE_CAP", 0);
@@ -633,19 +634,33 @@
   };
   std::vector<double> ltr = pad_genes<double>(j.left_trans, W, nL, pL, 1, 0.0);
   for (size_t l = 0; l < nL; ++l) ltr[l] = j.enter_trans[l];
+  const std::vector<double> llo = pad_genes<double>(j.left_lo, W, nL, pL, 1, 0.0),
+                            nlo = pad_genes<double>(j.right_nlo, W, nR, pR, 4, 0.0),
+                            rtr = pad_genes<double>(j.right_trans, W, nR, pR, 1, 0.0),
+                            rli = pad_genes<double>(j.right_gp_li, W, nR, pR, 1, 0.0);
+  auto row_alive = [](const std::vector<double>& t, size_t i, size_t stride) {
+    return std::any_of(t.begin() + i * stride, t.begin() + (i + 1) * stride, [](double x) { return !(x == 0.0); });
+  };
+  d->left_live_rows = 0;
+  d->right_first_row = j.n_rows;
+  for (size_t i = 0; i < W; ++i) {
+    if (row_alive(ltr, i, pL) || row_alive(llo, i, pL)) d->left_live_rows = (int32_t)i + 1;
+    if (d->right_first_row == j.n_rows && (row_alive(nlo, i, 4 * pR) || row_alive(rtr, i, pR) || row_alive(rli, i, pR)))
+      d->right_first_row = (int32_t)i;
+  }
   std::vector<double> ntt(pR * 16, 0.0);
   for (size_t r = 0; r < nR; ++r)
     for (int a = 0; a < 4; ++a)
       for (int b = 0; b < 4; ++b) ntt[r * 16 + b * 4 + a] = j.right_ntt[r * 16 + a * 4 + b];
   if (upload_vec(f, pad_genes<double>(j.enter_lo, 1, nL, pL, 1, 0.0), &d->enter_lo)) return 1;
   if (upload_vec(f, ltr, &d->left_trans)) return 1;
-  if (upload_vec(f, pad_genes<double>(j.left_lo, W, nL, pL, 1, 0.0), &d->left_lo)) return 1;
+  if (upload_vec(f, llo, &d->left_lo)) return 1;
   if (upload_vec(f, cols(j.left_xmsa, W, nL, pL, 1), &d->left_xmsa)) return 1;
   if (upload_vec(f, pad_genes<double>(j.right_gp_nli, 1, nR, pR, 4, 0.0), &d->right_gp_nli)) return 1;
   if (upload_vec(f, ntt, &d->right_ntt)) return 1;
-  if (upload_vec(f, pad_genes<double>(j.right_nlo, W, nR, pR, 4, 0.0), &d->right_nlo)) return 1;
-  if (upload_vec(f, pad_genes<double>(j.right_trans, W, nR, pR, 1, 0.0), &d->right_trans)) return 1;
-  if (upload_vec(f, pad_genes<double>(j.right_gp_li, W, nR, pR, 1, 0.0), &d->right_gp_li)) return 1;
+  if (upload_vec(f, nlo, &d->right_nlo)) return 1;
+  if (upload_vec(f, rtr, &d->right_trans)) return 1;
+  if (upload_vec(f, rli, &d->right_gp_li)) return 1;
   if (upload_vec(f, cols(j.right_xmsa, W, nR, pR, 1), &d->right_xmsa)) return 1;
   if (upload_vec(f, cols(j.nti_xmsa, W, nR, pR, 4), &d->nti_xmsa)) return 1;
   if (upload_vec(f, pad_genes<double>(j.exit_nlo, 1, nR, pR, 4, 0.0), &d->exit_nlo)) return 1;
@@ -1265,6 +1280,15 @@
 int lh_family_forward_dj_samples(const lh_family* f) { return f ? f->k2_dj_samples : 0; }
 int lh_family_forward_dj_waves(const lh_family* f) { return f ? f->k2_dj_waves : 0; }
 
+int lh_family_forward_row_phases(const lh_family* f, int junction, int32_t* left_live_rows, int32_t* right_first_row) {
+  if (!f || !left_live_rows || !right_first_row) return fail("lh_family_forward_row_phases: null argument");
+  if (junction < 0 || junction > (f->host.has_d ? 1 : 0)) return fail("lh_family_forward_row_phases: no such junction");
+  const lh::DevJunction& d = junction == 0 ? f->host.vd : f->host.dj;
+  *left_live_rows = d.left_live_rows;
+  *right_first_row = d.right_first_row;
+  return 0;
+}
+
 int lh_family_consensus_sets(const lh_family* f) {
   if (!f) return 0;
   const lh::DevFamily& h = f->host;
diff --git a/linearham_amd/csrc/lh_device.h b/linearham_amd/csrc/lh_device.h
--- a/linearham_amd/csrc/lh_device.h
+++ b/linearham_amd/csrc/lh_device.h
@@ -69,6 +69,8 @@
   const double *exit_nlo;
   const double *exit_trans, *exit_gp_li;
   const int32_t* row_pat;
+  int32_t left_live_rows;
+  int32_t right_first_row;
 };
 
 struct DevFamily {
@@ -389,6 +391,7 @@
   bool k2b_no_pair = false;
   bool k2b_vd_single = false;
   bool k2b_dj_pair = false;
+  bool k2b_full_rows = false;
   bool sample_timing = false;
   bool k4_no_save = false;
   int k1_tile_cap = 0;
diff --git a/linearham_amd/csrc/lh_forward.hip b/linearham_amd/csrc/lh_forward.hip
--- a/linearham_amd/csrc/lh_forward.hip
+++ b/linearham_amd/csrc/lh_forward.hip
@@ -662,34 +662,63 @@
   RightRow right[GR];
 };
 
+template <bool kGerm = true>
 __device__ static __forceinline__ void load_right_row(const DevJunction& J, int i, unsigned r, RightRow& t) {
   const size_t orr = (size_t)i * J.right_pad;
-  const double2* pn = reinterpret_cast<const double2*>(J.right_nlo) + 2 * orr;
-  const double2 a = pn[2u * r], b = pn[2u * r + 1u];
-  t.nlo[0] = a.x;
-  t.nlo[1] = a.y;
-  t.nlo[2] = b.x;
-  t.nlo[3] = b.y;
   t.nx = (reinterpret_cast<const int4*>(J.nti_xmsa) + orr)[r];
-  t.rtr = (J.right_trans + orr)[r];
-  t.rli = (J.right_gp_li + orr)[r];
-  t.ridx = (J.right_xmsa + orr)[r];
-}
-
-template <int GL, int GR>
+  if constexpr (kGerm) {
+    const double2* pn = reinterpret_cast<const double2*>(J.right_nlo) + 2 * orr;
+    const double2 a = pn[2u * r], b = pn[2u * r + 1u];
+    t.nlo[0] = a.x;
+    t.nlo[1] = a.y;
+    t.nlo[2] = b.x;
+    t.nlo[3] = b.y;
+    t.rtr = (J.right_trans + orr)[r];
+    t.rli = (J.right_gp_li + orr)[r];
+    t.ridx = (J.right_xmsa + orr)[r];
+  }
+}
+
+template <int GL, int GR, bool kLeft, bool kGerm>
 __device__ static inline void load_row(const DevJunction& J, int i, unsigned lane, RowTables<GL, GR>& t) {
-  const size_t ol = (size_t)i * J.left_pad;
-  const double* lt = J.left_trans + ol;
-  const double* ll = J.left_lo + ol;
-  const int32_t* lx = J.left_xmsa + ol;
-#pragma unroll
-  for (int q = 0; q < GL; ++q) {
-    t.ltr[q] = lt[lane + 64u * q];
-    t.llo[q] = ll[lane + 64u * q];
-    t.lidx[q] = lx[lane + 64u * q];
-  }
-#pragma unroll
-  for (int q = 0; q < GR; ++q) load_right_row(J, i, lane + 64u * q, t.right[q]);
+  if constexpr (kLeft) {
+    const size_t ol = (size_t)i * J.left_pad;
+    const double* lt = J.left_trans + ol;
+    const double* ll = J.left_lo + ol;
+    const int32_t* lx = J.left_xmsa + ol;
+#pragma unroll
+    for (int q = 0; q < GL; ++q) {
+      t.ltr[q] = lt[lane + 64u * q];
+      t.llo[q] = ll[lane + 64u * q];
+      t.lidx[q] = lx[lane + 64u * q];
+    }
+  }
+#pragma unroll
+  for (int q = 0; q < GR; ++q) load_right_row<kGerm>(J, i, lane + 64u * q, t.right[q]);
+}
+
+template <bool kLeft, bool kGerm>
+struct RowPhase {
+  static constexpr bool left = kLeft, germ = kGerm;
+};
+
+template <bool kPhased = true, class Row, class LeftEnd>
+__device__ static __forceinline__ void sweep_rows(const DevJunction& J, Row&& row, LeftEnd&& left_end) {
+  const int W = J.n_rows;
+  const int a = kPhased ? J.left_live_rows : W, b = kPhased ? J.right_first_row : 0;
+  int i = 0;
+  if constexpr (!kPhased) {
+    for (; i < W; ++i) row(i, RowPhase<true, true>{});
+    return;
+  }
+  auto run = [&](int end, auto phase) __attribute__((always_inline)) {
+    for (; i < end; ++i) row(i, phase);
+  };
+  run(min(min(a, b), W), RowPhase<true, false>{});
+  run(min(a, W), RowPhase<true, true>{});
+  if (i < W) left_end();
+  run(min(b, W), RowPhase<false, false>{});
+  run(W, RowPhase<false, true>{});
 }
 
 
@@ -699,7 +728,7 @@
   nli[0] = a.x, nli[1] = a.y, nli[2] = b.x, nli[3] = b.y;
 }
 
-template <bool kExt>
+template <bool kExt, bool kGerm = true>
 __device__ static __forceinline__ unsigned right_gene_step(unsigned key, double (&fN)[4], double& fR, double A,
                                                            const double (&nli)[4], const double* ntt_lds, unsigned r,
                                                            const RightRow& t, const double* jem) {
@@ -713,13 +742,17 @@
     s += A * nli[b];
     fN[b] = s * jem[nxs[b]];
   }
-  double s = ((n0 * t.nlo[0] + n1 * t.nlo[1]) + n2 * t.nlo[2]) + n3 * t.nlo[3];
-  s += fR * t.rtr;
-  s += A * t.rli;
-  fR = s * jem[t.ridx];
+  if constexpr (kGerm) {
+    double s = ((n0 * t.nlo[0] + n1 * t.nlo[1]) + n2 * t.nlo[2]) + n3 * t.nlo[3];
+    s += fR * t.rtr;
+    s += A * t.rli;
+    fR = s * jem[t.ridx];
+  } else {
+    fR = fN[0] * 0.0;
+  }
 #pragma unroll
   for (int b = 0; b < 4; ++b) key = key_add<kExt>(key, fN[b]);
-  return key_add<kExt>(key, fR);
+  return kGerm ? key_add<kExt>(key, fR) : key;
 }
 
 __device__ static __forceinline__ double exit_handoff(const DevJunction& J, unsigned r, int nR, const double (&fN)[4],
@@ -755,13 +788,13 @@
   return (size_t)J.n_rows * (J.n_left + 5 * (size_t)J.n_right);
 }
 
-template <int GL, int GR, bool kExt>
+template <int GL, int GR, bool kExt, bool kPhased = true>
 __device__ static int junction_wave(const DevJunction& J, const double* jem, const double* ntt_lds, int lane,
                                     const double (&f_in)[GL], int count_in, const double* __restrict__ germ_em,
                                     const double* __restrict__ pad_trans, const double* __restrict__ pad_em,
                                     double (&g_out)[GR], double* __restrict__ fwd_out,
                                     int32_t* __restrict__ scal_out, const int32_t* __restrict__ jrs) {
-  const int W = J.n_rows, nL = J.n_left, nR = J.n_right;
+  const int nL = J.n_left, nR = J.n_right;
   int count = count_in;
   double fL[GL], fN[GR][4], fR[GR];
   double nli[GR][4];
@@ -782,26 +815,37 @@
     A = wave_sum(part);
   }
 
-  auto step = [&](int i, const RowTables<GL, GR>& t) __attribute__((always_inline)) {
+  sweep_rows<kPhased>(J, [&](int i, auto phase) __attribute__((always_inline)) {
+    using P = decltype(phase);
+    RowTables<GL, GR> t;
+    load_row<GL, GR, P::left, P::germ>(J, i, lane, t);
     unsigned key = key_start<kExt>();
     double part = 0.0;
 #pragma unroll
     for (int q = 0; q < GL; ++q) {
-      const double v = (fL[q] * t.ltr[q]) * jem[t.lidx[q]];
-      fL[q] = v;
-      key = key_add<kExt>(key, v);
-      part += v * t.llo[q];
+      if constexpr (P::left) {
+        const double v = (fL[q] * t.ltr[q]) * jem[t.lidx[q]];
+        fL[q] = v;
+        key = key_add<kExt>(key, v);
+        part += v * t.llo[q];
+      }
     }
 #pragma unroll
     for (int q = 0; q < GR; ++q)
-      key = right_gene_step<kExt>(key, fN[q], fR[q], A, nli[q], ntt_lds, lane + 64u * q, t.right[q], jem);
-    A = wave_sum(part);
+      key = right_gene_step<kExt, P::germ>(key, fN[q], fR[q], A, nli[q], ntt_lds, lane + 64u * q, t.right[q],
+                                                   jem);
+    if constexpr (P::left)
+      A = wave_sum(part);
+    else
+      A *= 0.0;
     const RowScale sc = wave_row_scale<kExt>(key);
-    if constexpr (kExt) count += jrs[i];
+    if constexpr (kExt) count += *jrs++;
     if (sc.k != 0) {
-      A = sc.apply(A);
-#pragma unroll
-      for (int q = 0; q < GL; ++q) fL[q] = sc.apply(fL[q]);
+      if constexpr (P::left) {
+        A = sc.apply(A);
+#pragma unroll
+        for (int q = 0; q < GL; ++q) fL[q] = sc.apply(fL[q]);
+      }
 #pragma unroll
       for (int q = 0; q < GR; ++q) {
         fR[q] = sc.apply(fR[q]);
@@ -811,7 +855,7 @@
       count += sc.k;
     }
     if (fwd_out) {
-      double* o = fwd_out + (size_t)i * row_stride;
+      double* o = fwd_out;
 #pragma unroll
       for (int q = 0; q < GL; ++q) {
         const int g = lane + 64 * q;
@@ -819,15 +863,16 @@
       }
 #pragma unroll
       for (int q = 0; q < GR; ++q) store_right(o, nL, nR, lane + 64u * q, fN[q], fR[q]);
-    }
-    if (scal_out && lane == 0) scal_out[i] = count;
-  };
-
-  for (int i = 0; i < W; ++i) {
-    RowTables<GL, GR> t;
-    load_row<GL, GR>(J, i, lane, t);
-    step(i, t);
-  }
+      fwd_out += row_stride;
+    }
+    if (scal_out) {
+      if (lane == 0) *scal_out = count;
+      ++scal_out;
+    }
+  }, [&] {
+#pragma unroll
+    for (int q = 0; q < GL; ++q) fL[q] *= 0.0;
+  });
 
   unsigned key = key_start<kExt>();
 #pragma unroll
@@ -883,7 +928,7 @@
                                     const double* __restrict__ pad_trans, const double* __restrict__ pad_em,
                                     double& g_out, double* __restrict__ fwd_out, int32_t* __restrict__ scal_out,
                                     const int32_t* __restrict__ jrs, bool valid) {
-  const int W = J.n_rows, nL = J.n_left, nR = J.n_right;
+  const int nL = J.n_left, nR = J.n_right;
   const unsigned g = lane & 31;
   int count = count_in;
   double fL = f_in, fR = 0.0, fN[4] = {0.0, 0.0, 0.0, 0.0}, nli[4];
@@ -891,41 +936,52 @@
   const size_t row_stride = (size_t)nL + 5 * (size_t)nR;
   auto mine = [&](const HalfPair& p) { return hi ? p.b : p.a; };
   double A = mine(half_sums(f_in * J.enter_lo[g]));
-  for (int i = 0; i < W; ++i) {
-    const size_t ol = (size_t)i * J.left_pad;
-    const double ltr = J.left_trans[ol + g], llo = J.left_lo[ol + g];
-    const int lidx = J.left_xmsa[ol + g];
+  sweep_rows<false>(J, [&](int i, auto phase) __attribute__((always_inline)) {
+    using P = decltype(phase);
     RightRow t;
-    load_right_row(J, i, g, t);
+    load_right_row<P::germ>(J, i, g, t);
 
     unsigned key = key_start<kExt>();
-    {
+    double part = 0.0;
+    if constexpr (P::left) {
+      const size_t ol = (size_t)i * J.left_pad;
+      const double ltr = J.left_trans[ol + g], llo = J.left_lo[ol + g];
+      const int lidx = J.left_xmsa[ol + g];
       const double v = (fL * ltr) * jem[lidx];
       fL = v;
       key = key_add<kExt>(key, v);
-    }
-    const double part = fL * llo;
-    key = right_gene_step<kExt>(key, fN, fR, A, nli, ntt_lds, g, t, jem);
-    A = mine(half_sums(part));
+      part = fL * llo;
+    }
+    key = right_gene_step<kExt, P::germ>(key, fN, fR, A, nli, ntt_lds, g, t, jem);
+    if constexpr (P::left)
+      A = mine(half_sums(part));
+    else
+      A *= 0.0;
     const HalfKeys hk = half_keys<kExt>(key);
     const RowScale sa = row_scale(hk.a), sb = row_scale(hk.b);
-    if constexpr (kExt) count += jrs[i];
+    if constexpr (kExt) count += *jrs++;
     if ((sa.k | sb.k) != 0) {
       const RowScale sc = pick(hi, sa, sb);
-      A = sc.apply(A);
-      fL = sc.apply(fL);
+      if constexpr (P::left) {
+        A = sc.apply(A);
+        fL = sc.apply(fL);
+      }
       fR = sc.apply(fR);
 #pragma unroll
       for (int b = 0; b < 4; ++b) fN[b] = sc.apply(fN[b]);
       count += sc.k;
     }
     if (fwd_out && valid) {
-      double* o = fwd_out + (size_t)i * row_stride;
+      double* o = fwd_out;
       if ((int)g < nL) o[g] = fL;
       store_right(o, nL, nR, g, fN, fR);
-    }
-    if (scal_out && valid && g == 0) scal_out[i] = count;
-  }
+      fwd_out += row_stride;
+    }
+    if (scal_out && valid) {
+      if (g == 0) *scal_out = count;
+      ++scal_out;
+    }
+  }, [&] { fL *= 0.0; });
   g_out = exit_handoff(J, g, nR, fN, fR, A, germ_em, pad_trans, pad_em);
   const HalfKeys hk = half_keys<kExt>(key_add<kExt>(key_start<kExt>(), g_out));
   const RowScale last = pick(hi, row_scale(hk.a), row_scale(hk.b));
@@ -1123,9 +1179,9 @@
   const int vcount = initial_v_forward<GA, kExt>(fam, gem, lane, cv, gV, fwd, sco);
   double gD[1];
   const int dcount =
-      cd + junction_wave<GA, 1, kExt>(fam.vd, jem, ntt_vd, lane, gV, vcount, gem + 2 * (size_t)nV, nullptr, nullptr, gD,
-                                      fwd ? fwd + nV : nullptr, sco ? sco + 1 : nullptr,
-                                      kExt ? jrs_all + (size_t)s * (fam.vd.n_rows + fam.dj.n_rows) : nullptr);
+      cd + junction_wave<GA, 1, kExt, false>(fam.vd, jem, ntt_vd, lane, gV, vcount, gem + 2 * (size_t)nV, nullptr, nullptr,
+                                             gD, fwd ? fwd + nV : nullptr, sco ? sco + 1 : nullptr,
+                                             kExt ? jrs_all + (size_t)s * (fam.vd.n_rows + fam.dj.n_rows) : nullptr);
   if (fwd && lane < nD) fwd[nV + vd_fwd + lane] = gD[0];
   if (sco && lane == 0) sco[1 + fam.vd.n_rows] = dcount;
   if (lane < 32) dxf[(size_t)s * 32 + lane] = gD[0];
@@ -1231,7 +1287,6 @@
 
 struct DjSample {
   const double *jgerm_em, *jpad_em;
-  int cj;
   double* fwd;
   int32_t* sco;
   const int32_t* jrs;
@@ -1246,7 +1301,6 @@
   DjSample d;
   d.jgerm_em = gem_all + (size_t)s * fam.gem_size + 2 * (size_t)nV + nD;
   d.jpad_em = d.jgerm_em + nJ;
-  d.cj = gcnt_all[(size_t)s * 3 + 2];
   d.fwd = fwd_all ? fwd_all + (size_t)s * fam.forward_size + nV + junction_fwd_size(fam.vd) + nD : nullptr;
   d.sco = scal_all ? scal_all + (size_t)s * fam.scaler_size + 2 + fam.vd.n_rows : nullptr;
   d.jrs = kExt ? jrs_all + (size_t)s * (fam.vd.n_rows + fam.dj.n_rows) + fam.vd.n_rows : nullptr;
@@ -1288,9 +1342,9 @@
   const double f_in = valid ? dxf[(size_t)s2 * 32 + g] : 0.0;
   const int dcount = valid ? dxc[s2] : 0;
   double gJ;
-  const int jcount = d.cj + junction_pair<kExt>(fam.dj, jem0 + (size_t)(hi ? 1 : 0) * (NJ + 1), ntt_dj, lane, hi, f_in,
-                                                dcount, d.jgerm_em, fam.jpadding_transition, d.jpad_em, gJ, d.fwd,
-                                                d.sco, d.jrs, valid);
+  const int swept = junction_pair<kExt>(fam.dj, jem0 + (size_t)(hi ? 1 : 0) * (NJ + 1), ntt_dj, lane, hi, f_in, dcount,
+                                        d.jgerm_em, fam.jpadding_transition, d.jpad_em, gJ, d.fwd, d.sco, d.jrs, valid);
+  const int jcount = gcnt_all[(size_t)sr * 3 + 2] + swept;
   dj_finish(fam, d, s2, valid, g, gJ, jcount, [&] {
     const HalfPair tot = half_sums(gJ);
     return hi ? tot.b : tot.a;
@@ -1341,7 +1395,7 @@
                                     const double* __restrict__ pad_trans, const double* __restrict__ pad_em,
                                     double& g_out, double* __restrict__ fwd_out, int32_t* __restrict__ scal_out,
                                     const int32_t* __restrict__ jrs, bool valid) {
-  const int W = J.n_rows, nL = J.n_left, nR = J.n_right;
+  const int nL = J.n_left, nR = J.n_right;
   int count = count_in;
   double fL[GL], fR = 0.0, fN[4] = {0.0, 0.0, 0.0, 0.0}, nli[4];
 #pragma unroll
@@ -1355,51 +1409,68 @@
     for (int q = 0; q < GL; ++q) part[q] = f_in[q] * J.enter_lo[l + 16u * q];
     A = row_sums<GL>(part);
   }
-  for (int i = 0; i < W; ++i) {
-    const size_t ol = (size_t)i * J.left_pad;
+  sweep_rows<!(kExt && GL == 2)>(J, [&](int i, auto phase) __attribute__((always_inline)) {
+    using P = decltype(phase);
     double ltr[GL], llo[GL];
     int lidx[GL];
-#pragma unroll
-    for (int q = 0; q < GL; ++q) {
-      ltr[q] = J.left_trans[ol + l + 16u * q];
-      llo[q] = J.left_lo[ol + l + 16u * q];
-      lidx[q] = J.left_xmsa[ol + l + 16u * q];
+    if constexpr (P::left) {
+      const size_t ol = (size_t)i * J.left_pad;
+#pragma unroll
+      for (int q = 0; q < GL; ++q) {
+        ltr[q] = J.left_trans[ol + l + 16u * q];
+        llo[q] = J.left_lo[ol + l + 16u * q];
+        lidx[q] = J.left_xmsa[ol + l + 16u * q];
+      }
     }
     RightRow t;
-    load_right_row(J, i, l, t);
+    load_right_row<P::germ>(J, i, l, t);
 
     unsigned key = key_start<kExt>();
     double part[GL];
 #pragma unroll
     for (int q = 0; q < GL; ++q) {
-      const double v = (fL[q] * ltr[q]) * jem[lidx[q]];
-      fL[q] = v;
-      key = key_add<kExt>(key, v);
-      part[q] = fL[q] * llo[q];
-    }
-    key = right_gene_step<kExt>(key, fN, fR, A, nli, ntt_lds, l, t, jem);
-    A = row_sums<GL>(part);
+      if constexpr (P::left) {
+        const double v = (fL[q] * ltr[q]) * jem[lidx[q]];
+        fL[q] = v;
+        key = key_add<kExt>(key, v);
+        part[q] = fL[q] * llo[q];
+      }
+    }
+    key = right_gene_step<kExt, P::germ>(key, fN, fR, A, nli, ntt_lds, l, t, jem);
+    if constexpr (P::left)
+      A = row_sums<GL>(part);
+    else
+      A *= 0.0;
     const unsigned rk = row_key<kExt>(key);
-    if constexpr (kExt) count += jrs[i];
+    if constexpr (kExt) count += *jrs++;
     if (__builtin_amdgcn_ballot_w64(rk < kRescaleKeyEnd) != 0) {
       const RowScale sc = row_scale(rk);
-      A = sc.apply(A);
-#pragma unroll
-      for (int q = 0; q < GL; ++q) fL[q] = sc.apply(fL[q]);
+      if constexpr (P::left) {
+        A = sc.apply(A);
+#pragma unroll
+        for (int q = 0; q < GL; ++q) fL[q] = sc.apply(fL[q]);
+      }
       fR = sc.apply(fR);
 #pragma unroll
       for (int b = 0; b < 4; ++b) fN[b] = sc.apply(fN[b]);
       count += sc.k;
     }
     if (fwd_out && valid) {
-      double* o = fwd_out + (size_t)i * row_stride;
+      double* o = fwd_out;
 #pragma unroll
       for (int q = 0; q < GL; ++q)
         if ((int)(l + 16u * q) < nL) o[l + 16u * q] = fL[q];
       store_right(o, nL, nR, l, fN, fR);
-    }
-    if (scal_out && valid && l == 0) scal_out[i] = count;
-  }
+      fwd_out += row_stride;
+    }
+    if (scal_out && valid) {
+      if (l == 0) *scal_out = count;
+      ++scal_out;
+    }
+  }, [&] {
+#pragma unroll
+    for (int q = 0; q < GL; ++q) fL[q] *= 0.0;
+  });
   g_out = exit_handoff(J, l, nR, fN, fR, A, germ_em, pad_trans, pad_em);
   const RowScale last = row_scale(row_key<kExt>(key_add<kExt>(key_start<kExt>(), g_out)));
   g_out = last.apply(g_out);
@@ -1434,9 +1505,9 @@
   for (int q = 0; q < GL; ++q) f_in[q] = valid ? dxf[(size_t)s4 * 32 + l + 16u * q] : 0.0;
   const int dcount = valid ? dxc[s4] : 0;
   double gJ;
-  const int jcount = d.cj + junction_quad<GL, kExt>(fam.dj, jem0 + (size_t)sub * (NJ + 1), ntt_dj, l, f_in, dcount,
-                                                    d.jgerm_em, fam.jpadding_transition, d.jpad_em, gJ, d.fwd, d.sco,
-                                                    d.jrs, valid);
+  const int swept = junction_quad<GL, kExt>(fam.dj, jem0 + (size_t)sub * (NJ + 1), ntt_dj, l, f_in, dcount, d.jgerm_em,
+                                            fam.jpadding_transition, d.jpad_em, gJ, d.fwd, d.sco, d.jrs, valid);
+  const int jcount = gcnt_all[(size_t)sr * 3 + 2] + swept;
   dj_finish(fam, d, s4, valid, l, gJ, jcount, [&] { return row_sums<1>({gJ}); }, loglik);
 }
 
@@ -1698,8 +1769,15 @@
     emission(slots_c<4>{});
   const int ga = (fam.vgerm.n_genes + 63) / 64;
   const int gb = (std::max(fam.dgerm.n_genes, fam.jgerm.n_genes) + 63) / 64;
+  static const bool full_rows = debug_options().k2b_full_rows;
+  DevFamily jfam = fam;
+  if (full_rows) {
+    jfam.vd.left_live_rows = jfam.vd.n_rows;
+    jfam.dj.left_live_rows = jfam.dj.n_rows;
+    jfam.vd.right_first_row = jfam.dj.right_first_row = 0;
+  }
   auto junction = [&](auto G) {
-    launch_junction_a<decltype(G)::value>(gb, fam, n, gem, gcnt, jem, jrs, dxf, dxc, loglik, forward_out, scaler_out, ext,
+    launch_junction_a<decltype(G)::value>(gb, jfam, n, gem, gcnt, jem, jrs, dxf, dxc, loglik, forward_out, scaler_out, ext,
                                           stream);
   };
   if (ga <= 1)
```
